# DOGECOIN87/firedancer

Hardware: AMD Instinct MI355X
Metric: verified ed25519 sigs/sec (node) (higher is better)
Workload: dtype u32; 1 GPU; cfg2: 1000000 single-sig txns/GPU, msg U[180,220] B, 90% valid / 10% corrupted, device-resident batch, full verify + per-txn combine per step; parallelism=dp1 (independent per-GPU batches), queues=2

## Files before the change

### firedancer_amd/_lib.py

```python
import ctypes
import os

_HERE = os.path.dirname(os.path.abspath(__file__))
LIB_PATH = os.environ.get("FDGPU_LIB") or os.path.join(_HERE, "libfd_ed25519_gpu.so")
HEADER_PATH = os.path.join(os.path.dirname(_HERE), "include", "fd_ed25519_gpu.h")
SHRED_HEADER_PATH = os.path.join(os.path.dirname(_HERE), "include", "fd_shred_gpu.h")
SHRED_SETS_HEADER_PATH = os.path.join(os.path.dirname(_HERE), "include", "fd_shred_sets_gpu.h")
POH_HEADER_PATH = os.path.join(os.path.dirname(_HERE), "include", "fd_poh_gpu.h")
PRECOMPILE_HEADER_PATH = os.path.join(os.path.dirname(_HERE), "include", "fd_precompile_gpu.h")
SECP256K1_HEADER_PATH = os.path.join(os.path.dirname(_HERE), "include", "fd_secp256k1_gpu.h")

_LIB = None


class FdgpuTxn(ctypes.Structure):
    _fields_ = [("msg_off", ctypes.c_uint32), ("msg_sz", ctypes.c_uint32),
                ("sig_off", ctypes.c_uint32), ("pub_off", ctypes.c_uint32),
                ("sig_cnt", ctypes.c_uint32)]


class FdgpuCfg(ctypes.Structure):
    _fields_ = [("max_txn", ctypes.c_uint64), ("max_sig", ctypes.c_uint64),
                ("max_arena", ctypes.c_uint64), ("ring_depth", ctypes.c_uint32),
                ("flags", ctypes.c_uint32)]


def lib():
    global _LIB
    if _LIB is not None:
        return _LIB
    if not os.path.exists(LIB_PATH):
        raise RuntimeError(f"firedancer_amd: engine library not built: {LIB_PATH} "
                           "(run `make -C firedancer_amd/csrc`)")
    L = ctypes.CDLL(LIB_PATH)
    c = ctypes
    vp, u8p = c.c_void_p, c.c_char_p
    L.fd_ed25519_verify.argtypes = [u8p, c.c_uint64, u8p, u8p, vp]
    L.fd_ed25519_verify.restype = c.c_int
    L.fd_ed25519_verify_batch_single_msg.argtypes = [u8p, c.c_uint64, u8p, u8p, vp, c.c_uint8]
    L.fd_ed25519_verify_batch_single_msg.restype = c.c_int
    L.fd_ed25519_strerror.argtypes = [c.c_int]
    L.fd_ed25519_strerror.restype = c.c_char_p
    L.fdgpu_engine_open.argtypes = [c.c_int, c.POINTER(FdgpuCfg)]
    L.fdgpu_engine_open.restype = vp
    L.fdgpu_engine_reserve.argtypes = [vp, c.c_uint64]
    L.fdgpu_engine_reserve.restype = c.c_int
    L.fdgpu_engine_close.argtypes = [vp]
    L.fdgpu_engine_close.restype = None
    L.fdgpu_last_error.argtypes = []
    L.fdgpu_last_error.restype = c.c_char_p
    L.fdgpu_device_count.argtypes = []
    L.fdgpu_device_count.restype = c.c_int
    L.fdgpu_kernel_path.argtypes = []
    L.fdgpu_kernel_path.restype = c.c_char_p
    L.fdgpu_build_info.argtypes = []
    L.fdgpu_build_info.restype = c.c_char_p
    L.fdgpu_submit.argtypes = [vp, vp, c.c_uint64, vp, c.c_uint64]
    L.fdgpu_submit.restype = c.c_int64
    L.fdgpu_poll.argtypes = [vp, c.c_int64, vp, c.c_int]
    L.fdgpu_poll.restype = c.c_int
    L.fdgpu_stage_acquire.argtypes = [vp, c.POINTER(c.c_uint64)]
    L.fdgpu_stage_acquire.restype = vp
    L.fdgpu_stage_submit.argtypes = [vp, c.c_uint64, vp, c.c_uint64]
    L.fdgpu_stage_submit.restype = c.c_int64
    L.fdgpu_poll_keep.argtypes = [vp, c.c_int64, vp, c.c_int]
    L.fdgpu_poll_keep.restype = c.c_int
    L.fdgpu_release.argtypes = [vp, c.c_int64]
    L.fdgpu_release.restype = c.c_int
    L.fdgpu_stage_cancel.argtypes = [vp]
    L.fdgpu_stage_cancel.restype = c.c_int
    L.fdgpu_host_register.argtypes = [vp, vp, c.c_uint64]
    L.fdgpu_host_register.restype = c.c_int
    L.fdgpu_host_unregister.argtypes = [vp, vp]
    L.fdgpu_host_unregister.restype = c.c_int
    L.fdgpu_verify_device.argtypes = [vp, vp, vp, c.c_uint64, vp, c.c_uint64, vp, vp, vp]
    L.fdgpu_verify_device.restype = c.c_int
    L.fdgpu_engine_info.argtypes = [vp, c.POINTER(c.c_uint32), c.POINTER(c.c_uint32), c.POINTER(c.c_uint64)]
    L.fdgpu_engine_info.restype = c.c_int
    L.fdgpu_debug_fe_ops.argtypes = [vp, vp, c.c_uint64, vp]
    L.fdgpu_debug_decode.argtypes = [vp, vp, c.c_uint64, c.c_int, vp]
    L.fdgpu_debug_sha512.argtypes = [vp, vp, c.c_uint64, vp, c.c_uint64, vp]
    L.fdgpu_debug_hram.argtypes = [vp, vp, c.c_uint64, vp, c.c_uint64, vp]
    L.fdgpu_debug_sc_reduce.argtypes = [vp, vp, c.c_uint64, vp]
    L.fdgpu_debug_hs_split.argtypes = [vp, vp, c.c_uint64, vp]
    L.fdgpu_debug_sig_codes.argtypes = [vp, vp, c.c_uint64, vp, c.c_uint64, vp]
    L.fdgpu_dev_batch_upload.argtypes = [vp, vp, c.c_uint64, vp, c.c_uint64]
    L.fdgpu_dev_batch_upload.restype = vp
    L.fdgpu_dev_batch_verify.argtypes = [vp, vp]
    L.fdgpu_dev_batch_verify.restype = c.c_int
    L.fdgpu_dev_batch_own_queue.argtypes = [vp, vp]
    L.fdgpu_dev_batch_own_queue.restype = c.c_int
    L.fdgpu_dev_batch_codes.argtypes = [vp, vp, vp, vp]
    L.fdgpu_dev_batch_codes.restype = c.c_int
    L.fdgpu_dev_batch_upload_frags.argtypes = [vp, vp, c.c_uint64, vp, c.c_uint64]
    L.fdgpu_dev_batch_upload_frags.restype = vp
    L.fdgpu_dev_batch_txns.argtypes = [vp, vp, vp, vp]
    L.fdgpu_dev_batch_txns.restype = c.c_int
    L.fdgpu_dev_batch_time2.argtypes = [vp, vp, c.c_int] + [c.POINTER(c.c_double)] * 4
    L.fdgpu_dev_batch_time2.restype = c.c_int
    L.fdgpu_dev_batch_free.argtypes = [vp, vp]
    L.fdgpu_dev_batch_free.restype = None
    L.fdgpu_dev_batch_sig_cnt.argtypes = [vp]
    L.fdgpu_dev_batch_sig_cnt.restype = c.c_uint64
    L.fdgpu_dev_batch_device_ptrs.argtypes = [vp] + [vp] * 6
    L.fdgpu_dev_batch_device_ptrs.restype = c.c_int
    L.fdgpu_dev_batch_time.argtypes = [vp, vp, c.c_int, c.POINTER(c.c_double), c.POINTER(c.c_double),
                                       c.POINTER(c.c_double)]
    L.fdgpu_dev_batch_time.restype = c.c_int
    L.fdgpu_sync.argtypes = [vp]
    L.fdgpu_sync.restype = c.c_int
    L.fdgpu_submit_frags.argtypes = [vp, vp, c.c_uint64, vp, c.c_uint64, c.c_uint64]
    L.fdgpu_submit_frags.restype = c.c_int64
    L.fdgpu_poll_frags.argtypes = [vp, c.c_int64, vp, vp, c.c_int]
    L.fdgpu_poll_frags.restype = c.c_int
    L.fdgpu_submit_frags_io.argtypes = [vp, vp, c.c_uint64, vp, c.c_uint64, c.c_uint64, vp, c.c_uint64]
    L.fdgpu_submit_frags_io.restype = c.c_int64
    L.fdgpu_poll_frags_io.argtypes = [vp, c.c_int64, vp, vp, vp, c.c_int]
    L.fdgpu_poll_frags_io.restype = c.c_int
    L.fdgpu_debug_submit_times.argtypes = [vp, c.c_uint64]
    L.fdgpu_debug_submit_times.restype = c.c_uint64
    L.fdgpu_debug_h2d_gbps.argtypes = [vp, vp, c.c_uint64, c.c_int]
    L.fdgpu_debug_h2d_gbps.restype = c.c_double
    L.fdgpu_frag_out_cap.argtypes = [c.c_uint32]
    L.fdgpu_frag_out_cap.restype = c.c_uint32
    L.fdgpu_ed25519_verify.argtypes = [u8p, c.c_uint64, u8p, u8p]
    L.fdgpu_ed25519_verify.restype = c.c_int
    L.fdgpu_ed25519_verify_batch_single_msg.argtypes = [u8p, c.c_uint64, u8p, u8p, c.c_uint8]
    L.fdgpu_ed25519_verify_batch_single_msg.restype = c.c_int
    L.fdgpu_sync_stats.argtypes = [c.POINTER(c.c_uint64)] * 3
    L.fdgpu_sync_stats.restype = None
    L.fdgpu_sync_errors.argtypes = []
    L.fdgpu_sync_errors.restype = c.c_uint64
    L.fdgpu_submit_shreds.argtypes = [vp, vp, c.c_uint64, vp, c.c_uint64, c.c_uint16]
    L.fdgpu_submit_shreds.restype = c.c_int64
    L.fdgpu_poll_shreds.argtypes = [vp, c.c_int64, vp, vp, c.c_int]
    L.fdgpu_poll_shreds.restype = c.c_int
    L.fdgpu_debug_sha256.argtypes = [vp, vp, c.c_uint64, vp, c.c_uint64, vp]
    L.fdgpu_debug_sha256.restype = c.c_int
    L.fdgpu_debug_shred_roots.argtypes = [vp, vp, c.c_uint64, vp, c.c_uint64, c.c_uint16, vp, vp]
    L.fdgpu_debug_shred_roots.restype = c.c_int
    L.fdgpu_debug_shred_time.argtypes = [vp, vp, c.c_uint64, vp, c.c_uint64, c.c_uint16, c.c_int,
                                         c.POINTER(c.c_double), c.POINTER(c.c_double)]
    L.fdgpu_debug_shred_time.restype = c.c_int
    L.fdgpu_submit_shred_sets.argtypes = [vp, vp, c.c_uint64, vp, c.c_uint64, c.c_uint16]
    L.fdgpu_submit_shred_sets.restype = c.c_int64
    L.fdgpu_poll_shred_sets.argtypes = [vp, c.c_int64, vp, vp, vp, c.POINTER(c.c_uint64), c.c_int]
    L.fdgpu_poll_shred_sets.restype = c.c_int
    L.fdgpu_debug_shred_sets_time.argtypes = [vp, vp, c.c_uint64, vp, c.c_uint64, c.c_uint16, c.c_int,
                                              c.POINTER(c.c_double), c.POINTER(c.c_double)]
    L.fdgpu_debug_shred_sets_time.restype = c.c_int
    L.fdgpu_submit_poh.argtypes = [vp, vp, c.c_uint64, vp, c.c_uint64, vp, c.c_uint64, c.c_uint64]
    L.fdgpu_submit_poh.restype = c.c_int64
    L.fdgpu_poll_poh.argtypes = [vp, c.c_int64, vp, vp, c.c_int]
    L.fdgpu_poll_poh.restype = c.c_int
    L.fdgpu_poh_limits.argtypes = [vp] + [c.POINTER(c.c_uint64)] * 3
    L.fdgpu_poh_limits.restype = c.c_int
    L.fdgpu_poh_chunk.argtypes = []
    L.fdgpu_poh_chunk.restype = c.c_uint32
    L.fdgpu_debug_poh.argtypes = [vp, vp, c.c_uint64, vp, c.c_uint64, vp, c.c_uint64, c.c_uint64, c.c_uint32, vp, vp]
    L.fdgpu_debug_poh.restype = c.c_int
    L.fdgpu_debug_poh_time.argtypes = [vp, vp, c.c_uint64, vp, c.c_uint64, vp, c.c_uint64, c.c_uint64, c.c_int,
                                       c.POINTER(c.c_double), c.POINTER(c.c_double)]
    L.fdgpu_debug_poh_time.restype = c.c_int
    L.fdgpu_precompile_sig_bound.argtypes = [c.c_uint64]
    L.fdgpu_precompile_sig_bound.restype = c.c_uint32
    L.fdgpu_submit_precompiles.argtypes = [vp, vp, c.c_uint64, vp, c.c_uint64]
    L.fdgpu_submit_precompiles.restype = c.c_int64
    L.fdgpu_poll_precompiles.argtypes = [vp, c.c_int64, vp, vp, c.c_int]
    L.fdgpu_poll_precompiles.restype = c.c_int
    L.fdgpu_debug_precompile_walk.argtypes = [vp, vp, c.c_uint64, vp, c.c_uint64, vp, vp, vp, c.c_uint64,
                                              c.POINTER(c.c_uint64)]
    L.fdgpu_debug_precompile_walk.restype = c.c_int
    L.fdgpu_debug_precompile_time.argtypes = [vp, vp, c.c_uint64, vp, c.c_uint64, c.c_int, c.POINTER(c.c_double),
                                              c.POINTER(c.c_double)]
    L.fdgpu_debug_precompile_time.restype = c.c_int
    L.fdgpu_secp256k1_sig_bound.argtypes = [c.c_uint64]
    L.fdgpu_secp256k1_sig_bound.restype = c.c_uint32
    L.fdgpu_submit_secp256k1.argtypes = [vp, vp, c.c_uint64, vp, c.c_uint64, c.c_uint32]
    L.fdgpu_submit_secp256k1.restype = c.c_int64
    L.fdgpu_poll_secp256k1.argtypes = [vp, c.c_int64, vp, vp, c.c_int]
    L.fdgpu_poll_secp256k1.restype = c.c_int
    L.fdgpu_debug_secp256k1_walk.argtypes = [vp, vp, c.c_uint64, vp, c.c_uint64, c.c_uint32, vp, vp, vp, c.c_uint64,
                                             c.POINTER(c.c_uint64)]
    L.fdgpu_debug_secp256k1_walk.restype = c.c_int
    L.fdgpu_debug_keccak256.argtypes = [vp, vp, c.c_uint64, vp, c.c_uint64, vp]
    L.fdgpu_debug_keccak256.restype = c.c_int
    L.fdgpu_debug_secp256k1_recover.argtypes = [vp, vp, c.c_uint64, vp, vp]
    L.fdgpu_debug_secp256k1_recover.restype = c.c_int
    L.fdgpu_debug_secp256k1_time.argtypes = [vp, vp, c.c_uint64, vp, c.c_uint64, c.c_uint32, c.c_int,
                                             c.POINTER(c.c_double), c.POINTER(c.c_double)]
    L.fdgpu_debug_secp256k1_time.restype = c.c_int
    L.fdgpu_debug_secp256k1_ops.argtypes = [vp, vp, c.c_uint64, vp]
    L.fdgpu_debug_secp256k1_ops.restype = c.c_int
    L.fdgpu_debug_fe_raw.argtypes = [vp, vp, c.c_uint64, vp]
    L.fdgpu_debug_ge_ops.argtypes = [vp, vp, c.c_uint64, vp]
    L.fdgpu_debug_sc_recode.argtypes = [vp, vp, c.c_uint64, vp]
    L.fdgpu_debug_btab.argtypes = [vp, c.c_uint64, c.c_uint64, vp]
    L.fdgpu_debug_tabpack.argtypes = [vp, vp, c.c_uint64, vp]
    L.fdgpu_debug_verify_prehashed.argtypes = [vp, vp, c.c_uint64, vp, c.c_uint64, c.c_uint32, vp,
                                               c.POINTER(c.c_uint32)]
    L.fdgpu_bcomb_dim.argtypes = [c.c_int]
    L.fdgpu_bcomb_dim.restype = c.c_uint32
    L.fdgpu_test_ge_in_words.argtypes = []
    L.fdgpu_test_ge_in_words.restype = c.c_uint32
    L.fdgpu_test_ge_results.argtypes = []
    L.fdgpu_test_ge_results.restype = c.c_uint32
    for fn in ("fdgpu_debug_fe_ops", "fdgpu_debug_decode", "fdgpu_debug_sha512", "fdgpu_debug_hram",
               "fdgpu_debug_sc_reduce", "fdgpu_debug_hs_split", "fdgpu_debug_sig_codes",
               "fdgpu_debug_fe_raw", "fdgpu_debug_ge_ops", "fdgpu_debug_sc_recode", "fdgpu_debug_btab",
               "fdgpu_debug_tabpack", "fdgpu_debug_verify_prehashed"):
        getattr(L, fn).restype = c.c_int
    _LIB = L
    return L


def header_functions(path=None):
    import re
    text = open(path or HEADER_PATH).read()
    text = re.sub(r"/\*.*?\*/", "", text, flags=re.S)
    names = re.findall(r"^[A-Za-z_][\w \t\*]*?\b(fd\w+)\s*\(", text, flags=re.M)
    return sorted(set(n for n in names if not n.startswith("FD_")))


def build_info():
    import json
    return json.loads(lib().fdgpu_build_info().decode())


def require_product_build(allow_ab=False):
    info = build_info()
    if not info.get("product") and not allow_ab:
        raise RuntimeError(f"firedancer_amd: {LIB_PATH} is not the product build: {info} "
                           "(rebuild with `make -C firedancer_amd/csrc`, or pass the A/B flag)")
    return info


def last_error():
    return lib().fdgpu_last_error().decode()
```

### firedancer_amd/csrc/fdgpu_atab.h

```cpp
#pragma once

#include <hip/hip_runtime.h>

#include "fdgpu_ge.h"
#include "fdgpu_internal.h"

namespace fdgpu {

FDG_DEV void fe_tight(fe &h) {
#pragma unroll
  for (int pass = 0; pass < 2; pass++) {
#pragma unroll
    for (int i = 0; i < 9; i++) {
      const int w = (i & 1) ? 25 : 26;
      h.v[i + 1] += h.v[i] >> w;
      h.v[i] &= (1u << w) - 1;
    }
    const uint32_t c = h.v[9] >> 25;
    h.v[9] &= (1u << 25) - 1;
    h.v[0] += 19u * c;
  }
}

FDG_DEV void fe_pack8(uint32_t (&w)[8], const fe &t) {
#pragma unroll
  for (int h = 0; h < 2; h++) {
    const uint32_t s = t.v[8 + h];
    w[4 * h + 0] = t.v[4 * h + 0] | (s << 26);
    w[4 * h + 1] = t.v[4 * h + 1] | ((s >> 6) << 25);
    w[4 * h + 2] = t.v[4 * h + 2] | ((s >> 13) << 26);
    w[4 * h + 3] = t.v[4 * h + 3] | ((s >> 19) << 25);
  }
}

FDG_DEV void fe_unpack8(uint32_t *q, const uint32_t (&w)[8]) {
#pragma unroll
  for (int j = 0; j < 8; j++) q[j] = w[j] & ((j & 1) ? (1u << 25) - 1 : (1u << 26) - 1);
#pragma unroll
  for (int h = 0; h < 2; h++) {
    uint32_t s = w[4 * h + 3] >> 25;
    s = (s << 6) | (w[4 * h + 2] >> 26);
    s = (s << 7) | (w[4 * h + 1] >> 25);
    s = (s << 6) | (w[4 * h + 0] >> 26);
    q[8 + h] = s;
  }
}

__host__ __device__ constexpr int atab_pos(int c, int j) {
  return c >= 2 ? 8 * c + j : 4 * (j / 2) + 2 * c + (j % 2);
}

struct alignas(128) tab_ident_t { uint32_t w[FDGPU_PTAB_WORDS]; };
static __device__ const tab_ident_t g_tab_ident = {{1u, 0u, 1u, 0u, 0u, 0u, 0u, 0u, 0u, 0u, 0u, 0u, 0u, 0u, 0u, 0u, 2u}};
static_assert(atab_pos(0, 0) == 0 && atab_pos(1, 0) == 2 && atab_pos(2, 0) == 16 && atab_pos(3, 7) == 31 &&
              atab_pos(0, 7) == 13 && atab_pos(1, 7) == 15, "the stored order (and the identity entry's)");

FDG_DEV const uint32_t *tab_entry(const uint32_t *tab, int e) {
  return e ? tab + (uint32_t)(e < 0 ? -e : e) * FDGPU_PTAB_WORDS : g_tab_ident.w;
}

FDG_DEV void atab_store(uint32_t *tab, uint32_t entry, const ge_cached &c) {
  uint4 *p = (uint4 *)(tab + entry * FDGPU_PTAB_WORDS);
  uint32_t o[FDGPU_PTAB_WORDS];
#pragma unroll
  for (int cc = 0; cc < 4; cc++) {
    fe t = cc == 0 ? c.YpX : cc == 1 ? c.YmX : cc == 2 ? c.Z2 : c.T2d;
    fe_tight(t);
    uint32_t w[8];
    fe_pack8(w, t);
#pragma unroll
    for (int j = 0; j < 8; j++) o[atab_pos(cc, j)] = w[j];
  }
#pragma unroll
  for (int q = 0; q < 8; q++) p[q] = make_uint4(o[4 * q], o[4 * q + 1], o[4 * q + 2], o[4 * q + 3]);
}

FDG_DEV void atab_unpack(uint32_t (&q)[40], const uint32_t (&o)[FDGPU_PTAB_WORDS]) {
#pragma unroll
  for (int cc = 0; cc < 4; cc++) {
    uint32_t w[8];
#pragma unroll
    for (int j = 0; j < 8; j++) w[j] = o[atab_pos(cc, j)];
    fe_unpack8(q + 10 * cc, w);
  }
}

FDG_DEV void atab_load(uint32_t (&q)[40], const uint32_t *tab, int e) {
  const uint4 *ent = (const uint4 *)tab_entry(tab, e);
  uint32_t o[FDGPU_PTAB_WORDS];
#pragma unroll
  for (int i = 0; i < 8; i++) {
    const uint4 v = ent[i];
    o[4 * i] = v.x; o[4 * i + 1] = v.y; o[4 * i + 2] = v.z; o[4 * i + 3] = v.w;
  }
  atab_unpack(q, o);
}

FDG_DEV uint32_t atab_limb(const uint32_t *ent, int c, int w) {
  if (w < 8) return ent[atab_pos(c, w)] & ((w & 1) ? (1u << 25) - 1 : (1u << 26) - 1);
  const int b = 4 * (w - 8);
  uint32_t s = ent[atab_pos(c, b + 3)] >> 25;
  s = (s << 6) | (ent[atab_pos(c, b + 2)] >> 26);
  s = (s << 7) | (ent[atab_pos(c, b + 1)] >> 25);
  s = (s << 6) | (ent[atab_pos(c, b + 0)] >> 26);
  return s;
}

typedef __attribute__((address_space(3))) void lds_void_t;

FDG_DEV void stage_entry(uint32_t *lds_wave, const uint32_t *tab, int e) {
  const uint32_t *src = tab_entry(tab, e);
  constexpr int NCH = FDGPU_PTAB_WORDS / 4;
#pragma unroll
  for (int c = 0; c < NCH; c++)
    __builtin_amdgcn_global_load_lds((const void *)(src + 4 * c), (lds_void_t *)(lds_wave + 256 * c), 16, 0, 0);
}

FDG_DEV void unstage_entry_signed(uint32_t (&q)[40], const uint32_t *lds_wave, bool neg) {
  const uint32_t lane = threadIdx.x & 63u;
  const uint32_t *a = lds_wave + 4 * lane + (neg ? 2u : 0u), *b = lds_wave + 4 * lane + (neg ? 0u : 2u);
  uint32_t o[FDGPU_PTAB_WORDS];
#pragma unroll
  for (int c = 0; c < 4; c++) {
    const uint2 x = *(const uint2 *)(a + 256 * c), y = *(const uint2 *)(b + 256 * c);
    o[4 * c] = x.x; o[4 * c + 1] = x.y; o[4 * c + 2] = y.x; o[4 * c + 3] = y.y;
  }
#pragma unroll
  for (int c = 4; c < 8; c++) {
    const uint4 v = *(const uint4 *)(lds_wave + 256 * c + 4 * lane);
    o[4 * c] = v.x; o[4 * c + 1] = v.y; o[4 * c + 2] = v.z; o[4 * c + 3] = v.w;
  }
  atab_unpack(q, o);
}

}
```

### firedancer_amd/csrc/fdgpu_consts.h

```cpp
#pragma once
#include <stdint.h>

#define FDGPU_FE_D { 0x35978a3u, 0x0d37284u, 0x3156ebdu, 0x06a0a0eu, 0x001c029u, 0x179e898u, 0x3a03cbbu, 0x1ce7198u, 0x2e2b6ffu, 0x1480db3u }
#define FDGPU_FE_D2 { 0x2b2f159u, 0x1a6e509u, 0x22add7au, 0x0d4141du, 0x0038052u, 0x0f3d130u, 0x3407977u, 0x19ce331u, 0x1c56dffu, 0x0901b67u }
#define FDGPU_FE_SQRTM1 { 0x20ea0b0u, 0x186c9d2u, 0x08f189du, 0x035697fu, 0x0bd0c60u, 0x1fbd7a7u, 0x2804c9eu, 0x1e16569u, 0x004fc1du, 0x0ae0c92u }
#define FDGPU_FE_BX { 0x325d51au, 0x18b5823u, 0x0f6592au, 0x104a92du, 0x1a4b31du, 0x1d6dc5cu, 0x27118feu, 0x07fd814u, 0x13cd6e5u, 0x085a4dbu }
#define FDGPU_FE_BY { 0x2666658u, 0x1999999u, 0x0ccccccu, 0x1333333u, 0x1999999u, 0x0666666u, 0x3333333u, 0x0ccccccu, 0x2666666u, 0x1999999u }
#define FDGPU_FE_BT { 0x1b7dda3u, 0x1a2ace9u, 0x25eadbbu, 0x003ba8au, 0x083c27eu, 0x0abe37du, 0x1274732u, 0x0ccacddu, 0x0fd78b7u, 0x19e1d7cu }
#define FDGPU_FE_Y0 { 0x395e826u, 0x1ecb0a3u, 0x068b604u, 0x1944fa6u, 0x3c263bfu, 0x1acdfd5u, 0x1e36982u, 0x1162726u, 0x2d88023u, 0x017f14du }
#define FDGPU_FE_Y1 { 0x06a17c7u, 0x0134f5cu, 0x39749fbu, 0x06bb059u, 0x03d9c40u, 0x053202au, 0x21c967du, 0x0e9d8d9u, 0x1277fdcu, 0x1e80eb2u }

#define FDGPU_FE_2P { 0x07ffffdau, 0x03fffffeu, 0x07fffffeu, 0x03fffffeu, 0x07fffffeu, 0x03fffffeu, 0x07fffffeu, 0x03fffffeu, 0x07fffffeu, 0x03fffffeu }
#define FDGPU_FE_4P { 0x0fffffb4u, 0x07fffffcu, 0x0ffffffcu, 0x07fffffcu, 0x0ffffffcu, 0x07fffffcu, 0x0ffffffcu, 0x07fffffcu, 0x0ffffffcu, 0x07fffffcu }

#define FDGPU_SC_L { 0x5cf5d3edu, 0x5812631au, 0xa2f79cd6u, 0x14def9deu, 0x00000000u, 0x00000000u, 0x00000000u, 0x10000000u }
#define FDGPU_SC_MU { 0x0a2c131bu, 0xed9ce5a3u, 0x086329a7u, 0x2106215du, 0xffffffebu, 0xffffffffu, 0xffffffffu, 0xffffffffu, 0x0000000fu }
```

### firedancer_amd/csrc/fdgpu_diag.cpp

```cpp
#include "fdgpu_engine.h"
#include "fdgpu_shred.h"

using namespace fdgpu;

#define DALLOC(buf, n) do { if ((buf).alloc((size_t)(n) * sizeof(*(buf).p) + 64) != hipSuccess) { \
  set_err("alloc"); return FDGPU_ERR_DEVICE; } } while (0)

using MsgLaunch = hipError_t (*)(const uint8_t *, const fdgpu_sig_desc_t *, uint32_t, uint32_t *, hipStream_t);
static int debug_msgs(fdgpu_engine_t *e, uint8_t const *arena, uint64_t arena_sz, fdgpu_txn_t const *txns, uint64_t n,
                      uint8_t *out, MsgLaunch launch, uint64_t out_bytes, bool sig_pub) {
  if (!e || !n) return FDGPU_ERR_INVAL;
  HIPCHK(hipSetDevice(e->device), FDGPU_ERR_DEVICE);
  std::vector<fdgpu_sig_desc_t> d(n);
  for (uint64_t i = 0; i < n; i++) {
    if ((uint64_t)txns[i].msg_off + txns[i].msg_sz > arena_sz ||
        (sig_pub && ((uint64_t)txns[i].sig_off + 64 > arena_sz || (uint64_t)txns[i].pub_off + 32 > arena_sz))) {
      set_err("descriptor out of bounds"); return FDGPU_ERR_INVAL;
    }
    d[i].msg_off = txns[i].msg_off; d[i].msg_sz = txns[i].msg_sz;
    d[i].sig_off = txns[i].sig_off; d[i].pub_off = txns[i].pub_off;
  }
  DevBuf<uint8_t> da;
  DevBuf<fdgpu_sig_desc_t> dd;
  DevBuf<uint8_t> dout;
  HIPCHK(dev_arena(da, arena, arena_sz), FDGPU_ERR_DEVICE);
  DALLOC(dd, n);
  DALLOC(dout, n * out_bytes);
  HIPCHK(hipMemcpy(dd, d.data(), n * sizeof(fdgpu_sig_desc_t), hipMemcpyHostToDevice), FDGPU_ERR_DEVICE);
  HIPCHK(launch(da, dd, (uint32_t)n, (uint32_t *)dout.p, e->compute), FDGPU_ERR_DEVICE);
  HIPCHK(hipStreamSynchronize(e->compute), FDGPU_ERR_DEVICE);
  HIPCHK(hipMemcpy(out, dout, n * out_bytes, hipMemcpyDeviceToHost), FDGPU_ERR_DEVICE);
  return FDGPU_OK;
}

template <class Launch>
static int debug_map(fdgpu_engine_t *e, uint8_t const *in, uint64_t n, uint64_t in_words, uint64_t out_words,
                     uint8_t *out, Launch launch) {
  if (!e || !n) return FDGPU_ERR_INVAL;
  HIPCHK(hipSetDevice(e->device), FDGPU_ERR_DEVICE);
  DevBuf<uint32_t> din, dout;
  DALLOC(din, n * in_words);
  DALLOC(dout, n * out_words);
  HIPCHK(hipMemcpy(din, in, n * in_words * 4, hipMemcpyHostToDevice), FDGPU_ERR_DEVICE);
  HIPCHK(launch(din.p, dout.p, (uint32_t)n, e->compute), FDGPU_ERR_DEVICE);
  HIPCHK(hipStreamSynchronize(e->compute), FDGPU_ERR_DEVICE);
  HIPCHK(hipMemcpy(out, dout, n * out_words * 4, hipMemcpyDeviceToHost), FDGPU_ERR_DEVICE);
  return FDGPU_OK;
}

int fdgpu::time_two_stages(hipStream_t st, int iters, const char *what, const std::function<bool()> &warm,
                           const std::function<bool()> &first, const std::function<bool()> &second, double *first_ms,
                           double *second_ms) {
  Events ev;
  if (!ev.create(3)) { (void)hipGetLastError(); set_err("event"); return FDGPU_ERR_DEVICE; }
  bool ok = warm() && hipEventRecord(ev[0], st) == hipSuccess;
  for (int i = 0; i < iters && ok; i++) ok = first();
  ok = ok && hipEventRecord(ev[1], st) == hipSuccess;
  for (int i = 0; i < iters && ok; i++) ok = second();
  ok = ok && hipEventRecord(ev[2], st) == hipSuccess && hipEventSynchronize(ev[2]) == hipSuccess;
  float a = 0.f, b = 0.f;
  ok = ok && hipEventElapsedTime(&a, ev[0], ev[1]) == hipSuccess && hipEventElapsedTime(&b, ev[1], ev[2]) == hipSuccess;
  if (!ok) { (void)hipGetLastError(); set_err("%s timing failed", what); return FDGPU_ERR_DEVICE; }
  *first_ms = a / iters;
  *second_ms = b / iters;
  return FDGPU_OK;
}

extern "C" {

int fdgpu_debug_fe_ops(fdgpu_engine_t *e, uint8_t const *ab, uint64_t n, uint8_t *out) {
  return debug_map(e, ab, n, 16, 64, out, fdgpu_launch_test_fe);
}

int fdgpu_debug_decode(fdgpu_engine_t *e, uint8_t const *enc, uint64_t n, int ref_mapping, uint8_t *out) {
  const uint32_t flags = ref_mapping ? FDGPU_FLAG_REF_MAP : 0u;
  return debug_map(e, enc, n, 8, 18, out, [flags](const uint32_t *i, uint32_t *o, uint32_t k, hipStream_t st) {
    return fdgpu_launch_test_decode(i, o, k, flags, st);
  });
}

int fdgpu_debug_sha512(fdgpu_engine_t *e, uint8_t const *arena, uint64_t arena_sz, fdgpu_txn_t const *msgs,
                       uint64_t n, uint8_t *out) {
  return debug_msgs(e, arena, arena_sz, msgs, n, out, fdgpu_launch_test_sha512, 64, false);
}

int fdgpu_debug_hram(fdgpu_engine_t *e, uint8_t const *arena, uint64_t arena_sz, fdgpu_txn_t const *txns,
                     uint64_t n, uint8_t *out) {
  return debug_msgs(e, arena, arena_sz, txns, n, out, fdgpu_launch_test_hram, 32, true);
}

int fdgpu_debug_sha256(fdgpu_engine_t *e, uint8_t const *arena, uint64_t arena_sz, fdgpu_txn_t const *msgs, uint64_t n,
                       uint8_t *out) {
  if (!e || !n || !msgs || !out || (!arena && arena_sz) || arena_sz > 0xFFFFFF00ull) { set_err("bad argument"); return FDGPU_ERR_INVAL; }
  return debug_msgs(e, arena, arena_sz, msgs, n, out, fdgpu_launch_test_sha256, 32, false);
}

int fdgpu_debug_sc_reduce(fdgpu_engine_t *e, uint8_t const *in, uint64_t n, uint8_t *out) {
  return debug_map(e, in, n, 16, 8, out, fdgpu_launch_test_sc_reduce);
}

int fdgpu_debug_hs_split(fdgpu_engine_t *e, uint8_t const *k, uint64_t n, uint8_t *out) {
  return debug_map(e, k, n, 8, 16, out, fdgpu_launch_test_hs_split);
}

int fdgpu_debug_fe_raw(fdgpu_engine_t *e, uint8_t const *fg, uint64_t n, uint8_t *out) {
  return debug_map(e, fg, n, 20, 80, out, fdgpu_launch_test_fe_raw);
}

int fdgpu_debug_ge_ops(fdgpu_engine_t *e, uint8_t const *in, uint64_t n, uint8_t *out) {
  return debug_map(e, in, n, fdgpu_test_ge_in_words(), 32u * fdgpu_test_ge_results(), out, fdgpu_launch_test_ge);
}

int fdgpu_debug_sc_recode(fdgpu_engine_t *e, uint8_t const *s, uint64_t n, uint8_t *out) {
  return debug_map(e, s, n, 8, 16, out, fdgpu_launch_test_sc_recode);
}

int fdgpu_debug_tabpack(fdgpu_engine_t *e, uint8_t const *in, uint64_t n, uint8_t *out) {
  return debug_map(e, in, n, FDGPU_ATAB_WORDS, FDGPU_TABPACK_OUT_WORDS, out, fdgpu_launch_test_tabpack);
}

int fdgpu_debug_verify_prehashed(fdgpu_engine_t *e, uint8_t const *arena, uint64_t arena_sz,
                                 fdgpu_sig_desc_t const *descs, uint64_t n, uint32_t flags, int8_t *codes_out,
                                 uint32_t *n_full_out) {
  if (!e || !e->d_btab || !arena || !descs || !codes_out || !n_full_out || !n || n > (1u << 20) ||
      arena_sz > 0xFFFFFF00ull || (flags & ~(uint32_t)(FDGPU_FLAG_REF_MAP | FDGPU_FLAG_KFULL | FDGPU_FLAG_KPAIR))) {
    set_err("fdgpu_debug_verify_prehashed: bad argument"); return FDGPU_ERR_INVAL;
  }
  for (uint64_t i = 0; i < n; i++) {
    if ((descs[i].msg_off & 7u) || (uint64_t)descs[i].msg_off + 64 > arena_sz ||
        (uint64_t)descs[i].sig_off + 64 > arena_sz || (uint64_t)descs[i].pub_off + 32 > arena_sz) {
      set_err("fdgpu_debug_verify_prehashed: descriptor out of bounds"); return FDGPU_ERR_INVAL;
    }
  }
  HIPCHK(hipSetDevice(e->device), FDGPU_ERR_DEVICE);
  DevBuf<uint8_t> da;
  DevBuf<fdgpu_sig_desc_t> dd;
  DevBuf<int8_t> dc;
  DevBuf<uint32_t> dws;
  HIPCHK(dev_arena(da, arena, arena_sz), FDGPU_ERR_DEVICE);
  DALLOC(dd, n);
  DALLOC(dc, n);
  if (dws.alloc(fdgpu_ws_bytes(n)) != hipSuccess) { set_err("alloc"); return FDGPU_ERR_DEVICE; }
  HIPCHK(hipMemcpy(dd, descs, n * sizeof(fdgpu_sig_desc_t), hipMemcpyHostToDevice), FDGPU_ERR_DEVICE);
  HIPCHK(hipMemsetAsync(dc, 0x7f, n, e->compute), FDGPU_ERR_DEVICE);
  HIPCHK(fdgpu_launch_verify_prehashed(da, dd, (uint32_t)n, e->d_btab, dws, dc, flags, e->compute), FDGPU_ERR_DEVICE);
  HIPCHK(hipStreamSynchronize(e->compute), FDGPU_ERR_DEVICE);
  HIPCHK(hipMemcpy(codes_out, dc, n, hipMemcpyDeviceToHost), FDGPU_ERR_DEVICE);
  HIPCHK(hipMemcpy(n_full_out, fdgpu_ws_layout(dws, n).cnt, sizeof(uint32_t), hipMemcpyDeviceToHost), FDGPU_ERR_DEVICE);
  return FDGPU_OK;
}

int fdgpu_debug_btab(fdgpu_engine_t *e, uint64_t first_entry, uint64_t n_entries, uint32_t *out) {
  const uint64_t total = (uint64_t)FDGPU_BCOMB_NDIG * FDGPU_BCOMB_ENTRIES;
  if (!e || !e->d_btab || !out || first_entry > total || n_entries > total - first_entry) {
    set_err("fdgpu_debug_btab: entries out of the table"); return FDGPU_ERR_INVAL;
  }
  if (!n_entries) return FDGPU_OK;
  HIPCHK(hipSetDevice(e->device), FDGPU_ERR_DEVICE);
  HIPCHK(hipStreamSynchronize(e->compute), FDGPU_ERR_DEVICE);
  HIPCHK(hipMemcpy(out, e->d_btab + first_entry * FDGPU_BCOMB_STRIDE, n_entries * FDGPU_BCOMB_STRIDE * sizeof(uint32_t),
                   hipMemcpyDeviceToHost), FDGPU_ERR_DEVICE);
  return FDGPU_OK;
}

uint32_t fdgpu_bcomb_dim(int which) {
  switch (which) {
    case 0: return FDGPU_BCOMB_BITS;
    case 1: return FDGPU_BCOMB_NDIG;
    case 2: return FDGPU_BCOMB_ENTRIES;
    case 3: return FDGPU_BCOMB_STRIDE;
    case 4: return FDGPU_BCOMB_CHUNK;
    default: return 0u;
  }
}

int fdgpu_debug_sig_codes(fdgpu_engine_t *e, uint8_t const *arena, uint64_t arena_sz, fdgpu_txn_t const *txns,
                          uint64_t txn_cnt, int8_t *sig_codes) {
  if (!e) return FDGPU_ERR_INVAL;
  HIPCHK(hipSetDevice(e->device), FDGPU_ERR_DEVICE);
  uint64_t total = 0;
  for (uint64_t t = 0; t < txn_cnt; t++) total += (txns[t].sig_cnt >= 1 && txns[t].sig_cnt <= 16) ? txns[t].sig_cnt : 0;
  std::vector<fdgpu_sig_desc_t> sd(total + 1);
  std::vector<fdgpu_txn_desc_t> td(txn_cnt + 1);
  std::vector<uint32_t> pm(total + 1);
  uint32_t *perm = bucket(e) ? pm.data() : nullptr;
  const int64_t ns = expand(arena_sz, txns, txn_cnt, total, sd.data(), td.data(), perm);
  if (ns < 0) return FDGPU_ERR_INVAL;
  if (!ns) return FDGPU_OK;
  DevBuf<uint8_t> da;
  DevBuf<fdgpu_sig_desc_t> dd;
  DevBuf<uint32_t> dp;
  DevBuf<int8_t> dc;
  HIPCHK(dev_arena(da, arena, arena_sz), FDGPU_ERR_DEVICE);
  DALLOC(dd, ns);
  DALLOC(dp, ns);
  DALLOC(dc, ns);
  HIPCHK(hipMemcpy(dd, sd.data(), ns * sizeof(fdgpu_sig_desc_t), hipMemcpyHostToDevice), FDGPU_ERR_DEVICE);
  if (perm) HIPCHK(hipMemcpy(dp, perm, ns * sizeof(uint32_t), hipMemcpyHostToDevice), FDGPU_ERR_DEVICE);
  const uint32_t flags = kflags(e);
  if ((uint64_t)ns > e->ws_sig) { int rc = ensure_ws(e, (uint64_t)ns); if (rc) return rc; }
  HIPCHK(fdgpu_launch_verify_sigs(da, dd, (uint32_t)ns, perm ? dp.p : nullptr, e->d_btab, e->d_ws, dc, flags,
                                  e->compute, nullptr, e->resident_blocks, e->kc_seed),
         FDGPU_ERR_DEVICE);
  HIPCHK(hipStreamSynchronize(e->compute), FDGPU_ERR_DEVICE);
  HIPCHK(hipMemcpy(sig_codes, dc, ns, hipMemcpyDeviceToHost), FDGPU_ERR_DEVICE);
  return FDGPU_OK;
}

}
```

### firedancer_amd/csrc/fdgpu_ge.h

```cpp
#pragma once

#include "fdgpu_fe.h"

namespace fdgpu {

struct ge_p2 { fe X, Y, Z; };
struct ge_p3 { fe X, Y, Z, T; };
struct ge_p1p1 { fe X, Y, Z, T; };
struct ge_cached { fe YpX, YmX, Z2, T2d; };
struct ge_niels { fe ypx, ymx, xy2d; };

FDG_DEV void ge_p2_0(ge_p2 &h) { fe_0(h.X); fe_1(h.Y); fe_1(h.Z); }
FDG_DEV void ge_p3_0(ge_p3 &h) { fe_0(h.X); fe_1(h.Y); fe_1(h.Z); fe_0(h.T); }
FDG_DEV void ge_cached_0(ge_cached &h) { fe_1(h.YpX); fe_1(h.YmX); fe_0(h.Z2); h.Z2.v[0] = 2; fe_0(h.T2d); }

FDG_DEV void ge_p1p1_to_p2(ge_p2 &r, const ge_p1p1 &p) {
  fe_mul(r.X, p.X, p.T);
  fe_mul(r.Y, p.Z, p.Y);
  fe_mul(r.Z, p.Z, p.T);
}
FDG_DEV void ge_p1p1_to_p3(ge_p3 &r, const ge_p1p1 &p) {
  fe_mul(r.X, p.X, p.T);
  fe_mul(r.Y, p.Z, p.Y);
  fe_mul(r.Z, p.Z, p.T);
  fe_mul(r.T, p.X, p.Y);
}

FDG_DEV void ge_dbl(ge_p1p1 &r, const ge_p2 &p) {
  fe s;
  fe_sq(r.X, p.X);
  fe_sq(r.Z, p.Y);
  fe_add(r.Y, r.Z, r.X);
  fe_sub(r.Z, r.Z, r.X);
  fe_add(s, p.X, p.Y);
  fe_sq(r.X, s);
  fe_sub4(r.X, r.X, r.Y);
  fe_sq2(r.T, p.Z);
  fe_sub4(r.T, r.T, r.Z);
  fe_carry_par(r.T);
}

FDG_DEV void fe_cswap(fe &a, fe &b, bool c) {
#pragma unroll
  for (int i = 0; i < 10; i++) { const uint32_t x = a.v[i], y = b.v[i]; a.v[i] = c ? y : x; b.v[i] = c ? x : y; }
}
FDG_DEV void fe_cneg(fe &a, bool c) {
  constexpr uint32_t P2[10] = FDGPU_FE_2P;
#pragma unroll
  for (int i = 0; i < 10; i++) a.v[i] = c ? P2[i] - a.v[i] : a.v[i];
}

FDG_DEV void ge_add_cached(ge_p1p1 &r, const ge_p3 &p, ge_cached q, bool neg) {
  fe t;
  fe_cswap(q.YpX, q.YmX, neg);
  fe_cneg(q.T2d, neg);
  fe_mul(r.Z, p.T, q.T2d);
  fe_mul(r.T, p.Z, q.Z2);
  fe_add(t, p.Y, p.X);
  fe_mul(r.X, t, q.YpX);
  fe_sub(t, p.Y, p.X);
  fe_mul(r.Y, t, q.YmX);
  fe_add(t, r.T, r.Z);
  fe_sub(r.T, r.T, r.Z);
  r.Z = t;
  fe_add(t, r.X, r.Y);
  fe_sub(r.X, r.X, r.Y);
  r.Y = t;
}

FDG_DEV void ge_add_niels(ge_p1p1 &r, const ge_p3 &p, ge_niels q, bool neg) {
  fe t;
  fe_cswap(q.ypx, q.ymx, neg);
  fe_cneg(q.xy2d, neg);
  fe_mul(r.Z, p.T, q.xy2d);
  fe_add(r.T, p.Z, p.Z);
  fe_add(t, p.Y, p.X);
  fe_mul(r.X, t, q.ypx);
  fe_sub(t, p.Y, p.X);
  fe_mul(r.Y, t, q.ymx);
  fe_add(t, r.T, r.Z);
  fe_sub(r.T, r.T, r.Z);
  fe_carry(r.T);
  r.Z = t;
  fe_add(t, r.X, r.Y);
  fe_sub(r.X, r.X, r.Y);
  r.Y = t;
}

template <class LD>
FDG_DEV void ld_fe(fe &h, const LD &ld, int coord) {
#pragma unroll
  for (int i = 0; i < 10; i++) h.v[i] = ld(coord, i);
}

template <class LD>
FDG_DEV void ge_add_cached_ld(ge_p1p1 &r, const ge_p3 &p, const LD &ld, bool neg) {
  fe t, q;
  ld_fe(q, ld, 3); fe_cneg(q, neg);
  fe_mul(r.Z, p.T, q);
  ld_fe(q, ld, 2);
  fe_mul(r.T, p.Z, q);
  ld_fe(q, ld, neg ? 1 : 0);
  fe_add(t, p.Y, p.X);
  fe_mul(r.X, t, q);
  ld_fe(q, ld, neg ? 0 : 1);
  fe_sub(t, p.Y, p.X);
  fe_mul(r.Y, t, q);
  fe_add(t, r.T, r.Z);
  fe_sub(r.T, r.T, r.Z);
  r.Z = t;
  fe_add(t, r.X, r.Y);
  fe_sub(r.X, r.X, r.Y);
  r.Y = t;
}

template <class LD>
FDG_DEV void ge_add_niels_ld(ge_p1p1 &r, const ge_p3 &p, const LD &ld, bool neg) {
  fe t, q;
  ld_fe(q, ld, 2); fe_cneg(q, neg);
  fe_mul(r.Z, p.T, q);
  fe_add(r.T, p.Z, p.Z);
  ld_fe(q, ld, neg ? 1 : 0);
  fe_add(t, p.Y, p.X);
  fe_mul(r.X, t, q);
  ld_fe(q, ld, neg ? 0 : 1);
  fe_sub(t, p.Y, p.X);
  fe_mul(r.Y, t, q);
  fe_add(t, r.T, r.Z);
  fe_sub(r.T, r.T, r.Z);
  fe_carry_par(r.T);
  r.Z = t;
  fe_add(t, r.X, r.Y);
  fe_sub(r.X, r.X, r.Y);
  r.Y = t;
}

FDG_DEV void ge_add_cached_regs(ge_p1p1 &r, const ge_p3 &p, const uint32_t (&q)[40], bool neg) {
  fe t, c;
#pragma unroll
  for (int i = 0; i < 10; i++) c.v[i] = q[30 + i];
  fe_cneg(c, neg);
  fe_mul(r.Z, p.T, c);
#pragma unroll
  for (int i = 0; i < 10; i++) c.v[i] = q[20 + i];
  fe_mul(r.T, p.Z, c);
#pragma unroll
  for (int i = 0; i < 10; i++) c.v[i] = neg ? q[10 + i] : q[i];
  fe_add(t, p.Y, p.X);
  fe_mul(r.X, t, c);
#pragma unroll
  for (int i = 0; i < 10; i++) c.v[i] = neg ? q[i] : q[10 + i];
  fe_sub(t, p.Y, p.X);
  fe_mul(r.Y, t, c);
  fe_add(t, r.T, r.Z);
  fe_sub(r.T, r.T, r.Z);
  r.Z = t;
  fe_add(t, r.X, r.Y);
  fe_sub(r.X, r.X, r.Y);
  r.Y = t;
}

FDG_DEV void ge_add_cached_regs_swapped(ge_p1p1 &r, const ge_p3 &p, const uint32_t (&q)[40], bool neg) {
  fe t, c;
#pragma unroll
  for (int i = 0; i < 10; i++) c.v[i] = q[30 + i];
  fe_cneg(c, neg);
  fe_mul(r.Z, p.T, c);
#pragma unroll
  for (int i = 0; i < 10; i++) c.v[i] = q[20 + i];
  fe_mul(r.T, p.Z, c);
#pragma unroll
  for (int i = 0; i < 10; i++) c.v[i] = q[i];
  fe_add(t, p.Y, p.X);
  fe_mul(r.X, t, c);
#pragma unroll
  for (int i = 0; i < 10; i++) c.v[i] = q[10 + i];
  fe_sub(t, p.Y, p.X);
  fe_mul(r.Y, t, c);
  fe_add(t, r.T, r.Z);
  fe_sub(r.T, r.T, r.Z);
  r.Z = t;
  fe_add(t, r.X, r.Y);
  fe_sub(r.X, r.X, r.Y);
  r.Y = t;
}

FDG_DEV void ge_cached_regs_to_p2(ge_p2 &r, const uint32_t (&q)[40], bool neg) {
  fe a, b;
#pragma unroll
  for (int i = 0; i < 10; i++) { a.v[i] = neg ? q[10 + i] : q[i]; b.v[i] = neg ? q[i] : q[10 + i]; }
  fe_sub(r.X, a, b); fe_carry(r.X);
  fe_add(r.Y, a, b); fe_carry(r.Y);
#pragma unroll
  for (int i = 0; i < 10; i++) r.Z.v[i] = q[20 + i];
}

FDG_DEV void ge_niels_regs_to_p3(ge_p3 &r, const uint32_t (&q)[32], bool neg) {
  fe a, b, x2, y2;
#pragma unroll
  for (int i = 0; i < 10; i++) { a.v[i] = neg ? q[10 + i] : q[i]; b.v[i] = neg ? q[i] : q[10 + i]; }
  fe_sub(x2, a, b); fe_carry(x2);
  fe_add(y2, a, b); fe_carry(y2);
  fe_mul(r.T, x2, y2);
  fe_add(r.X, x2, x2); fe_carry(r.X);
  fe_add(r.Y, y2, y2); fe_carry(r.Y);
  fe_0(r.Z); r.Z.v[0] = 4;
}

FDG_DEV void ge_add_niels_regs(ge_p1p1 &r, const ge_p3 &p, const uint32_t (&q)[32], bool neg) {
  fe t, c;
#pragma unroll
  for (int i = 0; i < 10; i++) c.v[i] = q[20 + i];
  fe_cneg(c, neg);
  fe_mul(r.Z, p.T, c);
  fe_add(r.T, p.Z, p.Z);
#pragma unroll
  for (int i = 0; i < 10; i++) c.v[i] = neg ? q[10 + i] : q[i];
  fe_add(t, p.Y, p.X);
  fe_mul(r.X, t, c);
#pragma unroll
  for (int i = 0; i < 10; i++) c.v[i] = neg ? q[i] : q[10 + i];
  fe_sub(t, p.Y, p.X);
  fe_mul(r.Y, t, c);
  fe_add(t, r.T, r.Z);
  fe_sub(r.T, r.T, r.Z);
  fe_carry_par(r.T);
  r.Z = t;
  fe_add(t, r.X, r.Y);
  fe_sub(r.X, r.X, r.Y);
  r.Y = t;
}

FDG_DEV void ge_p3_to_cached(ge_cached &r, const ge_p3 &p) {
  constexpr uint32_t D2[10] = FDGPU_FE_D2;
  fe d2; fe_set(d2, D2);
  fe_add(r.YpX, p.Y, p.X); fe_carry(r.YpX);
  fe_sub(r.YmX, p.Y, p.X); fe_carry(r.YmX);
  fe_add(r.Z2, p.Z, p.Z);  fe_carry(r.Z2);
  fe_mul(r.T2d, p.T, d2);
}

FDG_DEV void ge_p3_to_p2(ge_p2 &r, const ge_p3 &p) { r.X = p.X; r.Y = p.Y; r.Z = p.Z; }

FDG_DEV void ge_p3_neg(ge_p3 &r, const ge_p3 &p) {
  fe_neg(r.X, p.X); fe_carry(r.X);
  r.Y = p.Y; r.Z = p.Z;
  fe_neg(r.T, p.T); fe_carry(r.T);
}

FDG_DEV bool ge_decode(ge_p3 &P, const uint32_t (&enc)[8], bool ref_map) {
  constexpr uint32_t DD[10] = FDGPU_FE_D, SQ[10] = FDGPU_FE_SQRTM1;
  fe d, sqrtm1, one;
  fe_set(d, DD); fe_set(sqrtm1, SQ); fe_1(one);
  const uint32_t sign = enc[7] >> 31;
  fe y, ysq, u, v, v2, v3, v4, uv3, uv7, t0, x, x2, vx2, t1, t2;
  fe_frombytes(y, enc);
  fe_sq(ysq, y);
  fe_sub(u, ysq, one);
  fe_mul(v, d, ysq); fe_add(v, v, one);
  fe_sq(v2, v);
  fe_sq(v4, v2);
  fe_mul(v3, v, v2);
  fe_mul(uv3, u, v3);
  fe_mul(uv7, uv3, v4);
  fe_pow22523(t0, uv7);
  fe_mul(x, uv3, t0);
  fe_sq(x2, x);
  fe_mul(vx2, v, x2);
  fe_carry(u);
  fe_sub(t1, vx2, u);
  fe_add(t2, vx2, u);
  const bool t1nz = !fe_iszero(t1), t2nz = !fe_iszero(t2);
  bool ok = !(t1nz && t2nz);
  fe xs; fe_mul(xs, x, sqrtm1);
  fe_cmov(x, xs, x, t1nz);
  fe xc = x; fe_canon(xc);
  uint32_t xnz = 0;
#pragma unroll
  for (int i = 0; i < 10; i++) xnz |= xc.v[i];
  if (!ref_map && xnz == 0 && sign) ok = false;
  fe nx; fe_neg(nx, xc); fe_carry(nx);
  fe_cmov(x, nx, xc, (xc.v[0] & 1u) != sign);
  P.X = x; P.Y = y; fe_1(P.Z); fe_mul(P.T, x, y);
  return ok;
}

FDG_DEV bool ge_is_small_order_affine(const ge_p3 &P) {
  constexpr uint32_t Y0[10] = FDGPU_FE_Y0, Y1[10] = FDGPU_FE_Y1;
  fe y0, y1; fe_set(y0, Y0); fe_set(y1, Y1);
  fe yc = P.Y; fe_canon(yc);
  bool yz = true, e0 = true, e1 = true;
#pragma unroll
  for (int i = 0; i < 10; i++) { yz &= yc.v[i] == 0; e0 &= yc.v[i] == y0.v[i]; e1 &= yc.v[i] == y1.v[i]; }
  return fe_iszero(P.X) || yz || e0 || e1;
}

}
```

### firedancer_amd/csrc/fdgpu_internal.h

```cpp
#pragma once

#include <hip/hip_runtime_api.h>
#include <stddef.h>
#include <stdint.h>

#include "../../include/fd_ed25519_gpu.h"
#include "../../include/fd_poh_gpu.h"

typedef struct {
  uint32_t msg_off;
  uint32_t msg_sz;
  uint32_t sig_off;
  uint32_t pub_off;
} fdgpu_sig_desc_t;

typedef struct {
  uint32_t sig0;
  uint32_t sig_cnt;
} fdgpu_txn_desc_t;

#define FDGPU_ARENA_SLACK   160u
#define FDGPU_ATAB_ENTRIES  9u
#ifndef FDGPU_ATAB_WORDS
#define FDGPU_ATAB_WORDS    40u
#endif
#define FDGPU_PTAB_WORDS    32u
#ifndef FDGPU_VERIFY_WAVES
#define FDGPU_VERIFY_WAVES  2
#endif
#ifndef FDGPU_PHASE_STAMPS
#define FDGPU_PHASE_STAMPS  0
#endif
#define FDGPU_BCOMB_BITS    16u
#define FDGPU_BCOMB_NDIG    ((254u + FDGPU_BCOMB_BITS - 1u) / FDGPU_BCOMB_BITS)
#define FDGPU_BCOMB_ENTRIES ((1u << (FDGPU_BCOMB_BITS - 1u)) + 1u)
#define FDGPU_BCOMB_STRIDE  32u
#define FDGPU_BCOMB_CHUNK   64u
#define HS_MAX_WIN          40u
#define FDGPU_TAB_STORED    (FDGPU_ATAB_ENTRIES - 1u)
#define FDGPU_WS_RTAB       FDGPU_TAB_STORED
#define FDGPU_WS_ENTRIES    (2u * FDGPU_TAB_STORED + 2u)
#define FDGPU_WS_LANE_WORDS (FDGPU_WS_ENTRIES * FDGPU_ATAB_WORDS)
#define FDGPU_WS_TAB_WORDS  (2u * FDGPU_TAB_STORED * FDGPU_PTAB_WORDS)
#define FDGPU_WS_AUX_WORDS  (FDGPU_WS_LANE_WORDS - FDGPU_WS_TAB_WORDS)
#define FDGPU_AUX_PARK      0u
#define FDGPU_AUX_SB        FDGPU_ATAB_WORDS
#define FDGPU_BLOCK         256u
#define FDGPU_FLAG_REF_MAP  1u
#define FDGPU_FLAG_KFULL    2u
#define FDGPU_FLAG_KCACHE   4u
#define FDGPU_FLAG_KPAIR    8u
#define FDGPU_FLAG_KSPREAD  16u
#define FDGPU_STAGE_WAVE_WORDS (FDGPU_PTAB_WORDS / 4u * 256u)
#define FDGPU_STAGE_LDS        (FDGPU_BLOCK / 64u * 2u * FDGPU_STAGE_WAVE_WORDS * 4u)
#define FDGPU_STAGE_LDS_PAIR   (FDGPU_BLOCK / 64u * FDGPU_STAGE_WAVE_WORDS * 4u)
#define FDGPU_CU_LDS           (160u * 1024u)
#define FDGPU_SPREAD_LDS       (FDGPU_CU_LDS / 2u - FDGPU_STAGE_LDS + 1024u)
#define FDGPU_SPREAD_LDS_PAIR  (FDGPU_CU_LDS / 2u - FDGPU_STAGE_LDS_PAIR + 1024u)
#ifdef __cplusplus
static_assert(2u * (FDGPU_STAGE_LDS + FDGPU_SPREAD_LDS) > FDGPU_CU_LDS &&
              2u * (FDGPU_STAGE_LDS_PAIR + FDGPU_SPREAD_LDS_PAIR) > FDGPU_CU_LDS &&
              FDGPU_STAGE_LDS + FDGPU_SPREAD_LDS <= FDGPU_CU_LDS && FDGPU_STAGE_LDS_PAIR + FDGPU_SPREAD_LDS_PAIR <= FDGPU_CU_LDS,
              "a spread launch's LDS admits one block per CU, and no more");
#endif
#define FDGPU_FULL_BLOCKS   16u
#define FDGPU_AUX_BLOCKS    64u
#define FDGPU_IO_BLOCKS     16u
#define FDGPU_NBLK_GROUPS   32u
#define FDGPU_POH_CHUNK     64u

#ifdef __cplusplus
extern "C" {
#endif


size_t     fdgpu_btab_bytes(void);
hipError_t fdgpu_btab_build(uint32_t *d_btab, hipStream_t stream);

hipError_t fdgpu_launch_verify_sigs(const uint8_t *d_arena, const fdgpu_sig_desc_t *d_sigs, uint32_t n_sig,
                                    const uint32_t *d_perm, const uint32_t *d_btab, uint32_t *d_ws,
                                    int8_t *d_sig_codes, uint32_t flags, hipStream_t stream,
                                    const uint32_t *d_n_sig, uint32_t resident_blocks, uint64_t kc_seed,
                                    int cnt_zeroed = 0);
uint64_t   fdgpu_sha512_stream_blocks(uint64_t msg_sz);
hipError_t fdgpu_launch_sha512_stream(const uint8_t *d_mbuf, uint64_t m0, uint64_t mlen, uint64_t msg_sz,
                                      uint64_t blk0, uint32_t nblk, const uint8_t *d_ra, uint64_t *d_state,
                                      uint32_t n, hipStream_t stream);
hipError_t fdgpu_launch_verify_prehashed(const uint8_t *d_arena, const fdgpu_sig_desc_t *d_sigs, uint32_t n_sig,
                                         const uint32_t *d_btab, uint32_t *d_ws, int8_t *d_sig_codes, uint32_t flags,
                                         hipStream_t stream);
typedef struct {
  uint64_t lanes, ht_slots;
  uint32_t *queue, *cnt, *rep_cnt, *ht, *key_of, *kverd, *reps;
  size_t bytes;
} fdgpu_ws_layout_t;
static inline fdgpu_ws_layout_t fdgpu_ws_layout(uint32_t *d_ws, uint64_t n_sig) {
  fdgpu_ws_layout_t l;
  l.lanes = (n_sig + FDGPU_BLOCK - 1) / FDGPU_BLOCK * FDGPU_BLOCK;
  for (l.ht_slots = 64; l.ht_slots < 2 * l.lanes;) l.ht_slots <<= 1;
  const uint64_t queue = l.lanes * FDGPU_WS_LANE_WORDS, cnt = queue + l.lanes, ht = cnt + 16, key_of = ht + l.ht_slots;
  auto at = [d_ws](uint64_t word) { return d_ws ? d_ws + word : nullptr; };
  l.queue = at(queue);
  l.cnt = at(cnt);
  l.rep_cnt = at(cnt + 1);
  l.ht = at(ht);
  l.key_of = at(key_of);
  l.kverd = at(key_of + l.lanes);
  l.reps = at(key_of + 2 * l.lanes);
  l.bytes = (size_t)(key_of + 3 * l.lanes) * sizeof(uint32_t);
  return l;
}
typedef struct {
  const uint8_t *arena;
  const fdgpu_sig_desc_t *sigs;
  const uint32_t *n_sig;
  uint32_t *ws;
  int8_t *codes;
  uint32_t *queue, *cnt;
  uint32_t bound;
  uint32_t slow;
} fdgpu_mbatch_t;
hipError_t fdgpu_launch_verify_multi(const fdgpu_mbatch_t *mb, uint32_t nb, uint32_t grid_max, uint32_t slow_max,
                                     const uint32_t *d_btab, uint32_t flags, hipStream_t stream);
hipError_t fdgpu_launch_combine(const fdgpu_txn_desc_t *d_txns, uint32_t n_txn, const int8_t *d_sig_codes,
                                int8_t *d_txn_codes, uint64_t *d_accept, hipStream_t stream);
hipError_t fdgpu_verify_occupancy(int *blocks_per_cu);
int        fdgpu_kernel_build_info(char *buf, size_t n);
size_t     fdgpu_ws_bytes(uint64_t n_sig);

__attribute__((visibility("hidden"))) hipError_t fdgpu_ingest_load(void);
uint64_t   fdgpu_frag_sig_bound(uint32_t sz);
hipError_t fdgpu_launch_frag_ingest(const uint8_t *d_arena, const void *d_frags, uint32_t frag_stride, uint32_t n,
                                    uint8_t *d_txn_out, uint16_t *d_txn_sz, fdgpu_txn_t *d_txd, uint32_t *d_cnt,
                                    uint32_t *d_sig0, uint32_t *d_blocktot, uint32_t *d_n_sig,
                                    fdgpu_sig_desc_t *d_sigs, fdgpu_txn_desc_t *d_tds, hipStream_t stream);
hipError_t fdgpu_launch_frag_codes(const uint16_t *d_txn_sz, uint32_t n, int8_t *d_codes, hipStream_t stream);
#define FDGPU_SMALL_SCAN_MAX 65536u
hipError_t fdgpu_launch_frag_ring(const uint8_t *d_arena, const fdgpu_frag_ex_t *d_fx, uint32_t n, uint8_t *d_txn_out,
                                  uint16_t *d_txn_sz, fdgpu_txn_t *d_txd, uint32_t *d_cnt, uint32_t *d_sig0,
                                  uint32_t *d_blocktot, uint32_t *d_n_sig, fdgpu_sig_desc_t *d_sigs,
                                  fdgpu_txn_desc_t *d_tds, hipStream_t stream);
hipError_t fdgpu_launch_frag_finish(const fdgpu_txn_desc_t *d_tds, uint32_t n, const int8_t *d_sig_codes,
                                    const uint16_t *d_txn_sz, const fdgpu_frag_ex_t *d_fx, const uint8_t *d_txn_out,
                                    int8_t *d_codes, uint8_t *d_trailers, hipStream_t stream);
#define FDGPU_FX_LAPPED 0x80000000u
#define FDGPU_IO_RANGES_MAX 255u
uint64_t   fdgpu_frag_fp_bound(uint32_t sz);
hipError_t fdgpu_launch_frag_ingest_io(const uint64_t *d_src, const fdgpu_frag_ex_t *d_fx, const uint64_t *d_chk,
                                       const uint64_t *d_rtab, uint32_t n, uint8_t *d_arena,
                                       fdgpu_frag_ex_t *d_fx_dev, uint8_t *d_txn_out, uint16_t *d_txn_sz,
                                       fdgpu_sig_desc_t *d_sigs, fdgpu_txn_desc_t *d_tds, uint32_t *d_n_sig,
                                       uint32_t *d_zero_word, hipStream_t stream);
hipError_t fdgpu_launch_frag_finish_io(const fdgpu_txn_desc_t *d_tds, uint32_t n, const int8_t *d_sig_codes,
                                       const uint16_t *d_txn_sz, const fdgpu_frag_ex_t *d_fx, const uint8_t *d_txn_out,
                                       const uint8_t *d_arena, uint64_t hash_seed, uint8_t *d_out, int8_t *d_codes,
                                       uint64_t *d_tags, uint16_t *d_out_szs, uint32_t *d_zero_next,
                                       hipStream_t stream);

hipError_t fdgpu_launch_poh_tree(const uint8_t *d_arena, const fdgpu_poh_entry_t *d_entries, uint32_t n,
                                 const uint32_t *d_sig_offs, uint32_t sig_total, uint32_t *d_nodes, hipStream_t stream);
hipError_t fdgpu_launch_poh_chains(const uint8_t *d_arena, const fdgpu_poh_entry_t *d_entries, uint32_t n,
                                   const uint32_t *d_order, uint32_t n_q, const uint32_t *d_nodes, uint32_t cap,
                                   uint32_t grid_waves, uint32_t *d_head, int8_t *d_codes, uint8_t *d_hashes,
                                   hipStream_t stream);

hipError_t fdgpu_launch_test_fe(const uint32_t *d_in, uint32_t *d_out, uint32_t n, hipStream_t stream);
hipError_t fdgpu_launch_test_decode(const uint32_t *d_enc, uint32_t *d_out, uint32_t n, uint32_t flags, hipStream_t stream);
hipError_t fdgpu_launch_test_sha512(const uint8_t *d_arena, const fdgpu_sig_desc_t *d_msgs, uint32_t n,
                                    uint32_t *d_out, hipStream_t stream);
hipError_t fdgpu_launch_test_hram(const uint8_t *d_arena, const fdgpu_sig_desc_t *d_sigs, uint32_t n,
                                  uint32_t *d_out, hipStream_t stream);
hipError_t fdgpu_launch_test_sc_reduce(const uint32_t *d_in, uint32_t *d_out, uint32_t n, hipStream_t stream);
hipError_t fdgpu_launch_test_hs_split(const uint32_t *d_in, uint32_t *d_out, uint32_t n, hipStream_t stream);
hipError_t fdgpu_launch_test_fe_raw(const uint32_t *d_in, uint32_t *d_out, uint32_t n, hipStream_t stream);
uint32_t   fdgpu_test_ge_in_words(void);
uint32_t   fdgpu_test_ge_results(void);
hipError_t fdgpu_launch_test_ge(const uint32_t *d_in, uint32_t *d_out, uint32_t n, hipStream_t stream);
hipError_t fdgpu_launch_test_sc_recode(const uint32_t *d_in, uint32_t *d_out, uint32_t n, hipStream_t stream);
#define FDGPU_TABPACK_OUT_WORDS 160u
hipError_t fdgpu_launch_test_tabpack(const uint32_t *d_in, uint32_t *d_out, uint32_t n, hipStream_t stream);

int      fdgpu_debug_fe_raw(fdgpu_engine_t *e, uint8_t const *fg, uint64_t n, uint8_t *out);
int      fdgpu_debug_ge_ops(fdgpu_engine_t *e, uint8_t const *in, uint64_t n, uint8_t *out);
int      fdgpu_debug_sc_recode(fdgpu_engine_t *e, uint8_t const *s, uint64_t n, uint8_t *out);
int      fdgpu_debug_tabpack(fdgpu_engine_t *e, uint8_t const *in, uint64_t n, uint8_t *out);
int      fdgpu_debug_verify_prehashed(fdgpu_engine_t *e, uint8_t const *arena, uint64_t arena_sz,
                                      fdgpu_sig_desc_t const *descs, uint64_t n, uint32_t flags, int8_t *codes_out,
                                      uint32_t *n_full_out);
int      fdgpu_debug_btab(fdgpu_engine_t *e, uint64_t first_entry, uint64_t n_entries, uint32_t *out);
uint32_t fdgpu_bcomb_dim(int which);

#ifdef __cplusplus
}
#endif
```

### firedancer_amd/csrc/fdgpu_sha512.h

```cpp
#pragma once

#include "fdgpu_fe.h"

namespace fdgpu {

__constant__ static const uint64_t SHA512_K[80] = {
  0x428a2f98d728ae22ULL, 0x7137449123ef65cdULL, 0xb5c0fbcfec4d3b2fULL, 0xe9b5dba58189dbbcULL,
  0x3956c25bf348b538ULL, 0x59f111f1b605d019ULL, 0x923f82a4af194f9bULL, 0xab1c5ed5da6d8118ULL,
  0xd807aa98a3030242ULL, 0x12835b0145706fbeULL, 0x243185be4ee4b28cULL, 0x550c7dc3d5ffb4e2ULL,
  0x72be5d74f27b896fULL, 0x80deb1fe3b1696b1ULL, 0x9bdc06a725c71235ULL, 0xc19bf174cf692694ULL,
  0xe49b69c19ef14ad2ULL, 0xefbe4786384f25e3ULL, 0x0fc19dc68b8cd5b5ULL, 0x240ca1cc77ac9c65ULL,
  0x2de92c6f592b0275ULL, 0x4a7484aa6ea6e483ULL, 0x5cb0a9dcbd41fbd4ULL, 0x76f988da831153b5ULL,
  0x983e5152ee66dfabULL, 0xa831c66d2db43210ULL, 0xb00327c898fb213fULL, 0xbf597fc7beef0ee4ULL,
  0xc6e00bf33da88fc2ULL, 0xd5a79147930aa725ULL, 0x06ca6351e003826fULL, 0x142929670a0e6e70ULL,
  0x27b70a8546d22ffcULL, 0x2e1b21385c26c926ULL, 0x4d2c6dfc5ac42aedULL, 0x53380d139d95b3dfULL,
  0x650a73548baf63deULL, 0x766a0abb3c77b2a8ULL, 0x81c2c92e47edaee6ULL, 0x92722c851482353bULL,
  0xa2bfe8a14cf10364ULL, 0xa81a664bbc423001ULL, 0xc24b8b70d0f89791ULL, 0xc76c51a30654be30ULL,
  0xd192e819d6ef5218ULL, 0xd69906245565a910ULL, 0xf40e35855771202aULL, 0x106aa07032bbd1b8ULL,
  0x19a4c116b8d2d0c8ULL, 0x1e376c085141ab53ULL, 0x2748774cdf8eeb99ULL, 0x34b0bcb5e19b48a8ULL,
  0x391c0cb3c5c95a63ULL, 0x4ed8aa4ae3418acbULL, 0x5b9cca4f7763e373ULL, 0x682e6ff3d6b2b8a3ULL,
  0x748f82ee5defb2fcULL, 0x78a5636f43172f60ULL, 0x84c87814a1f0ab72ULL, 0x8cc702081a6439ecULL,
  0x90befffa23631e28ULL, 0xa4506cebde82bde9ULL, 0xbef9a3f7b2c67915ULL, 0xc67178f2e372532bULL,
  0xca273eceea26619cULL, 0xd186b8c721c0c207ULL, 0xeada7dd6cde0eb1eULL, 0xf57d4f7fee6ed178ULL,
  0x06f067aa72176fbaULL, 0x0a637dc5a2c898a6ULL, 0x113f9804bef90daeULL, 0x1b710b35131c471bULL,
  0x28db77f523047d84ULL, 0x32caab7b40c72493ULL, 0x3c9ebe0a15c9bebcULL, 0x431d67c49c100d4cULL,
  0x4cc5d4becb3e42b6ULL, 0x597f299cfc657e2aULL, 0x5fcb6fab3ad6faecULL, 0x6c44198c4a475817ULL,
};

FDG_DEV uint64_t rotr64(uint64_t x, int r) {
  const uint32_t lo = (uint32_t)x, hi = (uint32_t)(x >> 32);
  const uint32_t a = r < 32 ? hi : lo, b = r < 32 ? lo : hi, n = (uint32_t)(r & 31);
  return ((uint64_t)__builtin_amdgcn_alignbit(b, a, n) << 32) | __builtin_amdgcn_alignbit(a, b, n);
}
FDG_DEV uint64_t maj64(uint64_t a, uint64_t b, uint64_t c) {
  const uint32_t lo = __builtin_amdgcn_bitop3_b32((uint32_t)a, (uint32_t)b, (uint32_t)c, 0xE8);
  const uint32_t hi = __builtin_amdgcn_bitop3_b32((uint32_t)(a >> 32), (uint32_t)(b >> 32), (uint32_t)(c >> 32), 0xE8);
  return ((uint64_t)hi << 32) | lo;
}
FDG_DEV uint64_t shr64(uint64_t x, int r) {
  const uint32_t lo = (uint32_t)x, hi = (uint32_t)(x >> 32);
  return ((uint64_t)(hi >> r) << 32) | __builtin_amdgcn_alignbit(hi, lo, (uint32_t)r);
}
FDG_DEV uint64_t xor3_64(uint64_t a, uint64_t b, uint64_t c) {
  const uint32_t lo = __builtin_amdgcn_bitop3_b32((uint32_t)a, (uint32_t)b, (uint32_t)c, 0x96);
  const uint32_t hi = __builtin_amdgcn_bitop3_b32((uint32_t)(a >> 32), (uint32_t)(b >> 32), (uint32_t)(c >> 32), 0x96);
  return ((uint64_t)hi << 32) | lo;
}
FDG_DEV uint32_t bswap32(uint32_t x) { return __builtin_bswap32(x); }

FDG_DEV void sha512_compress(uint64_t (&h)[8], uint64_t (&w)[16]) {
  uint64_t a = h[0], b = h[1], c = h[2], d = h[3], e = h[4], f = h[5], g = h[6], hh = h[7];
  for (int r = 0; r < 80; r += 16) {
#pragma unroll
    for (int t = 0; t < 16; t++) {
      if (r) {
        const uint64_t w15 = w[(t + 1) & 15], w2 = w[(t + 14) & 15];
        const uint64_t s0 = xor3_64(rotr64(w15, 1), rotr64(w15, 8), shr64(w15, 7));
        const uint64_t s1 = xor3_64(rotr64(w2, 19), rotr64(w2, 61), shr64(w2, 6));
        w[t] += s0 + w[(t + 9) & 15] + s1;
      }
      const uint64_t S1 = xor3_64(rotr64(e, 14), rotr64(e, 18), rotr64(e, 41));
      const uint64_t ch = (e & f) ^ (~e & g);
      const uint64_t t1 = hh + S1 + ch + SHA512_K[r + t] + w[t];
      const uint64_t S0 = xor3_64(rotr64(a, 28), rotr64(a, 34), rotr64(a, 39));
      const uint64_t maj = maj64(a, b, c);
      hh = g; g = f; f = e; e = d + t1; d = c; c = b; b = a; a = t1 + S0 + maj;
    }
  }
  h[0] += a; h[1] += b; h[2] += c; h[3] += d; h[4] += e; h[5] += f; h[6] += g; h[7] += hh;
}

FDG_DEV uint32_t load_u32_unaligned(const uint8_t *p) {
  const uint32_t mis = (uint32_t)((uintptr_t)p & 3u);
  const uint32_t *q = (const uint32_t *)(p - mis);
  const uint32_t lo = q[0], hi = q[1];
  return (uint32_t)((((uint64_t)hi << 32) | lo) >> (8u * mis));
}

template <int T0>
FDG_DEV void msg_block(uint64_t (&w)[16], const uint8_t *msg, uint32_t msg_sz, uint32_t base) {
  constexpr int NW = 16 - T0;
  const uint32_t lb = base < msg_sz ? base : 0u;
  const uint8_t *p = msg + lb;
  const uint32_t mis = (uint32_t)((uintptr_t)p & 3u);
  const uint32_t *q = (const uint32_t *)(p - mis);
  uint32_t d[2 * NW + 1];
#pragma unroll
  for (int i = 0; i < 2 * NW + 1; i++) d[i] = q[i];
#pragma unroll
  for (int u = 0; u < NW; u++) {
    const uint32_t lo = (uint32_t)((((uint64_t)d[2 * u + 1] << 32) | d[2 * u]) >> (8u * mis));
    const uint32_t hi = (uint32_t)((((uint64_t)d[2 * u + 2] << 32) | d[2 * u + 1]) >> (8u * mis));
    uint64_t v = ((uint64_t)hi << 32) | lo;
    const int64_t rem = (int64_t)msg_sz - (int64_t)base - 8 * u;
    if (rem < 8) {
      const int n = rem < 0 ? 0 : (int)rem;
      v = n ? (v & ((~0ull) >> (64 - 8 * n))) : 0ull;
      if (rem >= 0) v |= 0x80ull << (8 * n);
    }
    w[T0 + u] = ((uint64_t)bswap32((uint32_t)v) << 32) | bswap32((uint32_t)(v >> 32));
  }
}

FDG_DEV uint32_t sha512_hram_blocks(uint32_t msg_sz) { return (64u + msg_sz + 16u) / 128u + 1u; }

FDG_DEV void sha512_hram(uint64_t (&h)[8], const uint32_t (&R)[8], const uint32_t (&A)[8],
                         const uint8_t *msg, uint32_t msg_sz, uint32_t nblk_wave) {
  const uint64_t H0[8] = {0x6a09e667f3bcc908ULL, 0xbb67ae8584caa73bULL, 0x3c6ef372fe94f82bULL,
                          0xa54ff53a5f1d36f1ULL, 0x510e527fade682d1ULL, 0x9b05688c2b3e6c1fULL,
                          0x1f83d9abfb41bd6bULL, 0x5be0cd19137e2179ULL};
#pragma unroll
  for (int i = 0; i < 8; i++) h[i] = H0[i];
  const uint32_t nblk = sha512_hram_blocks(msg_sz);
  const uint64_t bitlen = (uint64_t)(64u + msg_sz) * 8u;
  for (uint32_t blk = 0; blk < nblk_wave; blk++) {
    uint64_t w[16];
    if (blk == 0) {
      msg_block<8>(w, msg, msg_sz, 0u);
#pragma unroll
      for (int t = 0; t < 4; t++) w[t] = ((uint64_t)bswap32(R[2 * t]) << 32) | bswap32(R[2 * t + 1]);
#pragma unroll
      for (int t = 0; t < 4; t++) w[4 + t] = ((uint64_t)bswap32(A[2 * t]) << 32) | bswap32(A[2 * t + 1]);
    } else {
      msg_block<0>(w, msg, msg_sz, 128u * blk - 64u);
    }
    if (blk + 1 == nblk) { w[14] = 0; w[15] = bitlen; }
    uint64_t hs[8];
#pragma unroll
    for (int i = 0; i < 8; i++) hs[i] = h[i];
    sha512_compress(hs, w);
    if (blk < nblk) {
#pragma unroll
      for (int i = 0; i < 8; i++) h[i] = hs[i];
    }
  }
}

FDG_DEV void sha512_plain(uint64_t (&h)[8], const uint8_t *msg, uint32_t msg_sz, uint32_t nblk_wave) {
  const uint64_t H0[8] = {0x6a09e667f3bcc908ULL, 0xbb67ae8584caa73bULL, 0x3c6ef372fe94f82bULL,
                          0xa54ff53a5f1d36f1ULL, 0x510e527fade682d1ULL, 0x9b05688c2b3e6c1fULL,
                          0x1f83d9abfb41bd6bULL, 0x5be0cd19137e2179ULL};
#pragma unroll
  for (int i = 0; i < 8; i++) h[i] = H0[i];
  const uint32_t nblk = (msg_sz + 16u) / 128u + 1u;
  const uint64_t bitlen = (uint64_t)msg_sz * 8u;
  for (uint32_t blk = 0; blk < nblk_wave; blk++) {
    uint64_t w[16];
    msg_block<0>(w, msg, msg_sz, 128u * blk);
    if (blk + 1 == nblk) { w[14] = 0; w[15] = bitlen; }
    uint64_t hs[8];
#pragma unroll
    for (int i = 0; i < 8; i++) hs[i] = h[i];
    sha512_compress(hs, w);
    if (blk < nblk) {
#pragma unroll
      for (int i = 0; i < 8; i++) h[i] = hs[i];
    }
  }
}

}
```

### firedancer_amd/csrc/fdgpu_test_kernels.hip

```cpp
#include <hip/hip_runtime.h>

#include "fdgpu_atab.h"
#include "fdgpu_ge.h"
#include "fdgpu_hram.h"
#include "fdgpu_internal.h"
#include "fdgpu_lattice.h"
#include "fdgpu_sc.h"
#include "fdgpu_sha512.h"

using namespace fdgpu;

namespace {

__global__ void __launch_bounds__(64) fdgpu_test_fe_kernel(const uint32_t *in, uint32_t *out, uint32_t n) {
  const uint32_t i = blockIdx.x * blockDim.x + threadIdx.x;
  if (i >= n) return;
  uint32_t aw[8], bw[8];
#pragma unroll
  for (int j = 0; j < 8; j++) { aw[j] = in[16 * i + j]; bw[j] = in[16 * i + 8 + j]; }
  fe a, b, r;
  fe_frombytes(a, aw); fe_frombytes(b, bw);
  uint32_t o[8];
  uint32_t *dst = out + 64 * i;
  fe_mul(r, a, b); fe_tobytes(o, r);
  for (int j = 0; j < 8; j++) dst[j] = o[j];
  fe_sq(r, a); fe_tobytes(o, r);
  for (int j = 0; j < 8; j++) dst[8 + j] = o[j];
  fe_add(r, a, b); fe_tobytes(o, r);
  for (int j = 0; j < 8; j++) dst[16 + j] = o[j];
  fe_sub(r, a, b); fe_tobytes(o, r);
  for (int j = 0; j < 8; j++) dst[24 + j] = o[j];
  fe_pow22523(r, a); fe_tobytes(o, r);
  for (int j = 0; j < 8; j++) dst[32 + j] = o[j];
  fe_invert(r, a); fe_tobytes(o, r);
  for (int j = 0; j < 8; j++) dst[40 + j] = o[j];
  fe_tobytes(o, a);
  for (int j = 0; j < 8; j++) dst[48 + j] = o[j];
  fe_neg(r, a); fe_tobytes(o, r);
  for (int j = 0; j < 8; j++) dst[56 + j] = o[j];
}

__global__ void __launch_bounds__(64) fdgpu_test_decode_kernel(const uint32_t *enc, uint32_t *out, uint32_t n, uint32_t flags) {
  const uint32_t i = blockIdx.x * blockDim.x + threadIdx.x;
  if (i >= n) return;
  uint32_t e[8];
  for (int j = 0; j < 8; j++) e[j] = enc[8 * i + j];
  ge_p3 P;
  const bool ok = ge_decode(P, e, (flags & FDGPU_FLAG_REF_MAP) != 0);
  uint32_t *dst = out + 18 * i;
  dst[0] = ok ? 0u : 0xffffffffu;
  dst[1] = ok ? (ge_is_small_order_affine(P) ? 1u : 0u) : 0xffffffffu;
  uint32_t x[8], y[8];
  fe_tobytes(x, P.X); fe_tobytes(y, P.Y);
  for (int j = 0; j < 8; j++) { dst[2 + j] = x[j]; dst[10 + j] = y[j]; }
}

__global__ void __launch_bounds__(64) fdgpu_test_sha512_kernel(const uint8_t *arena, const fdgpu_sig_desc_t *msgs, uint32_t n,
                                         uint32_t *out) {
  const uint32_t i = blockIdx.x * blockDim.x + threadIdx.x;
  const bool active = i < n;
  const fdgpu_sig_desc_t d = msgs[active ? i : n - 1];
  uint32_t nb = (d.msg_sz + 16u) / 128u + 1u;
  for (int off = 32; off > 0; off >>= 1) nb = max(nb, (uint32_t)__shfl_xor((int)nb, off));
  uint64_t h[8];
  sha512_plain(h, arena + d.msg_off, d.msg_sz, nb);
  if (!active) return;
  for (int j = 0; j < 8; j++) {
    out[16 * i + 2 * j] = bswap32((uint32_t)(h[j] >> 32));
    out[16 * i + 2 * j + 1] = bswap32((uint32_t)h[j]);
  }
}

__global__ void __launch_bounds__(64) fdgpu_test_hram_kernel(const uint8_t *arena, const fdgpu_sig_desc_t *sigs, uint32_t n,
                                       uint32_t *out) {
  const uint32_t i = blockIdx.x * blockDim.x + threadIdx.x;
  const bool active = i < n;
  const fdgpu_sig_desc_t d = sigs[active ? i : n - 1];
  const uint32_t nb = wave_max_u32(sha512_hram_blocks(d.msg_sz));
  uint32_t R[8], A[8], k[8];
  load32(R, arena + d.sig_off);
  load32(A, arena + d.pub_off);
  hram_k(k, R, A, arena, d, nb);
  if (!active) return;
  for (int j = 0; j < 8; j++) out[8 * i + j] = k[j];
}

__global__ void __launch_bounds__(64) fdgpu_test_sc_reduce_kernel(const uint32_t *in, uint32_t *out, uint32_t n) {
  const uint32_t i = blockIdx.x * blockDim.x + threadIdx.x;
  if (i >= n) return;
  uint32_t x[16], r[8];
  for (int j = 0; j < 16; j++) x[j] = in[16 * i + j];
  sc_reduce512(r, x);
  for (int j = 0; j < 8; j++) out[8 * i + j] = r[j];
}

__global__ void __launch_bounds__(64) fdgpu_test_hs_split_kernel(const uint32_t *in, uint32_t *out, uint32_t n) {
  const uint32_t i = blockIdx.x * blockDim.x + threadIdx.x;
  uint32_t k[8];
  for (int j = 0; j < 8; j++) k[j] = i < n ? in[8 * i + j] : 0u;
  hs_split_t o;
  hs_split(o, k);
  if (i >= n) return;
  uint32_t *w = out + 16 * (size_t)i;
  for (int j = 0; j < 5; j++) { w[j] = o.u[j]; w[5 + j] = o.v[j]; }
  w[10] = o.ok; w[11] = o.u_neg; w[12] = o.v_neg; w[13] = o.bits; w[14] = 0u; w[15] = 0u;
}

FDG_DEV void put_fe(uint32_t *dst, const fe &f) {
  uint32_t o[8];
  fe_tobytes(o, f);
#pragma unroll
  for (int j = 0; j < 8; j++) dst[j] = o[j];
}

__global__ void __launch_bounds__(64) fdgpu_test_fe_raw_kernel(const uint32_t *in, uint32_t *out, uint32_t n) {
  const uint32_t i = blockIdx.x * blockDim.x + threadIdx.x;
  if (i >= n) return;
  fe f, g, r, s;
#pragma unroll
  for (int j = 0; j < 10; j++) { f.v[j] = in[20 * (size_t)i + j]; g.v[j] = in[20 * (size_t)i + 10 + j]; }
  uint32_t *dst = out + 80 * (size_t)i;
  fe_mul(r, f, g);  put_fe(dst, r);
  fe_sq(r, f);      put_fe(dst + 8, r);
  fe_add(r, f, g);  put_fe(dst + 16, r);
  fe_sub(s, f, g);  put_fe(dst + 24, s);
  fe_mul(r, s, g);  put_fe(dst + 32, r);
  fe_neg(s, f);     put_fe(dst + 40, s);
  fe_mul(r, s, g);  put_fe(dst + 48, r);
  put_fe(dst + 56, f);
  fe_sub4(s, f, g); put_fe(dst + 64, s);
  fe_mul(r, s, g);  put_fe(dst + 72, r);
}

FDG_DEV void get_fe(fe &h, const uint32_t *src) {
  uint32_t w[8];
#pragma unroll
  for (int j = 0; j < 8; j++) w[j] = src[j];
  fe_frombytes(h, w);
}
FDG_DEV void put_p3(uint32_t *dst, const ge_p3 &p) {
  put_fe(dst, p.X); put_fe(dst + 8, p.Y); put_fe(dst + 16, p.Z); put_fe(dst + 24, p.T);
}
FDG_DEV void put_p2(uint32_t *dst, const ge_p2 &p) {
  put_fe(dst, p.X); put_fe(dst + 8, p.Y); put_fe(dst + 16, p.Z);
#pragma unroll
  for (int j = 0; j < 8; j++) dst[24 + j] = 0u;
}
FDG_DEV void put_p1p1(uint32_t *dst, const ge_p1p1 &t) {
  ge_p3 r;
  ge_p1p1_to_p3(r, t);
  put_p3(dst, r);
}

#define GE_IN_WORDS  88u
#define GE_RESULTS   21u
#define GE_OUT_WORDS (GE_RESULTS * 32u)

__global__ void __launch_bounds__(64) fdgpu_test_ge_kernel(const uint32_t *in, uint32_t *out, uint32_t n) {
  const uint32_t i = blockIdx.x * blockDim.x + threadIdx.x;
  if (i >= n) return;
  const uint32_t *src = in + GE_IN_WORDS * (size_t)i;
  uint32_t *dst = out + GE_OUT_WORDS * (size_t)i;
  ge_p3 P, Q;
  get_fe(P.X, src); get_fe(P.Y, src + 8); get_fe(P.Z, src + 16); get_fe(P.T, src + 24);
  get_fe(Q.X, src + 32); get_fe(Q.Y, src + 40); get_fe(Q.Z, src + 48); get_fe(Q.T, src + 56);
  ge_niels N;
  get_fe(N.ypx, src + 64); get_fe(N.ymx, src + 72); get_fe(N.xy2d, src + 80);
  ge_cached C;
  ge_p3_to_cached(C, Q);
  uint32_t qc[40], qn[32];
#pragma unroll
  for (int w = 0; w < 10; w++) {
    qc[w] = C.YpX.v[w]; qc[10 + w] = C.YmX.v[w]; qc[20 + w] = C.Z2.v[w]; qc[30 + w] = C.T2d.v[w];
    qn[w] = N.ypx.v[w]; qn[10 + w] = N.ymx.v[w]; qn[20 + w] = N.xy2d.v[w];
  }
  qn[30] = 0u; qn[31] = 0u;

  ge_p1p1 t;
  ge_p2 a2;
  ge_p3 r3;
  ge_p3_to_p2(a2, P);
  ge_dbl(t, a2);
  put_p1p1(dst, t);
  ge_p1p1_to_p2(a2, t);
  put_p2(dst + 32, a2);

  auto ldc = [&C](int c, int w) { return c == 0 ? C.YpX.v[w] : c == 1 ? C.YmX.v[w] : c == 2 ? C.Z2.v[w] : C.T2d.v[w]; };
#pragma unroll 1
  for (int s = 0; s < 2; s++) {
    const bool neg = s != 0;
    uint32_t *d = dst + 32 * s;
    ge_add_cached(t, P, C, neg);          put_p1p1(d + 32 * 2, t);
    ge_add_cached_ld(t, P, ldc, neg);     put_p1p1(d + 32 * 4, t);
    ge_add_cached_regs(t, P, qc, neg);    put_p1p1(d + 32 * 6, t);
    uint32_t qs[40];
#pragma unroll
    for (int w = 0; w < 10; w++) {
      qs[w] = neg ? qc[10 + w] : qc[w]; qs[10 + w] = neg ? qc[w] : qc[10 + w]; qs[20 + w] = qc[20 + w]; qs[30 + w] = qc[30 + w];
    }
    ge_add_cached_regs_swapped(t, P, qs, neg); put_p1p1(d + 32 * 8, t);
    ge_add_niels(t, P, N, neg);           put_p1p1(d + 32 * 10, t);
    ge_add_niels_regs(t, P, qn, neg);     put_p1p1(d + 32 * 12, t);
    ge_cached_regs_to_p2(a2, qc, neg);    put_p2(d + 32 * 14, a2);
    ge_niels_regs_to_p3(r3, qn, neg);     put_p3(d + 32 * 16, r3);

    ge_p3_to_p2(a2, P);
#pragma unroll 1
    for (int k = 0; k < 4; k++) { ge_dbl(t, a2); ge_p1p1_to_p2(a2, t); }
    r3.X = a2.X; r3.Y = a2.Y; r3.Z = a2.Z; fe_mul(r3.T, t.X, t.Y);
    ge_add_cached_regs_swapped(t, r3, qc, false);
    ge_p1p1_to_p3(r3, t);
    ge_add_cached_regs_swapped(t, r3, qs, neg);
    put_p1p1(d + 32 * 19, t);
  }
  ge_p3_neg(r3, P);
  put_p3(dst + 32 * 18, r3);
}

__global__ void __launch_bounds__(64) fdgpu_test_sc_recode_kernel(const uint32_t *in, uint32_t *out, uint32_t n) {
  const uint32_t i = blockIdx.x * blockDim.x + threadIdx.x;
  if (i >= n) return;
  constexpr int NW = COMB_WORDS(FDGPU_BCOMB_BITS, FDGPU_BCOMB_NDIG);
  static_assert(NW <= 8, "the record holds 8 words of comb digits");
  uint32_t s[8], d16[8], dc[NW];
  for (int j = 0; j < 8; j++) s[j] = in[8 * (size_t)i + j];
  sc_recode16(d16, s);
  sc_recode_comb<(int)FDGPU_BCOMB_BITS, (int)FDGPU_BCOMB_NDIG>(dc, s);
  uint32_t *w = out + 16 * (size_t)i;
  for (int j = 0; j < 8; j++) { w[j] = d16[j]; w[8 + j] = j < NW ? dc[j] : 0u; }
}

__global__ void __launch_bounds__(64) fdgpu_test_tabpack_kernel(const uint32_t *in, uint32_t *out, uint32_t n) {
  __shared__ uint32_t s_stage[FDGPU_STAGE_WAVE_WORDS];
  const uint32_t i = blockIdx.x * blockDim.x + threadIdx.x;
  if (i >= n) return;
  const uint32_t *src = in + FDGPU_ATAB_WORDS * (size_t)i;
  uint32_t *dst = out + FDGPU_TABPACK_OUT_WORDS * (size_t)i;
  ge_cached c;
#pragma unroll
  for (int w = 0; w < 10; w++) { c.YpX.v[w] = src[w]; c.YmX.v[w] = src[10 + w]; c.Z2.v[w] = src[20 + w]; c.T2d.v[w] = src[30 + w]; }
  uint32_t *tab = dst - FDGPU_PTAB_WORDS;
  atab_store(tab, 1, c);
  __threadfence();
  uint32_t q[40];
  atab_load(q, tab, 1);
#pragma unroll
  for (int w = 0; w < 40; w++) dst[32 + w] = q[w];
  stage_entry(s_stage, tab, 1);
  asm volatile("s_waitcnt vmcnt(0)" ::: "memory");
  unstage_entry_signed(q, s_stage, false);
#pragma unroll
  for (int w = 0; w < 40; w++) dst[72 + w] = q[w];
  unstage_entry_signed(q, s_stage, true);
#pragma unroll
  for (int w = 0; w < 40; w++) dst[112 + w] = q[w];
}

}

extern "C" {

hipError_t fdgpu_launch_test_fe(const uint32_t *d_in, uint32_t *d_out, uint32_t n, hipStream_t stream) {
  hipLaunchKernelGGL(fdgpu_test_fe_kernel, dim3((n + 63) / 64), dim3(64), 0, stream, d_in, d_out, n);
  return hipGetLastError();
}
hipError_t fdgpu_launch_test_decode(const uint32_t *d_enc, uint32_t *d_out, uint32_t n, uint32_t flags,
                                    hipStream_t stream) {
  hipLaunchKernelGGL(fdgpu_test_decode_kernel, dim3((n + 63) / 64), dim3(64), 0, stream, d_enc, d_out, n, flags);
  return hipGetLastError();
}
hipError_t fdgpu_launch_test_sha512(const uint8_t *d_arena, const fdgpu_sig_desc_t *d_msgs, uint32_t n,
                                    uint32_t *d_out, hipStream_t stream) {
  hipLaunchKernelGGL(fdgpu_test_sha512_kernel, dim3((n + 63) / 64), dim3(64), 0, stream, d_arena, d_msgs, n, d_out);
  return hipGetLastError();
}
hipError_t fdgpu_launch_test_hram(const uint8_t *d_arena, const fdgpu_sig_desc_t *d_sigs, uint32_t n,
                                  uint32_t *d_out, hipStream_t stream) {
  hipLaunchKernelGGL(fdgpu_test_hram_kernel, dim3((n + 63) / 64), dim3(64), 0, stream, d_arena, d_sigs, n, d_out);
  return hipGetLastError();
}
hipError_t fdgpu_launch_test_sc_reduce(const uint32_t *d_in, uint32_t *d_out, uint32_t n, hipStream_t stream) {
  hipLaunchKernelGGL(fdgpu_test_sc_reduce_kernel, dim3((n + 63) / 64), dim3(64), 0, stream, d_in, d_out, n);
  return hipGetLastError();
}
hipError_t fdgpu_launch_test_hs_split(const uint32_t *d_in, uint32_t *d_out, uint32_t n, hipStream_t stream) {
  hipLaunchKernelGGL(fdgpu_test_hs_split_kernel, dim3((n + 63) / 64), dim3(64), 0, stream, d_in, d_out, n);
  return hipGetLastError();
}
hipError_t fdgpu_launch_test_fe_raw(const uint32_t *d_in, uint32_t *d_out, uint32_t n, hipStream_t stream) {
  hipLaunchKernelGGL(fdgpu_test_fe_raw_kernel, dim3((n + 63) / 64), dim3(64), 0, stream, d_in, d_out, n);
  return hipGetLastError();
}
uint32_t fdgpu_test_ge_in_words(void) { return GE_IN_WORDS; }
uint32_t fdgpu_test_ge_results(void) { return GE_RESULTS; }
hipError_t fdgpu_launch_test_ge(const uint32_t *d_in, uint32_t *d_out, uint32_t n, hipStream_t stream) {
  hipLaunchKernelGGL(fdgpu_test_ge_kernel, dim3((n + 63) / 64), dim3(64), 0, stream, d_in, d_out, n);
  return hipGetLastError();
}
hipError_t fdgpu_launch_test_sc_recode(const uint32_t *d_in, uint32_t *d_out, uint32_t n, hipStream_t stream) {
  hipLaunchKernelGGL(fdgpu_test_sc_recode_kernel, dim3((n + 63) / 64), dim3(64), 0, stream, d_in, d_out, n);
  return hipGetLastError();
}
hipError_t fdgpu_launch_test_tabpack(const uint32_t *d_in, uint32_t *d_out, uint32_t n, hipStream_t stream) {
  hipLaunchKernelGGL(fdgpu_test_tabpack_kernel, dim3((n + 63) / 64), dim3(64), 0, stream, d_in, d_out, n);
  return hipGetLastError();
}

}
```

### firedancer_amd/csrc/fdgpu_verify.hip

```cpp
#include <hip/hip_runtime.h>

#include "fdgpu_atab.h"
#include "fdgpu_bcomb.h"
#include "fdgpu_ge.h"
#include "fdgpu_hram.h"
#include "fdgpu_internal.h"
#include "fdgpu_lattice.h"
#include "fdgpu_sc.h"
#include "fdgpu_sha512.h"
#include "fdgpu_stamps.h"

using namespace fdgpu;

namespace {


FDG_DEV uint32_t *tab_a(uint32_t *wsl) { return wsl - FDGPU_PTAB_WORDS; }
FDG_DEV const uint32_t *tab_a(const uint32_t *wsl) { return wsl - FDGPU_PTAB_WORDS; }
FDG_DEV uint32_t *tab_r(uint32_t *wsl) { return wsl + (FDGPU_WS_RTAB - 1u) * FDGPU_PTAB_WORDS; }

FDG_DEV void sb_store(uint32_t *aux, const ge_cached &c) {
  uint4 *p = (uint4 *)(aux + FDGPU_AUX_SB);
  uint32_t w[40];
#pragma unroll
  for (int i = 0; i < 10; i++) { w[i] = c.YpX.v[i]; w[10 + i] = c.YmX.v[i]; w[20 + i] = c.Z2.v[i]; w[30 + i] = c.T2d.v[i]; }
#pragma unroll
  for (int q = 0; q < 10; q++) p[q] = make_uint4(w[4 * q], w[4 * q + 1], w[4 * q + 2], w[4 * q + 3]);
}
FDG_DEV void sb_load(uint32_t (&q)[40], const uint32_t *aux) {
  const uint4 *ent = (const uint4 *)(aux + FDGPU_AUX_SB);
#pragma unroll
  for (int i = 0; i < 10; i++) {
    const uint4 v = ent[i];
    q[4 * i] = v.x; q[4 * i + 1] = v.y; q[4 * i + 2] = v.z; q[4 * i + 3] = v.w;
  }
}
FDG_DEV int sext4(uint32_t x) { return ((int)(x << 28)) >> 28; }

#define KD_WORDS 8

FDG_DEV void shl4(uint32_t (&w)[8]) {
#pragma unroll
  for (int i = 7; i > 0; i--) w[i] = (w[i] << 4) | (w[i - 1] >> 28);
  w[0] <<= 4;
}

FDG_DEV void dsm_k(ge_p2 &acc2, uint32_t (&kd)[KD_WORDS], const uint32_t *aux, const uint32_t *ta) {
  ge_p3 acc3;
  ge_p1p1 t;
  uint32_t q[40];
  {
    const int e = sext4(kd[7] >> 28);
    shl4(kd);
    atab_load(q, ta, e);
    ge_cached_regs_to_p2(acc2, q, e < 0);
  }
#pragma unroll 1
  for (int j = 62; j >= 0; j--) {
    const int e = sext4(kd[7] >> 28);
    shl4(kd);
    atab_load(q, ta, e);
#pragma unroll 1
    for (int r = 0; r < 4; r++) {
      ge_dbl(t, acc2);
      ge_p1p1_to_p2(acc2, t);
    }
    acc3.X = acc2.X; acc3.Y = acc2.Y; acc3.Z = acc2.Z; fe_mul(acc3.T, t.X, t.Y);
    ge_add_cached_regs(t, acc3, q, e < 0);
    if (j == 0) break;
    ge_p1p1_to_p2(acc2, t);
  }
  ge_p1p1_to_p3(acc3, t);
  uint32_t qs[40];
  sb_load(qs, aux);
  ge_add_cached_regs(t, acc3, qs, false);
  ge_p1p1_to_p2(acc2, t);
}

FDG_DEV void comb_sb(ge_p3 &acc, const uint32_t (&S)[8], const uint32_t *__restrict__ btab, uint32_t lo = 0,
                     uint32_t hi = BC_NDIG) {
  constexpr int NW = COMB_WORDS(BC_W, BC_NDIG), SLOT = COMB_SLOT(BC_W);
  uint32_t dg[NW];
  sc_recode_comb<(int)BC_W, (int)BC_NDIG>(dg, S);
  auto next_digit = [&dg]() {
    const int d = SLOT == 16 ? (int)(int16_t)(dg[0] & 0xffffu) : (int)dg[0];
#pragma unroll
    for (int i = 0; i < NW - 1; i++) dg[i] = SLOT == 16 ? (dg[i] >> 16) | (dg[i + 1] << 16) : dg[i + 1];
    dg[NW - 1] = SLOT == 16 ? dg[NW - 1] >> 16 : 0u;
    return d;
  };
  auto load_entry = [btab](uint32_t (&q)[32], uint32_t ti, int d) {
    const uint4 *ent = (const uint4 *)(btab + ((size_t)ti * BC_ENT + (uint32_t)(d < 0 ? -d : d)) * FDGPU_BCOMB_STRIDE);
#pragma unroll
    for (int i = 0; i < 8; i++) {
      const uint4 v = ent[i];
      q[4 * i] = v.x; q[4 * i + 1] = v.y; q[4 * i + 2] = v.z; q[4 * i + 3] = v.w;
    }
  };
  uint32_t qa[32], qb[32];
#pragma unroll 1
  for (uint32_t i = 0; i < lo; i++) (void)next_digit();
  int d = next_digit();
  load_entry(qa, lo, d);
  {
    const int dn = next_digit();
    load_entry(qb, lo + 1, dn);
    ge_niels_regs_to_p3(acc, qa, d < 0);
#pragma unroll
    for (int w = 0; w < 32; w++) qa[w] = qb[w];
    d = dn;
  }
  ge_p1p1 t;
#pragma unroll 1
  for (uint32_t i = lo + 1; i < hi; i++) {
    const int dn = next_digit();
    if (i + 1 < hi) load_entry(qb, i + 1, dn);
    ge_add_niels_regs(t, acc, qa, d < 0);
    ge_p1p1_to_p3(acc, t);
#pragma unroll
    for (int w = 0; w < 32; w++) qa[w] = qb[w];
    d = dn;
  }
}

FDG_DEV void atab_build(uint32_t *wsl, const ge_p3 &An) {
  ge_cached c;
  ge_p3_to_cached(c, An); atab_store(wsl, 1, c);
  ge_p1p1 t; ge_p2 a2; ge_p3 P;
  ge_p3_to_p2(a2, An); ge_dbl(t, a2); ge_p1p1_to_p3(P, t);
  ge_p3_to_cached(c, P); atab_store(wsl, 2, c);
  const uint32_t *ent1 = wsl + 1u * FDGPU_PTAB_WORDS;
  auto ld1 = [ent1](int cc, int w) { return atab_limb(ent1, cc, w); };
#pragma unroll 1
  for (uint32_t e = 3; e < FDGPU_ATAB_ENTRIES; e++) {
    if (e & 1u) {
      ge_add_cached_ld(t, P, ld1, false);
    } else {
      uint32_t q[40];
      atab_load(q, wsl, (int)(e >> 1));
      ge_cached_regs_to_p2(a2, q, false);
      ge_dbl(t, a2);
    }
    ge_p1p1_to_p3(P, t);
    ge_p3_to_cached(c, P); atab_store(wsl, e, c);
  }
}

FDG_DEV uint32_t *lane_ws(uint32_t *ws, uint32_t i) {
  return ws + (size_t)i * FDGPU_WS_TAB_WORDS;
}
FDG_DEV uint32_t *lane_aux(uint32_t *queue, uint32_t i) {
  return queue - ((size_t)i + 1u) * FDGPU_WS_AUX_WORDS;
}
FDG_DEV const uint32_t *lane_aux(const uint32_t *queue, uint32_t i) {
  return queue - ((size_t)i + 1u) * FDGPU_WS_AUX_WORDS;
}

FDG_DEV uint32_t out_idx(const uint32_t *__restrict__ perm, uint32_t i) { return perm ? perm[i] : i; }


#define HPARK_KD 0
#define HPARK_CODE 30
static_assert(HPARK_KD + KD_WORDS <= HPARK_CODE && HPARK_CODE < (int)FDGPU_AUX_SB - (int)FDGPU_AUX_PARK &&
              FDGPU_AUX_SB + FDGPU_ATAB_WORDS <= FDGPU_WS_AUX_WORDS && FDGPU_AUX_SB % 4u == 0 && FDGPU_WS_AUX_WORDS % 4u == 0,
              "aux layout");

FDG_DEV void recode16_160(uint32_t (&out)[5], uint32_t &nd, const uint32_t (&m)[5]) {
  uint32_t carry = 0;
  nd = 0;
#pragma unroll
  for (int w = 0; w < 5; w++) {
    uint32_t o = 0;
#pragma unroll
    for (int n = 0; n < 8; n++) {
      uint32_t e = ((m[w] >> (4 * n)) & 15u) + carry;
      carry = e >= 8u;
      e = (e - (carry << 4)) & 15u;
      o |= e << (4 * n);
      nd = e ? (uint32_t)(8 * w + n + 1) : nd;
    }
    out[w] = o;
  }
  nd = carry ? 41u : nd;
}

FDG_DEV void shl4_5(uint32_t (&w)[5]) {
#pragma unroll
  for (int i = 4; i > 0; i--) w[i] = (w[i] << 4) | (w[i - 1] >> 28);
  w[0] <<= 4;
}

FDG_DEV void hs_wscalar(uint32_t (&w)[8], const uint32_t (&v)[5], bool v_neg, const uint32_t (&S)[8]) {
  uint32_t x[16];
#pragma unroll
  for (int i = 0; i < 16; i++) x[i] = 0;
#pragma unroll
  for (int i = 0; i < 5; i++) {
    uint64_t c = 0;
#pragma unroll
    for (int j = 0; j < 8; j++) {
      const uint64_t t = (uint64_t)v[i] * S[j] + x[i + j] + c;
      x[i + j] = (uint32_t)t;
      c = t >> 32;
    }
    x[i + 8] = (uint32_t)c;
  }
  uint32_t r[8];
  sc_reduce512(r, x);
  constexpr uint32_t L[8] = FDGPU_SC_L;
  uint32_t nz = 0;
#pragma unroll
  for (int i = 0; i < 8; i++) nz |= r[i];
  const bool flip = v_neg && nz != 0;
  uint32_t bw = 0;
#pragma unroll
  for (int i = 0; i < 8; i++) {
    const uint64_t d = (uint64_t)L[i] - r[i] - bw;
    w[i] = flip ? (uint32_t)d : r[i];
    bw = (uint32_t)(d >> 63);
  }
}

FDG_DEV void hs_chain(ge_p1p1 &t, uint32_t (&ud)[5], uint32_t (&vd)[5], bool u_neg, bool v_neg, uint32_t nwin,
                      const uint32_t *wsl, const uint32_t *ta) {
  const uint32_t *tr = tab_r(const_cast<uint32_t *>(wsl));
  __shared__ uint32_t s_stage[FDGPU_BLOCK / 64][2][FDGPU_STAGE_WAVE_WORDS];
  static_assert(sizeof(s_stage) == FDGPU_STAGE_LDS, "FDGPU_SPREAD_LDS is derived from this");
  uint32_t *st_r = &s_stage[threadIdx.x >> 6][0][0];
  uint32_t *st_a = &s_stage[threadIdx.x >> 6][1][0];
  ge_p2 acc2;
  ge_p3 acc3;
  uint32_t q[40];
  {
    const int du = sext4(ud[4] >> 28), dv = sext4(vd[4] >> 28);
    shl4_5(ud); shl4_5(vd);
    atab_load(q, ta, du);
    ge_p3_0(acc3);
    ge_add_cached_regs(t, acc3, q, (du < 0) != u_neg);
    ge_p1p1_to_p3(acc3, t);
    atab_load(q, tr, dv);
    ge_add_cached_regs(t, acc3, q, (dv < 0) != v_neg);
  }
#pragma unroll 1
  for (uint32_t j = 1; j < nwin; j++) {
    ge_p1p1_to_p2(acc2, t);
    const int du = sext4(ud[4] >> 28), dv = sext4(vd[4] >> 28);
    shl4_5(ud); shl4_5(vd);
    stage_entry(st_a, ta, du);
    stage_entry(st_r, tr, dv);
#pragma unroll 1
    for (int r = 0; r < 4; r++) {
      ge_dbl(t, acc2);
      ge_p1p1_to_p2(acc2, t);
    }
    acc3.X = acc2.X; acc3.Y = acc2.Y; acc3.Z = acc2.Z; fe_mul(acc3.T, t.X, t.Y);
    asm volatile("s_waitcnt vmcnt(0)" ::: "memory");
    unstage_entry_signed(q, st_a, (du < 0) != u_neg);
    ge_add_cached_regs_swapped(t, acc3, q, (du < 0) != u_neg);
    ge_p1p1_to_p3(acc3, t);
    unstage_entry_signed(q, st_r, (dv < 0) != v_neg);
    ge_add_cached_regs_swapped(t, acc3, q, (dv < 0) != v_neg);
  }
}


FDG_DEV uint32_t decode_neg_table(uint32_t *tab, const uint32_t (&enc)[8], bool ref_map) {
  ge_p3 P, Pn;
  const bool ok = ge_decode(P, enc, ref_map);
  const bool small = ge_is_small_order_affine(P);
  ge_p3_neg(Pn, P);
  atab_build(tab, Pn);
  return (ok ? 1u : 0u) | (small ? 2u : 0u);
}

FDG_DEV void hs_split_masked(hs_split_t &hs, const uint32_t (&k)[8], bool need) {
  uint32_t ke[8];
#pragma unroll
  for (int j = 0; j < 8; j++) ke[j] = need ? k[j] : 0u;
  hs_split(hs, ke);
}

FDG_DEV uint32_t hs_digits(uint32_t (&ud)[5], uint32_t (&vd)[5], const hs_split_t &hs) {
  uint32_t ndu = 0, ndv = 0;
  recode16_160(ud, ndu, hs.u);
  recode16_160(vd, ndv, hs.v);
  return max(max(ndu, ndv), 1u);
}

FDG_DEV void comb_scalar(uint32_t (&w)[8], const hs_split_t &hs, const uint32_t (&S)[8], bool half) {
  hs_wscalar(w, hs.v, hs.v_neg, S);
#pragma unroll
  for (int j = 0; j < 8; j++) w[j] = half ? w[j] : S[j];
}

FDG_DEV void park_full(uint32_t *park, const uint32_t (&k)[8]) {
  uint32_t kd[KD_WORDS];
  sc_recode16(kd, k);
#pragma unroll
  for (int j = 0; j < KD_WORDS; j++) park[HPARK_KD + j] = kd[j];
  park[HPARK_CODE] = 0u;
}

FDG_DEV void queue_full_lanes(uint32_t *queue, uint32_t *queue_cnt, bool q_full, uint32_t i) {
  const uint64_t m = __ballot(q_full);
  if (m) {
    const int lane = (int)(threadIdx.x & 63u);
    const int leader = __ffsll((long long)m) - 1;
    uint32_t base = 0;
    if (lane == leader) base = atomicAdd(queue_cnt, (uint32_t)__popcll(m));
    base = (uint32_t)__shfl((int)base, leader, 64);
    if (q_full) queue[base + (uint32_t)__popcll(m & ((1ull << lane) - 1ull))] = i;
  }
}

template <bool KC, bool PH = false>
FDG_DEV void verify_hs_body(const uint8_t *__restrict__ arena, const fdgpu_sig_desc_t *__restrict__ sigs, uint32_t n_sig_arg,
                            const uint32_t *__restrict__ n_sig_dev, const uint32_t *__restrict__ btab,
                            uint32_t *__restrict__ ws, const uint32_t *__restrict__ perm, int8_t *__restrict__ codes,
                            uint32_t *__restrict__ queue, uint32_t *__restrict__ queue_cnt, uint32_t flags,
                            const uint32_t *__restrict__ key_of, const uint32_t *__restrict__ kverd, uint32_t bx) {
  const uint32_t n_sig = n_sig_dev ? *n_sig_dev : n_sig_arg;
  if (bx * blockDim.x >= n_sig) return;
  const uint32_t i = bx * blockDim.x + threadIdx.x;
  const bool active = i < n_sig;
  const bool ref_map = (flags & FDGPU_FLAG_REF_MAP) != 0;
  const fdgpu_sig_desc_t d = sigs[active ? i : n_sig - 1];
  uint32_t nb = sha512_hram_blocks(d.msg_sz);
#pragma unroll
  for (int off = 32; off > 0; off >>= 1) nb = max(nb, (uint32_t)__shfl_xor((int)nb, off));
  uint32_t *wsl = lane_ws(ws, i);
  uint32_t *aux = lane_aux(queue, i);
  const uint32_t *ta = tab_a(wsl);
  FDGPU_STAMP(0);
  uint32_t Renc[8], Aenc[8];
  load32(Renc, arena + d.sig_off);
  load32(Aenc, arena + d.pub_off);
  uint32_t k[8];
  {
    uint64_t h[8];
    if (PH) {
#pragma unroll
      for (int j = 0; j < 8; j++) h[j] = ((const uint64_t *)(arena + d.msg_off))[j];
    } else {
      sha512_hram(h, Renc, Aenc, arena + d.msg_off, d.msg_sz, nb);
    }
    FDGPU_STAMP(1);
    uint32_t kx[16];
#pragma unroll
    for (int j = 0; j < 8; j++) { kx[2 * j] = bswap32((uint32_t)(h[j] >> 32)); kx[2 * j + 1] = bswap32((uint32_t)h[j]); }
    sc_reduce512(k, kx);
  }
  uint32_t S[8];
  load32(S, arena + d.sig_off + 32);
  int code = sc_lt_L(S) ? 0 : -1;
#pragma unroll
  for (int j = 0; j < 8; j++) S[j] = code ? 0u : S[j];
  FDGPU_STAMP(2);
  {
    ge_p3 P, Pn;
    bool a_ok, a_small;
    if (KC) {
      const uint32_t di = active ? i : n_sig - 1u, r = key_of[di], vd = kverd[r];
      a_ok = (vd & 1u) != 0;
      a_small = (vd & 2u) != 0;
      ta = tab_a(lane_ws(ws, r));
    } else {
      a_ok = ge_decode(P, Aenc, ref_map);
      a_small = ge_is_small_order_affine(P);
      ge_p3_neg(Pn, P);
      atab_build(tab_a(wsl), Pn);
    }
    FDGPU_STAMP(3);
    const bool r_ok = ge_decode(P, Renc, ref_map);
    const bool r_small = ge_is_small_order_affine(P);
    ge_p3_neg(Pn, P);
    atab_build(tab_r(wsl), Pn);
    if (code == 0 && !a_ok) code = ref_map ? -2 : -1;
    if (code == 0 && !r_ok) code = -1;
    if (code == 0 && a_small) code = -2;
    if (code == 0 && r_small) code = -1;
  }
  FDGPU_STAMP(4);
  const bool need = active && code == 0;
  hs_split_t hs;
  hs_split_masked(hs, k, need);
  uint32_t ud[5], vd[5];
  const uint32_t nd_lane = hs_digits(ud, vd, hs);
  const bool full = need && (!hs.ok || nd_lane > HS_MAX_WIN || (flags & FDGPU_FLAG_KFULL));
  const bool half = need && !full;
  FDGPU_STAMP(5);
  {
    uint32_t w[8];
    comb_scalar(w, hs, S, half);
    ge_p3 WB;
    comb_sb(WB, w, btab);
    ge_cached c; ge_p3_to_cached(c, WB);
    sb_store(aux, c);
  }
  if (full) park_full(aux + FDGPU_AUX_PARK, k);
  FDGPU_STAMP(6);
  bool eq = false;
  if (__any(half)) {
    const uint32_t nwin = wave_max_u32(half ? nd_lane : 1u);
#pragma unroll 1
    for (uint32_t s = nwin; s < 40; s++) { shl4_5(ud); shl4_5(vd); }
    ge_p1p1 t;
    hs_chain(t, ud, vd, hs.u_neg, hs.v_neg, nwin, wsl, ta);
    uint32_t q[40];
    sb_load(q, aux);
    fe ypx, ymx, z2, xw, yw, l1, l2;
#pragma unroll
    for (int j = 0; j < 10; j++) { ypx.v[j] = q[j]; ymx.v[j] = q[10 + j]; z2.v[j] = q[20 + j]; }
    fe_sub(xw, ypx, ymx);
    fe_add(yw, ypx, ymx);
    fe_mul(l1, t.X, z2);
    fe_mul(l2, t.Z, xw);
    fe_add(l1, l1, l2);
    const bool ex = fe_iszero(l1);
    fe_mul(l1, t.Y, z2);
    fe_mul(l2, t.T, yw);
    fe_sub(l1, l1, l2);
    eq = ex && fe_iszero(l1);
  }
  FDGPU_STAMP(7);
  if (active && !full) codes[out_idx(perm, i)] = (int8_t)(code ? code : (eq ? 0 : -3));
  queue_full_lanes(queue, queue_cnt, full, i);
}

template <bool KC, bool PH = false>
__global__ void __launch_bounds__(FDGPU_BLOCK, FDGPU_VERIFY_WAVES)
fdgpu_verify_hs_kernel(const uint8_t *__restrict__ arena, const fdgpu_sig_desc_t *__restrict__ sigs, uint32_t n_sig_arg,
                       const uint32_t *__restrict__ n_sig_dev, const uint32_t *__restrict__ btab,
                       uint32_t *__restrict__ ws, const uint32_t *__restrict__ perm, int8_t *__restrict__ codes,
                       uint32_t *__restrict__ queue, uint32_t *__restrict__ queue_cnt, uint32_t flags,
                       const uint32_t *__restrict__ key_of, const uint32_t *__restrict__ kverd) {
  verify_hs_body<KC, PH>(arena, sigs, n_sig_arg, n_sig_dev, btab, ws, perm, codes, queue, queue_cnt, flags, key_of,
                         kverd, blockIdx.x);
}

__global__ void __launch_bounds__(64) fdgpu_sha512_stream_kernel(const uint8_t *__restrict__ mbuf, uint64_t m0,
                                                                 uint64_t mlen, uint64_t msg_sz, uint64_t blk0,
                                                                 uint32_t nblk, const uint8_t *__restrict__ ra,
                                                                 uint64_t *__restrict__ state, uint32_t n) {
  const uint32_t i = threadIdx.x;
  if (i >= n) return;
  const uint64_t H0[8] = {0x6a09e667f3bcc908ULL, 0xbb67ae8584caa73bULL, 0x3c6ef372fe94f82bULL,
                          0xa54ff53a5f1d36f1ULL, 0x510e527fade682d1ULL, 0x9b05688c2b3e6c1fULL,
                          0x1f83d9abfb41bd6bULL, 0x5be0cd19137e2179ULL};
  uint64_t h[8];
  for (int j = 0; j < 8; j++) h[j] = blk0 ? state[8 * i + j] : H0[j];
  const uint64_t total = (64u + msg_sz + 16u) / 128u + 1u, bitlen = (64u + msg_sz) * 8u;
  for (uint64_t b = blk0; b < blk0 + nblk; b++) {
    uint64_t w[16];
    for (int t = 0; t < 16; t++) {
      uint64_t v = 0;
      for (int j = 0; j < 8; j++) {
        const uint64_t s = 128u * b + 8u * (uint64_t)t + (uint64_t)j;
        uint32_t byte;
        if (s < 64u) {
          byte = ra[64u * i + s];
        } else {
          const uint64_t g = s - 64u;
          byte = g < msg_sz ? (g >= m0 && g < m0 + mlen ? mbuf[g - m0] : 0u) : g == msg_sz ? 0x80u : 0u;
        }
        v = (v << 8) | byte;
      }
      w[t] = v;
    }
    if (b + 1 == total) { w[14] = 0; w[15] = bitlen; }
    sha512_compress(h, w);
  }
  for (int j = 0; j < 8; j++) state[8 * i + j] = h[j];
}

__global__ void __launch_bounds__(FDGPU_BLOCK, FDGPU_VERIFY_WAVES)
fdgpu_verify_hs_multi_kernel(const fdgpu_mbatch_t *__restrict__ mb, const uint32_t *__restrict__ btab, uint32_t flags) {
  const fdgpu_mbatch_t b = mb[blockIdx.y];
  if (blockIdx.x * blockDim.x >= b.bound) return;
  verify_hs_body<false>(b.arena, b.sigs, b.bound, b.n_sig, btab, b.ws, nullptr, b.codes, b.queue, b.cnt, flags, nullptr,
                        nullptr, blockIdx.x);
}


FDG_DEV void hs_chain1(ge_p1p1 &t, uint32_t (&dd)[5], bool neg, uint32_t nwin, const uint32_t *tab) {
  __shared__ uint32_t s_stage1[FDGPU_BLOCK / 64][FDGPU_STAGE_WAVE_WORDS];
  static_assert(sizeof(s_stage1) == FDGPU_STAGE_LDS_PAIR, "FDGPU_SPREAD_LDS_PAIR is derived from this");
  uint32_t *st = &s_stage1[threadIdx.x >> 6][0];
  ge_p2 acc2;
  ge_p3 acc3;
  uint32_t q[40];
  {
    const int d = sext4(dd[4] >> 28);
    shl4_5(dd);
    atab_load(q, tab, d);
    ge_p3_0(acc3);
    ge_add_cached_regs(t, acc3, q, (d < 0) != neg);
  }
#pragma unroll 1
  for (uint32_t j = 1; j < nwin; j++) {
    ge_p1p1_to_p2(acc2, t);
    const int d = sext4(dd[4] >> 28);
    shl4_5(dd);
    stage_entry(st, tab, d);
#pragma unroll 1
    for (int r = 0; r < 4; r++) {
      ge_dbl(t, acc2);
      ge_p1p1_to_p2(acc2, t);
    }
    acc3.X = acc2.X; acc3.Y = acc2.Y; acc3.Z = acc2.Z; fe_mul(acc3.T, t.X, t.Y);
    asm volatile("s_waitcnt vmcnt(0)" ::: "memory");
    unstage_entry_signed(q, st, (d < 0) != neg);
    ge_add_cached_regs_swapped(t, acc3, q, (d < 0) != neg);
  }
}

FDG_DEV void fe_xchg_pair(fe &r, const fe &a) {
#pragma unroll
  for (int j = 0; j < 10; j++) r.v[j] = (uint32_t)__shfl_xor((int)a.v[j], 1);
}

template <bool PH = false>
__global__ void __launch_bounds__(FDGPU_BLOCK, FDGPU_VERIFY_WAVES)
fdgpu_verify_pair_kernel(const uint8_t *__restrict__ arena, const fdgpu_sig_desc_t *__restrict__ sigs, uint32_t n_sig_arg,
                         const uint32_t *__restrict__ n_sig_dev, const uint32_t *__restrict__ btab,
                         uint32_t *__restrict__ ws, const uint32_t *__restrict__ perm, int8_t *__restrict__ codes,
                         uint32_t *__restrict__ queue, uint32_t *__restrict__ queue_cnt, uint32_t flags) {
  const uint32_t n_sig = n_sig_dev ? *n_sig_dev : n_sig_arg;
  if (blockIdx.x * (blockDim.x / 2u) >= n_sig) return;
  const uint32_t g = blockIdx.x * blockDim.x + threadIdx.x, i = g >> 1;
  const bool rl = (g & 1u) != 0;
  const bool active = i < n_sig;
  const bool ref_map = (flags & FDGPU_FLAG_REF_MAP) != 0;
  const fdgpu_sig_desc_t d = sigs[active ? i : n_sig - 1];
  const uint32_t nb = wave_max_u32(sha512_hram_blocks(d.msg_sz));
  uint32_t *wsl = lane_ws(ws, i);
  uint32_t *aux = lane_aux(queue, i);
  uint32_t *tab = rl ? tab_r(wsl) : tab_a(wsl);
  uint32_t Renc[8], Aenc[8];
  load32(Renc, arena + d.sig_off);
  load32(Aenc, arena + d.pub_off);
  uint32_t k[8];
  if (PH) {
    uint32_t kx[16];
#pragma unroll
    for (int j = 0; j < 8; j++) {
      const uint64_t h = ((const uint64_t *)(arena + d.msg_off))[j];
      kx[2 * j] = bswap32((uint32_t)(h >> 32)); kx[2 * j + 1] = bswap32((uint32_t)h);
    }
    sc_reduce512(k, kx);
  } else {
    hram_k(k, Renc, Aenc, arena, d, nb);
  }
  uint32_t S[8];
  load32(S, arena + d.sig_off + 32);
  int code = sc_lt_L(S) ? 0 : -1;
#pragma unroll
  for (int j = 0; j < 8; j++) S[j] = code ? 0u : S[j];
  {
    uint32_t enc[8];
#pragma unroll
    for (int j = 0; j < 8; j++) enc[j] = rl ? Renc[j] : Aenc[j];
    const uint32_t mine = decode_neg_table(tab, enc, ref_map);
    const uint32_t other = (uint32_t)__shfl_xor((int)mine, 1);
    const uint32_t av = rl ? other : mine, rv = rl ? mine : other;
    if (code == 0 && !(av & 1u)) code = ref_map ? -2 : -1;
    if (code == 0 && !(rv & 1u)) code = -1;
    if (code == 0 && (av & 2u)) code = -2;
    if (code == 0 && (rv & 2u)) code = -1;
  }
  const bool need = active && code == 0;
  hs_split_t hs;
  hs_split_masked(hs, k, need);
  uint32_t ud[5], vd[5];
  const uint32_t nd_lane = hs_digits(ud, vd, hs);
  const bool full = need && (!hs.ok || nd_lane > HS_MAX_WIN || (flags & FDGPU_FLAG_KFULL));
  const bool half = need && !full;
  {
    uint32_t w[8];
    comb_scalar(w, hs, S, half);
    ge_p3 WB, WBo;
    comb_sb(WB, w, btab, rl ? BC_NDIG / 2u : 0u, rl ? BC_NDIG : BC_NDIG / 2u);
    fe_xchg_pair(WBo.X, WB.X);
    fe_xchg_pair(WBo.Y, WB.Y);
    fe_xchg_pair(WBo.Z, WB.Z);
    fe_xchg_pair(WBo.T, WB.T);
    ge_cached c; ge_p3_to_cached(c, WBo);
    ge_p1p1 tw; ge_add_cached(tw, WB, c, false);
    ge_p1p1_to_p3(WB, tw);
    ge_p3_to_cached(c, WB);
    if (!rl) sb_store(aux, c);
  }
  if (full && !rl) park_full(aux + FDGPU_AUX_PARK, k);
  bool eq = false;
  if (__any(half)) {
    const uint32_t nwin = wave_max_u32(half ? nd_lane : 1u);
    uint32_t dd[5];
#pragma unroll
    for (int j = 0; j < 5; j++) dd[j] = rl ? vd[j] : ud[j];
#pragma unroll 1
    for (uint32_t s2 = nwin; s2 < 40; s2++) shl4_5(dd);
    ge_p1p1 t;
    hs_chain1(t, dd, rl ? hs.v_neg : hs.u_neg, nwin, tab);
    ge_p3 mine, other;
    ge_p1p1_to_p3(mine, t);
    fe_xchg_pair(other.X, mine.X);
    fe_xchg_pair(other.Y, mine.Y);
    fe_xchg_pair(other.Z, mine.Z);
    fe_xchg_pair(other.T, mine.T);
    ge_cached oc;
    ge_p3_to_cached(oc, other);
    ge_add_cached(t, mine, oc, false);
    uint32_t q[40];
    sb_load(q, aux);
    fe ypx, ymx, z2, xw, yw, l1, l2;
#pragma unroll
    for (int j = 0; j < 10; j++) { ypx.v[j] = q[j]; ymx.v[j] = q[10 + j]; z2.v[j] = q[20 + j]; }
    fe_sub(xw, ypx, ymx);
    fe_add(yw, ypx, ymx);
    fe_mul(l1, t.X, z2);
    fe_mul(l2, t.Z, xw);
    fe_add(l1, l1, l2);
    const bool ex = fe_iszero(l1);
    fe_mul(l1, t.Y, z2);
    fe_mul(l2, t.T, yw);
    fe_sub(l1, l1, l2);
    eq = ex && fe_iszero(l1);
  }
  if (active && !full && !rl) codes[out_idx(perm, i)] = (int8_t)(code ? code : (eq ? 0 : -3));
  queue_full_lanes(queue, queue_cnt, full && !rl, i);
}

#define KC_PROBES 32u
#define KC_EMPTY 0xffffffffu

FDG_DEV uint32_t kc_hash(const uint32_t (&a)[8], uint64_t seed) {
  uint64_t h = seed;
#pragma unroll
  for (int j = 0; j < 4; j++) {
    h ^= ((uint64_t)a[2 * j + 1] << 32) | a[2 * j];
    h *= 0x9e3779b97f4a7c15ull;
    h ^= h >> 29;
  }
  h *= 0xbf58476d1ce4e5b9ull;
  return (uint32_t)(h >> 32) ^ (uint32_t)h;
}

__global__ void __launch_bounds__(256) fdgpu_key_dedup_kernel(const uint8_t *__restrict__ arena,
                                                              const fdgpu_sig_desc_t *__restrict__ sigs,
                                                              uint32_t n_sig_arg, const uint32_t *__restrict__ n_sig_dev,
                                                              uint32_t *__restrict__ ht, uint32_t ht_mask,
                                                              uint32_t *__restrict__ key_of, uint32_t *__restrict__ reps,
                                                              uint32_t *__restrict__ rep_cnt, uint64_t seed) {
  const uint32_t n_sig = n_sig_dev ? *n_sig_dev : n_sig_arg;
  if (blockIdx.x * blockDim.x >= n_sig) return;
  const uint32_t i = blockIdx.x * blockDim.x + threadIdx.x;
  bool is_rep = false;
  if (i < n_sig) {
    uint32_t a[8];
    load32(a, arena + sigs[i].pub_off);
    uint32_t slot = kc_hash(a, seed) & ht_mask, rep = i;
    for (uint32_t p = 0; p < KC_PROBES; p++, slot = (slot + 1u) & ht_mask) {
      uint32_t v = ht[slot];
      if (v == KC_EMPTY) {
        v = atomicCAS(&ht[slot], KC_EMPTY, i);
        if (v == KC_EMPTY) break;
      }
      uint32_t b[8];
      load32(b, arena + sigs[v].pub_off);
      uint32_t diff = 0;
#pragma unroll
      for (int j = 0; j < 8; j++) diff |= a[j] ^ b[j];
      if (!diff) { rep = v; break; }
    }
    key_of[i] = rep;
    is_rep = rep == i;
  }
  __shared__ uint32_t s_cnt, s_base;
  if (threadIdx.x == 0) s_cnt = 0;
  __syncthreads();
  const uint64_t m = __ballot(is_rep);
  const int lane = (int)(threadIdx.x & 63u);
  uint32_t wbase = 0;
  if (m && lane == __ffsll((long long)m) - 1) wbase = atomicAdd(&s_cnt, (uint32_t)__popcll(m));
  if (m) wbase = (uint32_t)__shfl((int)wbase, __ffsll((long long)m) - 1, 64);
  __syncthreads();
  if (threadIdx.x == 0) s_base = s_cnt ? atomicAdd(rep_cnt, s_cnt) : 0u;
  __syncthreads();
  if (is_rep) reps[s_base + wbase + (uint32_t)__popcll(m & ((1ull << lane) - 1ull))] = i;
}

__global__ void __launch_bounds__(FDGPU_BLOCK, FDGPU_VERIFY_WAVES)
fdgpu_key_table_kernel(const uint8_t *__restrict__ arena, const fdgpu_sig_desc_t *__restrict__ sigs,
                       uint32_t *__restrict__ ws, const uint32_t *__restrict__ reps,
                       const uint32_t *__restrict__ rep_cnt, uint32_t *__restrict__ kverd, uint32_t flags) {
  const uint32_t q = blockIdx.x * blockDim.x + threadIdx.x;
  if (q >= *rep_cnt) return;
  const uint32_t i = reps[q];
  uint32_t Aenc[8];
  load32(Aenc, arena + sigs[i].pub_off);
  kverd[i] = decode_neg_table(tab_a(lane_ws(ws, i)), Aenc, (flags & FDGPU_FLAG_REF_MAP) != 0);
}

__global__ void __launch_bounds__(FDGPU_BLOCK, FDGPU_VERIFY_WAVES)
fdgpu_full_kernel(uint32_t *__restrict__ ws, const uint32_t *__restrict__ perm, int8_t *__restrict__ codes,
                  const uint32_t *__restrict__ queue, const uint32_t *__restrict__ queue_cnt, uint32_t slots,
                  const uint32_t *__restrict__ key_of);

FDG_DEV void full_body(uint32_t *__restrict__ ws, const uint32_t *__restrict__ perm, int8_t *__restrict__ codes,
                       const uint32_t *__restrict__ queue, const uint32_t *__restrict__ queue_cnt, uint32_t slots,
                       const uint32_t *__restrict__ key_of, uint32_t bx) {
  const uint32_t cnt = *queue_cnt;
  if (bx * blockDim.x >= cnt) return;
  for (uint32_t q = bx * blockDim.x + threadIdx.x; q < cnt; q += slots) {
    const uint32_t i = queue[q];
    uint32_t *wsl = lane_ws(ws, i);
    const uint32_t *aux = lane_aux(queue, i), *park = aux + FDGPU_AUX_PARK;
    uint32_t kd[KD_WORDS];
#pragma unroll
    for (int j = 0; j < KD_WORDS; j++) kd[j] = park[HPARK_KD + j];
    ge_p2 Rc;
    dsm_k(Rc, kd, aux, tab_a(key_of ? lane_ws(ws, key_of[i]) : wsl));
    uint32_t er[40];
    atab_load(er, tab_r(wsl), 1);
    fe ypx, ymx, z2, x2, y2, l, r;
#pragma unroll
    for (int j = 0; j < 10; j++) { ypx.v[j] = er[j]; ymx.v[j] = er[10 + j]; z2.v[j] = er[20 + j]; }
    fe_carry(ypx); fe_carry(ymx); fe_carry(z2);
    fe_sub(x2, ymx, ypx);
    fe_add(y2, ypx, ymx);
    fe_mul(l, Rc.X, z2); fe_mul(r, x2, Rc.Z);
    bool eq = fe_eq(l, r);
    fe_mul(l, Rc.Y, z2); fe_mul(r, y2, Rc.Z);
    eq = eq && fe_eq(l, r);
    codes[out_idx(perm, i)] = (int8_t)(eq ? 0 : -3);
  }
}

__global__ void __launch_bounds__(FDGPU_BLOCK, FDGPU_VERIFY_WAVES)
fdgpu_full_kernel(uint32_t *__restrict__ ws, const uint32_t *__restrict__ perm, int8_t *__restrict__ codes,
                  const uint32_t *__restrict__ queue, const uint32_t *__restrict__ queue_cnt, uint32_t slots,
                  const uint32_t *__restrict__ key_of) {
  full_body(ws, perm, codes, queue, queue_cnt, slots, key_of, blockIdx.x);
}

__global__ void __launch_bounds__(FDGPU_BLOCK, FDGPU_VERIFY_WAVES)
fdgpu_full_multi_kernel(const fdgpu_mbatch_t *__restrict__ mb) {
  const fdgpu_mbatch_t b = mb[blockIdx.y];
  if (blockIdx.x >= b.slow) return;
  full_body(b.ws, nullptr, b.codes, b.queue, b.cnt, b.slow * FDGPU_BLOCK, nullptr, blockIdx.x);
}

__global__ void __launch_bounds__(256) fdgpu_combine_kernel(const fdgpu_txn_desc_t *__restrict__ txns, uint32_t n_txn,
                                                            const int8_t *__restrict__ sig_codes,
                                                            int8_t *__restrict__ txn_codes,
                                                            uint64_t *__restrict__ accept) {
  for (uint32_t t0 = blockIdx.x * blockDim.x; t0 < n_txn; t0 += gridDim.x * blockDim.x) {
    const uint32_t t = t0 + threadIdx.x;
    int code = -1;
    if (t < n_txn) {
      const fdgpu_txn_desc_t d = txns[t];
      if (d.sig_cnt >= 1 && d.sig_cnt <= 16) {
        int first_struct = 0, any_msg = 0;
        for (uint32_t j = 0; j < d.sig_cnt; j++) {
          const int c = sig_codes[d.sig0 + j];
          if (c == -3) any_msg = 1;
          else if (c != 0 && first_struct == 0) first_struct = c;
        }
        code = first_struct ? first_struct : (any_msg ? -3 : 0);
      }
      txn_codes[t] = (int8_t)code;
    }
    const uint64_t ok = __ballot(t < n_txn && code == 0);
    if (accept && (threadIdx.x & 63u) == 0 && t < n_txn) accept[t >> 6] = ok;
  }
}

}

extern "C" {

char const *fdgpu_kernel_path(void) { return "halfsize: fdgpu_verify_hs_kernel + fdgpu_full_kernel"; }

int fdgpu_kernel_build_info(char *buf, size_t n) {
  snprintf(buf, n, "\"verify_waves\":%d,\"atab_words\":%u,\"phase_stamps\":%d", (int)FDGPU_VERIFY_WAVES,
           (unsigned)FDGPU_ATAB_WORDS, (int)FDGPU_PHASE_STAMPS);
  return FDGPU_VERIFY_WAVES == 2 && FDGPU_ATAB_WORDS == 40u && FDGPU_PHASE_STAMPS == 0;
}

hipError_t fdgpu_verify_occupancy(int *blocks_per_cu) {
  return hipOccupancyMaxActiveBlocksPerMultiprocessor(blocks_per_cu, fdgpu_verify_hs_kernel<false>, FDGPU_BLOCK, 0);
}

size_t fdgpu_ws_bytes(uint64_t n_sig) { return fdgpu_ws_layout(nullptr, n_sig).bytes; }

hipError_t fdgpu_launch_verify_sigs(const uint8_t *d_arena, const fdgpu_sig_desc_t *d_sigs, uint32_t n_sig,
                                    const uint32_t *d_perm, const uint32_t *d_btab, uint32_t *d_ws,
                                    int8_t *d_sig_codes, uint32_t flags, hipStream_t stream, const uint32_t *d_n_sig,
                                    uint32_t resident_blocks, uint64_t kc_seed, int cnt_zeroed) {
  if (!n_sig) return hipSuccess;
  const uint32_t grid = (n_sig + FDGPU_BLOCK - 1) / FDGPU_BLOCK;
  const fdgpu_ws_layout_t l = fdgpu_ws_layout(d_ws, n_sig);
  hipError_t e = cnt_zeroed ? hipSuccess : hipMemsetAsync(l.cnt, 0, sizeof(uint32_t), stream);
  if (e != hipSuccess) return e;
  if (!resident_blocks) resident_blocks = 1;
  uint32_t slow_blocks = grid < resident_blocks ? grid : resident_blocks;
  const uint32_t slow_cap = grid > 64u ? FDGPU_FULL_BLOCKS : FDGPU_FULL_BLOCKS / 4u;
  if (slow_blocks > slow_cap) slow_blocks = slow_cap;
  const uint32_t *key_of = nullptr;
  if (flags & FDGPU_FLAG_KCACHE) {
    e = hipMemsetAsync(l.ht, 0xff, l.ht_slots * sizeof(uint32_t), stream);
    if (e == hipSuccess) e = hipMemsetAsync(l.rep_cnt, 0, sizeof(uint32_t), stream);
    if (e != hipSuccess) return e;
    hipLaunchKernelGGL(fdgpu_key_dedup_kernel, dim3((n_sig + 255) / 256), dim3(256), 0, stream, d_arena, d_sigs, n_sig,
                       d_n_sig, l.ht, (uint32_t)(l.ht_slots - 1), l.key_of, l.reps, l.rep_cnt, kc_seed);
    hipLaunchKernelGGL(fdgpu_key_table_kernel, dim3(grid), dim3(FDGPU_BLOCK), 0, stream, d_arena, d_sigs, d_ws, l.reps,
                       l.rep_cnt, l.kverd, flags);
    hipLaunchKernelGGL(fdgpu_verify_hs_kernel<true>, dim3(grid), dim3(FDGPU_BLOCK), 0, stream, d_arena, d_sigs, n_sig,
                       d_n_sig, d_btab, d_ws, d_perm, d_sig_codes, l.queue, l.cnt, flags, l.key_of, l.kverd);
    key_of = l.key_of;
  } else if (flags & FDGPU_FLAG_KPAIR) {
    const uint32_t pgrid = (2u * n_sig + FDGPU_BLOCK - 1) / FDGPU_BLOCK;
    hipLaunchKernelGGL(fdgpu_verify_pair_kernel<false>, dim3(pgrid), dim3(FDGPU_BLOCK),
                       (flags & FDGPU_FLAG_KSPREAD) ? FDGPU_SPREAD_LDS_PAIR : 0, stream, d_arena, d_sigs, n_sig,
                       d_n_sig, d_btab, d_ws, d_perm, d_sig_codes, l.queue, l.cnt, flags);
  } else {
    hipLaunchKernelGGL(fdgpu_verify_hs_kernel<false>, dim3(grid), dim3(FDGPU_BLOCK),
                       (flags & FDGPU_FLAG_KSPREAD) ? FDGPU_SPREAD_LDS : 0, stream, d_arena, d_sigs, n_sig,
                       d_n_sig, d_btab, d_ws, d_perm, d_sig_codes, l.queue, l.cnt, flags, nullptr, nullptr);
  }
  hipLaunchKernelGGL(fdgpu_full_kernel, dim3(slow_blocks), dim3(FDGPU_BLOCK), 0, stream, d_ws, d_perm, d_sig_codes,
                     l.queue, l.cnt, slow_blocks * FDGPU_BLOCK, key_of);
  return hipGetLastError();
}

uint64_t fdgpu_sha512_stream_blocks(uint64_t msg_sz) { return (64u + msg_sz + 16u) / 128u + 1u; }

hipError_t fdgpu_launch_sha512_stream(const uint8_t *d_mbuf, uint64_t m0, uint64_t mlen, uint64_t msg_sz,
                                      uint64_t blk0, uint32_t nblk, const uint8_t *d_ra, uint64_t *d_state,
                                      uint32_t n, hipStream_t stream) {
  if (!n || n > 64 || !nblk) return hipErrorInvalidValue;
  hipLaunchKernelGGL(fdgpu_sha512_stream_kernel, dim3(1), dim3(64), 0, stream, d_mbuf, m0, mlen, msg_sz, blk0, nblk,
                     d_ra, d_state, n);
  return hipGetLastError();
}

hipError_t fdgpu_launch_verify_prehashed(const uint8_t *d_arena, const fdgpu_sig_desc_t *d_sigs, uint32_t n_sig,
                                         const uint32_t *d_btab, uint32_t *d_ws, int8_t *d_sig_codes, uint32_t flags,
                                         hipStream_t stream) {
  if (!n_sig) return hipSuccess;
  const uint32_t grid = (n_sig + FDGPU_BLOCK - 1) / FDGPU_BLOCK;
  const fdgpu_ws_layout_t l = fdgpu_ws_layout(d_ws, n_sig);
  hipError_t e = hipMemsetAsync(l.cnt, 0, sizeof(uint32_t), stream);
  if (e != hipSuccess) return e;
  const uint32_t kf = flags & (FDGPU_FLAG_REF_MAP | FDGPU_FLAG_KFULL);
  if (flags & FDGPU_FLAG_KPAIR) {
    const uint32_t pgrid = (2u * n_sig + FDGPU_BLOCK - 1) / FDGPU_BLOCK;
    hipLaunchKernelGGL(fdgpu_verify_pair_kernel<true>, dim3(pgrid), dim3(FDGPU_BLOCK), 0, stream, d_arena, d_sigs,
                       n_sig, nullptr, d_btab, d_ws, nullptr, d_sig_codes, l.queue, l.cnt, kf);
  } else {
    hipLaunchKernelGGL((fdgpu_verify_hs_kernel<false, true>), dim3(grid), dim3(FDGPU_BLOCK), 0, stream, d_arena, d_sigs,
                       n_sig, nullptr, d_btab, d_ws, nullptr, d_sig_codes, l.queue, l.cnt, kf, nullptr, nullptr);
  }
  hipLaunchKernelGGL(fdgpu_full_kernel, dim3(1), dim3(FDGPU_BLOCK), 0, stream, d_ws, nullptr, d_sig_codes, l.queue,
                     l.cnt, FDGPU_BLOCK, nullptr);
  return hipGetLastError();
}

hipError_t fdgpu_launch_verify_multi(const fdgpu_mbatch_t *mb, uint32_t nb, uint32_t grid_max, uint32_t slow_max,
                                     const uint32_t *d_btab, uint32_t flags, hipStream_t stream) {
  if (!nb || !grid_max) return hipSuccess;
  hipLaunchKernelGGL(fdgpu_verify_hs_multi_kernel, dim3(grid_max, nb), dim3(FDGPU_BLOCK), 0, stream, mb, d_btab, flags);
  hipLaunchKernelGGL(fdgpu_full_multi_kernel, dim3(slow_max ? slow_max : 1, nb), dim3(FDGPU_BLOCK), 0, stream, mb);
  return hipGetLastError();
}

hipError_t fdgpu_launch_combine(const fdgpu_txn_desc_t *d_txns, uint32_t n_txn, const int8_t *d_sig_codes,
                                int8_t *d_txn_codes, uint64_t *d_accept, hipStream_t stream) {
  if (!n_txn) return hipSuccess;
  const uint32_t blocks = (n_txn + 255) / 256;
  hipLaunchKernelGGL(fdgpu_combine_kernel, dim3(blocks < FDGPU_AUX_BLOCKS ? blocks : FDGPU_AUX_BLOCKS), dim3(256), 0,
                     stream, d_txns, n_txn, d_sig_codes, d_txn_codes, d_accept);
  return hipGetLastError();
}

#if FDGPU_PHASE_STAMPS
int fdgpu_debug_stamps(uint64_t *out, uint64_t n_waves) {
  if (n_waves > FDGPU_STAMP_WAVES) n_waves = FDGPU_STAMP_WAVES;
  return hipMemcpyFromSymbol(out, HIP_SYMBOL(g_fdgpu_stamps), n_waves * FDGPU_STAMP_SLOTS * sizeof(uint64_t)) ==
                 hipSuccess ? 0 : -1;
}
#endif

}
```

### firedancer_amd/ed25519.py

```python
import ctypes

import numpy as np

from . import _lib

SUCCESS, ERR_SIG, ERR_PUBKEY, ERR_MSG = 0, -1, -2, -3

FLAG_REF_MAPPING = 1
FLAG_NO_BUCKET = 2
FLAG_FULL_PATH = 4
FLAG_KEY_CACHE = 8
FLAG_PAIR = 16
FLAG_PAIR_AUTO = 32
FLAG_MERGE = 64
FLAG_SPREAD = 128
FLAG_SPREAD_AUTO = 256

TXN_DTYPE = np.dtype([("msg_off", "<u4"), ("msg_sz", "<u4"), ("sig_off", "<u4"),
                      ("pub_off", "<u4"), ("sig_cnt", "<u4")])
SIG_DESC_DTYPE = np.dtype([("msg_off", "<u4"), ("msg_sz", "<u4"), ("sig_off", "<u4"), ("pub_off", "<u4")])
TXN_DESC_DTYPE = np.dtype([("sig0", "<u4"), ("sig_cnt", "<u4")])
KFLAG_REF_MAP, KFLAG_FULL, KFLAG_PAIR = 1, 2, 8
ARENA_SLACK = 160
SHRED_DTYPE = np.dtype([("off", "<u4"), ("sz", "<u4"), ("pub_off", "<u4")])
CODE_SHRED_REJECT = -67
SHRED_SZ_MAX = 1228 + 4
SET_SHRED_DTYPE = np.dtype([("off", "<u4"), ("sz", "<u4"), ("pub_off", "<u4"), ("known_off", "<u4")])
SHRED_NO_ROOT = 0xFFFFFFFF
CODE_SHRED_ROOT_MISMATCH = -74
POH_DTYPE = np.dtype([("hash_cnt", "<u8"), ("prev_off", "<u4"), ("hash_off", "<u4"), ("sig_first", "<u4"),
                      ("sig_cnt", "<u4"), ("mix_off", "<u4"), ("_pad", "<u4")])
POH_NO_MIX = 0xFFFFFFFF
POH_HASH_CNT_MAX = 1 << 20
CODE_POH_MISMATCH = -68
CODE_POH_TOO_LONG = -69
PRECOMPILE_DTYPE = np.dtype([("off", "<u4"), ("sz", "<u4"), ("sig_cap", "<u4")])
PRECOMPILE_INFO_DTYPE = np.dtype([("instr_idx", "<u2"), ("rec_idx", "<u2"), ("ed_instr_cnt", "<u2"), ("sig_cnt", "<u2"),
                                  ("ed_code", "i1"), ("_pad", "u1", (7,))])
PRECOMPILE_WALK_DTYPE = np.dtype([("sig0", "<u4"), ("sig_cnt", "<u2"), ("instr_idx", "<u2"), ("rec_idx", "<u2"),
                                  ("ed_instr_cnt", "<u2"), ("code", "i1"), ("_pad", "u1", (3,))])
CODE_PRECOMPILE_DATA_SIZE = -70
CODE_PRECOMPILE_DATA_OFFSET = -71
CODE_PRECOMPILE_SIGNATURE = -72
CODE_PRECOMPILE_CAP = -73


SECP256K1_FAIL_ON_BAD_COUNT = 1
SECP256K1_ERR_RECID = -1
SECP256K1_ERR_RANGE = -2
SECP256K1_ERR_POINT = -3
SECP256K1_ERR_INFINITY = -4
SECP256K1_ERR_ADDRESS = -5
SECP256K1_OPS_IN, SECP256K1_OPS_OUT = 49, 17


def secp256k1_sig_bound(sz):
    return int(_lib.lib().fdgpu_secp256k1_sig_bound(int(sz)))


def precompile_sig_bound(sz):
    return int(_lib.lib().fdgpu_precompile_sig_bound(int(sz)))


def poh_chunk():
    return int(_lib.lib().fdgpu_poh_chunk())


def bcomb_dims():
    L = _lib.lib()
    return {k: int(L.fdgpu_bcomb_dim(i)) for i, k in enumerate(("w", "ndig", "entries", "stride", "chunk"))}


def ge_ops_shape():
    L = _lib.lib()
    return int(L.fdgpu_test_ge_in_words()), int(L.fdgpu_test_ge_results())


def _poh_arrays(arena, entries, sig_offs):
    return (np.ascontiguousarray(arena, dtype=np.uint8), np.ascontiguousarray(entries, dtype=POH_DTYPE),
            np.ascontiguousarray(sig_offs, dtype=np.uint32))


def verify(msg, sig, public_key, sha=None):
    msg = bytes(msg)
    sig, public_key = bytes(sig), bytes(public_key)
    if len(sig) != 64 or len(public_key) != 32:
        raise ValueError("sig must be 64 bytes and public_key 32 bytes")
    return _lib.lib().fd_ed25519_verify(msg, len(msg), sig, public_key, None)


def verify_batch_single_msg(msg, signatures, pubkeys, shas, batch_sz):
    msg = bytes(msg)
    signatures, pubkeys = bytes(signatures), bytes(pubkeys)
    n = int(batch_sz)
    if n < 0 or n > 255:
        raise ValueError("batch_sz is a uchar")
    if 1 <= n <= 16 and (len(signatures) < 64 * n or len(pubkeys) < 32 * n):
        raise ValueError("signatures/pubkeys shorter than batch_sz records")
    return _lib.lib().fd_ed25519_verify_batch_single_msg(msg, len(msg), signatures, pubkeys, None, n)


def sync_stats():
    import ctypes as c
    v = [c.c_uint64() for _ in range(3)]
    _lib.lib().fdgpu_sync_stats(*[c.byref(x) for x in v])
    return {"calls": v[0].value, "batches": v[1].value, "errors": v[2].value}


def strerror(err):
    return _lib.lib().fd_ed25519_strerror(int(err)).decode()


def expand_txns(txns):
    txns = np.asarray(txns, dtype=TXN_DTYPE)
    cnt = txns["sig_cnt"].astype(np.int64)
    valid = (cnt >= 1) & (cnt <= 16)
    used = np.where(valid, cnt, 0)
    sig0 = np.zeros(len(txns), dtype=np.int64)
    if len(txns):
        sig0[1:] = np.cumsum(used)[:-1]
    n_sig = int(used.sum())
    tdesc = np.zeros(len(txns), dtype=TXN_DESC_DTYPE)
    tdesc["sig0"] = sig0
    tdesc["sig_cnt"] = used
    sdesc = np.zeros(n_sig, dtype=SIG_DESC_DTYPE)
    t_of_sig = np.repeat(np.arange(len(txns)), used)
    j = np.arange(n_sig) - sig0[t_of_sig]
    sdesc["msg_off"] = txns["msg_off"][t_of_sig]
    sdesc["msg_sz"] = txns["msg_sz"][t_of_sig]
    sdesc["sig_off"] = txns["sig_off"][t_of_sig] + 64 * j
    sdesc["pub_off"] = txns["pub_off"][t_of_sig] + 32 * j
    return sdesc, tdesc


class VerifyEngine:

    def __init__(self, device=0, max_txn=1 << 16, max_sig=None, max_arena=None, ring_depth=2, ref_mapping=False,
                 bucket=True, full_path=False, key_cache=False, pair=False, pair_auto=False, merge=False,
                 spread=False, spread_auto=False):
        L = _lib.lib()
        self.max_sig = max_sig or 12 * max_txn
        flags = ((FLAG_REF_MAPPING if ref_mapping else 0) | (0 if bucket else FLAG_NO_BUCKET) |
                 (FLAG_FULL_PATH if full_path else 0) | (FLAG_KEY_CACHE if key_cache else 0) |
                 (FLAG_PAIR if pair else 0) | (FLAG_PAIR_AUTO if pair_auto else 0) | (FLAG_MERGE if merge else 0) |
                 (FLAG_SPREAD if spread else 0) | (FLAG_SPREAD_AUTO if spread_auto else 0))
        cfg = _lib.FdgpuCfg(max_txn, self.max_sig, max_arena or 1232 * max_txn, ring_depth, flags)
        self._cfg = cfg
        self.max_arena = cfg.max_arena
        self._h = L.fdgpu_engine_open(int(device), ctypes.byref(cfg))
        if not self._h:
            raise RuntimeError(f"fdgpu_engine_open({device}) failed: {_lib.last_error()}")
        self.device = device
        self._pending = {}

    def reserve(self, n_sig=0):
        r = _lib.lib().fdgpu_engine_reserve(self._h, int(n_sig))
        if r:
            raise RuntimeError(f"fdgpu_engine_reserve failed: {r} ({_lib.last_error()})")

    def host_register(self, buf):
        arr = np.asarray(buf)
        r = _lib.lib().fdgpu_host_register(self._h, arr.ctypes.data, arr.nbytes)
        if r:
            raise RuntimeError(f"fdgpu_host_register failed: {r} ({_lib.last_error()})")

    def host_unregister(self, buf):
        r = _lib.lib().fdgpu_host_unregister(self._h, np.asarray(buf).ctypes.data)
        if r:
            raise RuntimeError(f"fdgpu_host_unregister failed: {r} ({_lib.last_error()})")

    def close(self):
        if self._h:
            _lib.lib().fdgpu_engine_close(self._h)
            self._h = None

    def __enter__(self):
        return self

    def __exit__(self, *a):
        self.close()

    def __del__(self):
        try:
            self.close()
        except Exception:
            pass

    def info(self):
        g, b, w = ctypes.c_uint32(), ctypes.c_uint32(), ctypes.c_uint64()
        _lib.lib().fdgpu_engine_info(self._h, ctypes.byref(g), ctypes.byref(b), ctypes.byref(w))
        return {"resident_blocks": g.value, "block_threads": b.value, "ws_bytes": w.value}

    def submit(self, arena, txns):
        arena = np.ascontiguousarray(arena, dtype=np.uint8)
        txns = np.ascontiguousarray(txns, dtype=TXN_DTYPE)
        tk = _lib.lib().fdgpu_submit(self._h, arena.ctypes.data, arena.size, txns.ctypes.data, len(txns))
        if tk < 0:
            raise RuntimeError(f"fdgpu_submit failed ({tk}): {_lib.last_error()}")
        self._pending[tk] = len(txns)
        return tk

    def poll(self, ticket, blocking=True):
        n = self._pending.get(ticket)
        if n is None:
            raise KeyError(ticket)
        out = np.zeros(max(n, 1), dtype=np.int8)
        rc = _lib.lib().fdgpu_poll(self._h, ticket, out.ctypes.data, 1 if blocking else 0)
        if rc == 1:
            return None
        if rc != 0:
            raise RuntimeError(f"fdgpu_poll failed ({rc}): {_lib.last_error()}")
        del self._pending[ticket]
        return out[:n]

    def verify_txns(self, arena, txns):
        return self.poll(self.submit(arena, txns), blocking=True)

    def submit_frags(self, arena, frags, trailer_sz):
        arena = np.ascontiguousarray(arena, dtype=np.uint8)
        frags = np.ascontiguousarray(frags, dtype=FRAG_EX_DTYPE)
        tk = _lib.lib().fdgpu_submit_frags(self._h, arena.ctypes.data, arena.size, frags.ctypes.data, len(frags),
                                           int(trailer_sz))
        if tk < 0:
            raise RuntimeError(f"fdgpu_submit_frags failed ({tk}): {_lib.last_error()}")
        self._pending[tk] = (len(frags), int(trailer_sz))
        return tk

    def poll_frags(self, ticket, blocking=True):
        n, tsz = self._pending[ticket]
        codes = np.zeros(max(n, 1), dtype=np.int8)
        tr = np.zeros(max(tsz, 1), dtype=np.uint8)
        rc = _lib.lib().fdgpu_poll_frags(self._h, ticket, codes.ctypes.data, tr.ctypes.data, 1 if blocking else 0)
        if rc == 1:
            return None
        if rc != 0:
            raise RuntimeError(f"fdgpu_poll_frags failed ({rc}): {_lib.last_error()}")
        del self._pending[ticket]
        return codes[:n], tr[:tsz]

    def submit_frags_io(self, frags, out, out_sz, hash_seed, links=None):
        frags = np.ascontiguousarray(frags, dtype=FRAG_IO_DTYPE)
        out = np.asarray(out)
        if out_sz > out.nbytes:
            raise ValueError("out_sz exceeds the out buffer")
        lk = np.array(list(links or []), dtype=LINK_DTYPE)
        tk = _lib.lib().fdgpu_submit_frags_io(self._h, frags.ctypes.data, len(frags), out.ctypes.data, int(out_sz),
                                              int(hash_seed), lk.ctypes.data if len(lk) else None, len(lk))
        if tk < 0:
            raise RuntimeError(f"fdgpu_submit_frags_io failed ({tk}): {_lib.last_error()}")
        self._pending[tk] = (len(frags), frags)
        return tk

    def poll_frags_io(self, ticket, blocking=True):
        n, _ = self._pending[ticket]
        codes = np.zeros(max(n, 1), dtype=np.int8)
        tags = np.zeros(max(n, 1), dtype=np.uint64)
        osz = np.zeros(max(n, 1), dtype=np.uint16)
        rc = _lib.lib().fdgpu_poll_frags_io(self._h, ticket, codes.ctypes.data, tags.ctypes.data, osz.ctypes.data,
                                            1 if blocking else 0)
        if rc == 1:
            return None
        if rc != 0:
            raise RuntimeError(f"fdgpu_poll_frags_io failed ({rc}): {_lib.last_error()}")
        del self._pending[ticket]
        return codes[:n], tags[:n], osz[:n]

    def submit_shreds(self, arena, shreds, expected_version):
        arena = np.ascontiguousarray(arena, dtype=np.uint8)
        shreds = np.ascontiguousarray(shreds, dtype=SHRED_DTYPE)
        tk = _lib.lib().fdgpu_submit_shreds(self._h, arena.ctypes.data, arena.size, shreds.ctypes.data, len(shreds),
                                            int(expected_version))
        if tk < 0:
            raise RuntimeError(f"fdgpu_submit_shreds failed ({tk}): {_lib.last_error()}")
        self._pending[tk] = len(shreds)
        return tk

    def poll_shreds(self, ticket, blocking=True):
        n = self._pending[ticket]
        codes = np.zeros(max(n, 1), dtype=np.int8)
        roots = np.zeros((max(n, 1), 32), dtype=np.uint8)
        rc = _lib.lib().fdgpu_poll_shreds(self._h, ticket, codes.ctypes.data, roots.ctypes.data, 1 if blocking else 0)
        if rc == 1:
            return None
        if rc != 0:
            raise RuntimeError(f"fdgpu_poll_shreds failed ({rc}): {_lib.last_error()}")
        del self._pending[ticket]
        return codes[:n], roots[:n]

    def verify_shreds(self, arena, shreds, expected_version):
        return self.poll_shreds(self.submit_shreds(arena, shreds, expected_version), blocking=True)

    def submit_shred_sets(self, arena, shreds, expected_version):
        arena = np.ascontiguousarray(arena, dtype=np.uint8)
        shreds = np.ascontiguousarray(shreds, dtype=SET_SHRED_DTYPE)
        tk = _lib.lib().fdgpu_submit_shred_sets(self._h, arena.ctypes.data, arena.size, shreds.ctypes.data, len(shreds),
                                                int(expected_version))
        if tk < 0:
            raise RuntimeError(f"fdgpu_submit_shred_sets failed ({tk}): {_lib.last_error()}")
        self._pending[tk] = len(shreds)
        return tk

    def poll_shred_sets(self, ticket, blocking=True, want_rep=True):
        n = self._pending[ticket]
        codes = np.zeros(max(n, 1), dtype=np.int8)
        roots = np.zeros((max(n, 1), 32), dtype=np.uint8)
        rep = np.zeros(max(n, 1), dtype=np.uint32) if want_rep else None
        lanes = ctypes.c_uint64(0)
        rc = _lib.lib().fdgpu_poll_shred_sets(self._h, ticket, codes.ctypes.data, roots.ctypes.data,
                                              rep.ctypes.data if want_rep else None,
                                              ctypes.byref(lanes) if want_rep else None, 1 if blocking else 0)
        if rc == 1:
            return None
        if rc != 0:
            raise RuntimeError(f"fdgpu_poll_shred_sets failed ({rc}): {_lib.last_error()}")
        del self._pending[ticket]
        return codes[:n], roots[:n], (rep[:n] if want_rep else None), (int(lanes.value) if want_rep else None)

    def verify_shred_sets(self, arena, shreds, expected_version):
        return self.poll_shred_sets(self.submit_shred_sets(arena, shreds, expected_version), blocking=True)

    def submit_precompiles(self, arena, txns):
        arena = np.ascontiguousarray(arena, dtype=np.uint8)
        txns = np.ascontiguousarray(txns, dtype=PRECOMPILE_DTYPE)
        tk = _lib.lib().fdgpu_submit_precompiles(self._h, arena.ctypes.data, arena.size, txns.ctypes.data, len(txns))
        if tk < 0:
            raise RuntimeError(f"fdgpu_submit_precompiles failed ({tk}): {_lib.last_error()}")
        self._pending[tk] = len(txns)
        return tk

    def poll_precompiles(self, ticket, blocking=True):
        n = self._pending[ticket]
        codes = np.zeros(max(n, 1), dtype=np.int8)
        info = np.zeros(max(n, 1), dtype=PRECOMPILE_INFO_DTYPE)
        rc = _lib.lib().fdgpu_poll_precompiles(self._h, ticket, codes.ctypes.data, info.ctypes.data,
                                               1 if blocking else 0)
        if rc == 1:
            return None
        if rc != 0:
            raise RuntimeError(f"fdgpu_poll_precompiles failed ({rc}): {_lib.last_error()}")
        del self._pending[ticket]
        return codes[:n], info[:n]

    def verify_precompiles(self, arena, txns):
        return self.poll_precompiles(self.submit_precompiles(arena, txns), blocking=True)

    def submit_secp256k1(self, arena, txns, flags=0):
        arena = np.ascontiguousarray(arena, dtype=np.uint8)
        txns = np.ascontiguousarray(txns, dtype=PRECOMPILE_DTYPE)
        tk = _lib.lib().fdgpu_submit_secp256k1(self._h, arena.ctypes.data, arena.size, txns.ctypes.data, len(txns),
                                               int(flags))
        if tk < 0:
            raise RuntimeError(f"fdgpu_submit_secp256k1 failed ({tk}): {_lib.last_error()}")
        self._pending[tk] = len(txns)
        return tk

    def poll_secp256k1(self, ticket, blocking=True):
        n = self._pending[ticket]
        codes = np.zeros(max(n, 1), dtype=np.int8)
        info = np.zeros(max(n, 1), dtype=PRECOMPILE_INFO_DTYPE)
        rc = _lib.lib().fdgpu_poll_secp256k1(self._h, ticket, codes.ctypes.data, info.ctypes.data, 1 if blocking else 0)
        if rc == 1:
            return None
        if rc != 0:
            raise RuntimeError(f"fdgpu_poll_secp256k1 failed ({rc}): {_lib.last_error()}")
        del self._pending[ticket]
        return codes[:n], info[:n]

    def verify_secp256k1(self, arena, txns, flags=0):
        return self.poll_secp256k1(self.submit_secp256k1(arena, txns, flags), blocking=True)

    def submit_poh(self, arena, entries, sig_offs, hash_cnt_cap):
        arena, entries, sig_offs = _poh_arrays(arena, entries, sig_offs)
        tk = _lib.lib().fdgpu_submit_poh(self._h, arena.ctypes.data, arena.size, entries.ctypes.data, len(entries),
                                         sig_offs.ctypes.data, len(sig_offs), int(hash_cnt_cap))
        if tk < 0:
            raise RuntimeError(f"fdgpu_submit_poh failed ({tk}): {_lib.last_error()}")
        self._pending[tk] = len(entries)
        return tk

    def poll_poh(self, ticket, blocking=True):
        n = self._pending[ticket]
        codes = np.zeros(max(n, 1), dtype=np.int8)
        hashes = np.zeros((max(n, 1), 32), dtype=np.uint8)
        rc = _lib.lib().fdgpu_poll_poh(self._h, ticket, codes.ctypes.data, hashes.ctypes.data, 1 if blocking else 0)
        if rc == 1:
            return None
        if rc != 0:
            raise RuntimeError(f"fdgpu_poll_poh failed ({rc}): {_lib.last_error()}")
        del self._pending[ticket]
        return codes[:n], hashes[:n]

    def verify_poh(self, arena, entries, sig_offs, hash_cnt_cap):
        return self.poll_poh(self.submit_poh(arena, entries, sig_offs, hash_cnt_cap), blocking=True)

    def verify_device(self, d_arena, d_sig_desc, n_sig, d_txn_desc, n_txn, d_sig_codes, d_txn_codes, stream=0):
        rc = _lib.lib().fdgpu_verify_device(self._h, d_arena, d_sig_desc, n_sig, d_txn_desc, n_txn,
                                            d_sig_codes, d_txn_codes, stream or None)
        if rc != 0:
            raise RuntimeError(f"fdgpu_verify_device failed ({rc}): {_lib.last_error()}")

    def upload(self, arena, txns):
        return DeviceBatch(self, arena, txns)

    def upload_frags(self, arena, frags):
        return FragBatch(self, arena, frags)

    def sync(self):
        self._chk(_lib.lib().fdgpu_sync(self._h), "fdgpu_sync")

    def _chk(self, rc, what):
        if rc != 0:
            raise RuntimeError(f"{what} failed ({rc}): {_lib.last_error()}")

    def debug_fe_ops(self, ab):
        ab = np.ascontiguousarray(ab, dtype=np.uint8).reshape(-1, 64)
        out = np.zeros((len(ab), 8, 32), dtype=np.uint8)
        self._chk(_lib.lib().fdgpu_debug_fe_ops(self._h, ab.ctypes.data, len(ab), out.ctypes.data), "debug_fe_ops")
        return out

    def debug_decode(self, enc, ref_mapping=False):
        enc = np.ascontiguousarray(enc, dtype=np.uint8).reshape(-1, 32)
        out = np.zeros((len(enc), 72), dtype=np.uint8)
        self._chk(_lib.lib().fdgpu_debug_decode(self._h, enc.ctypes.data, len(enc), 1 if ref_mapping else 0,
                                                out.ctypes.data), "debug_decode")
        rc = out[:, 0:4].copy().view(np.int32)[:, 0]
        so = out[:, 4:8].copy().view(np.int32)[:, 0]
        return rc, so, out[:, 8:40], out[:, 40:72]

    def debug_sha512(self, arena, txns):
        arena = np.ascontiguousarray(arena, dtype=np.uint8)
        txns = np.ascontiguousarray(txns, dtype=TXN_DTYPE)
        out = np.zeros((len(txns), 64), dtype=np.uint8)
        self._chk(_lib.lib().fdgpu_debug_sha512(self._h, arena.ctypes.data, arena.size, txns.ctypes.data, len(txns),
                                                out.ctypes.data), "debug_sha512")
        return out

    def debug_sha256(self, arena, txns):
        arena = np.ascontiguousarray(arena, dtype=np.uint8)
        txns = np.ascontiguousarray(txns, dtype=TXN_DTYPE)
        out = np.zeros((len(txns), 32), dtype=np.uint8)
        self._chk(_lib.lib().fdgpu_debug_sha256(self._h, arena.ctypes.data, arena.size, txns.ctypes.data, len(txns),
                                                out.ctypes.data), "debug_sha256")
        return out

    def debug_shred_roots(self, arena, shreds, expected_version):
        arena = np.ascontiguousarray(arena, dtype=np.uint8)
        shreds = np.ascontiguousarray(shreds, dtype=SHRED_DTYPE)
        ok = np.zeros(len(shreds), dtype=np.int8)
        roots = np.zeros((len(shreds), 32), dtype=np.uint8)
        self._chk(_lib.lib().fdgpu_debug_shred_roots(self._h, arena.ctypes.data, arena.size, shreds.ctypes.data,
                                                     len(shreds), int(expected_version), ok.ctypes.data,
                                                     roots.ctypes.data), "debug_shred_roots")
        return ok, roots

    def debug_shred_time(self, arena, shreds, expected_version, iters=5):
        arena = np.ascontiguousarray(arena, dtype=np.uint8)
        shreds = np.ascontiguousarray(shreds, dtype=SHRED_DTYPE)
        a, v = ctypes.c_double(), ctypes.c_double()
        self._chk(_lib.lib().fdgpu_debug_shred_time(self._h, arena.ctypes.data, arena.size, shreds.ctypes.data,
                                                    len(shreds), int(expected_version), int(iters), ctypes.byref(a),
                                                    ctypes.byref(v)), "debug_shred_time")
        return a.value, v.value

    def debug_shred_sets_time(self, arena, shreds, expected_version, iters=5):
        arena = np.ascontiguousarray(arena, dtype=np.uint8)
        shreds = np.ascontiguousarray(shreds, dtype=SET_SHRED_DTYPE)
        a, v = ctypes.c_double(), ctypes.c_double()
        self._chk(_lib.lib().fdgpu_debug_shred_sets_time(self._h, arena.ctypes.data, arena.size, shreds.ctypes.data,
                                                         len(shreds), int(expected_version), int(iters), ctypes.byref(a),
                                                         ctypes.byref(v)), "debug_shred_sets_time")
        return a.value, v.value

    def debug_precompile_walk(self, arena, txns):
        arena = np.ascontiguousarray(arena, dtype=np.uint8)
        txns = np.ascontiguousarray(txns, dtype=PRECOMPILE_DTYPE)
        cap = int(txns["sig_cap"].astype(np.uint64).sum())
        walk = np.zeros(len(txns), dtype=PRECOMPILE_WALK_DTYPE)
        descs = np.zeros(max(cap, 1), dtype=SIG_DESC_DTYPE)
        pos = np.zeros(max(cap, 1), dtype=np.uint32)
        k = ctypes.c_uint64()
        self._chk(_lib.lib().fdgpu_debug_precompile_walk(self._h, arena.ctypes.data, arena.size, txns.ctypes.data,
                                                         len(txns), walk.ctypes.data, descs.ctypes.data,
                                                         pos.ctypes.data, max(cap, 1), ctypes.byref(k)),
                  "debug_precompile_walk")
        return walk, descs[:k.value], pos[:k.value]

    def debug_precompile_time(self, arena, txns, iters=5):
        arena = np.ascontiguousarray(arena, dtype=np.uint8)
        txns = np.ascontiguousarray(txns, dtype=PRECOMPILE_DTYPE)
        a, v = ctypes.c_double(), ctypes.c_double()
        self._chk(_lib.lib().fdgpu_debug_precompile_time(self._h, arena.ctypes.data, arena.size, txns.ctypes.data,
                                                         len(txns), int(iters), ctypes.byref(a), ctypes.byref(v)),
                  "debug_precompile_time")
        return a.value, v.value

    def debug_secp256k1_walk(self, arena, txns, flags=0):
        arena = np.ascontiguousarray(arena, dtype=np.uint8)
        txns = np.ascontiguousarray(txns, dtype=PRECOMPILE_DTYPE)
        cap = int(txns["sig_cap"].astype(np.uint64).sum())
        walk = np.zeros(len(txns), dtype=PRECOMPILE_WALK_DTYPE)
        descs = np.zeros(max(cap, 1), dtype=SIG_DESC_DTYPE)
        pos = np.zeros(max(cap, 1), dtype=np.uint32)
        k = ctypes.c_uint64()
        self._chk(_lib.lib().fdgpu_debug_secp256k1_walk(self._h, arena.ctypes.data, arena.size, txns.ctypes.data,
                                                        len(txns), int(flags), walk.ctypes.data, descs.ctypes.data,
                                                        pos.ctypes.data, max(cap, 1), ctypes.byref(k)),
                  "debug_secp256k1_walk")
        return walk, descs[:k.value], pos[:k.value]

    def debug_keccak256(self, msgs):
        arena = np.frombuffer(b"".join(msgs) + b"\0", dtype=np.uint8)
        os_ = np.zeros((len(msgs), 2), dtype=np.uint32)
        at = 0
        for i, m in enumerate(msgs):
            os_[i] = (at, len(m))
            at += len(m)
        out = np.zeros((len(msgs), 32), dtype=np.uint8)
        self._chk(_lib.lib().fdgpu_debug_keccak256(self._h, arena.ctypes.data, arena.size - 1, os_.ctypes.data, len(msgs),
                                                   out.ctypes.data), "debug_keccak256")
        return out

    def debug_secp256k1_recover(self, items):
        buf = np.frombuffer(b"".join(bytes(h) + bytes(s) + bytes([r & 0xFF]) for h, s, r in items), dtype=np.uint8)
        if buf.size != 97 * len(items):
            raise ValueError("each item is 32 + 64 bytes and a recovery id")
        codes = np.zeros(len(items), dtype=np.int8)
        keys = np.zeros((len(items), 64), dtype=np.uint8)
        self._chk(_lib.lib().fdgpu_debug_secp256k1_recover(self._h, buf.ctypes.data, len(items), codes.ctypes.data,
                                                           keys.ctypes.data), "debug_secp256k1_recover")
        return codes, keys

    def debug_secp256k1_ops(self, items):
        buf = np.zeros((len(items), SECP256K1_OPS_IN), dtype=np.uint32)
        for i, it in enumerate(items):
            buf[i, 0] = it[0]
            for k, v in enumerate(it[1:]):
                buf[i, 1 + 8 * k:9 + 8 * k] = [(v >> (32 * j)) & 0xFFFFFFFF for j in range(8)]
        out = np.zeros((len(items), SECP256K1_OPS_OUT), dtype=np.uint32)
        self._chk(_lib.lib().fdgpu_debug_secp256k1_ops(self._h, buf.ctypes.data, len(items), out.ctypes.data),
                  "debug_secp256k1_ops")
        val = lambda w: sum(int(x) << (32 * j) for j, x in enumerate(w))
        return [(int(o[0]), val(o[1:9]), val(o[9:17])) for o in out]

    def debug_secp256k1_time(self, arena, txns, flags=0, iters=5):
        arena = np.ascontiguousarray(arena, dtype=np.uint8)
        txns = np.ascontiguousarray(txns, dtype=PRECOMPILE_DTYPE)
        a, v = ctypes.c_double(), ctypes.c_double()
        self._chk(_lib.lib().fdgpu_debug_secp256k1_time(self._h, arena.ctypes.data, arena.size, txns.ctypes.data,
                                                        len(txns), int(flags), int(iters), ctypes.byref(a),
                                                        ctypes.byref(v)), "debug_secp256k1_time")
        return a.value, v.value

    def debug_poh(self, arena, entries, sig_offs, hash_cnt_cap, grid_waves=0):
        arena, entries, sig_offs = _poh_arrays(arena, entries, sig_offs)
        codes = np.zeros(len(entries), dtype=np.int8)
        hashes = np.zeros((len(entries), 32), dtype=np.uint8)
        self._chk(_lib.lib().fdgpu_debug_poh(self._h, arena.ctypes.data, arena.size, entries.ctypes.data, len(entries),
                                             sig_offs.ctypes.data, len(sig_offs), int(hash_cnt_cap), int(grid_waves),
                                             codes.ctypes.data, hashes.ctypes.data), "debug_poh")
        return codes, hashes

    def debug_poh_time(self, arena, entries, sig_offs, hash_cnt_cap, iters=5):
        arena, entries, sig_offs = _poh_arrays(arena, entries, sig_offs)
        t, ch = ctypes.c_double(), ctypes.c_double()
        self._chk(_lib.lib().fdgpu_debug_poh_time(self._h, arena.ctypes.data, arena.size, entries.ctypes.data,
                                                  len(entries), sig_offs.ctypes.data, len(sig_offs), int(hash_cnt_cap),
                                                  int(iters), ctypes.byref(t), ctypes.byref(ch)), "debug_poh_time")
        return t.value, ch.value

    def debug_hram(self, arena, txns):
        arena = np.ascontiguousarray(arena, dtype=np.uint8)
        txns = np.ascontiguousarray(txns, dtype=TXN_DTYPE)
        out = np.zeros((len(txns), 32), dtype=np.uint8)
        self._chk(_lib.lib().fdgpu_debug_hram(self._h, arena.ctypes.data, arena.size, txns.ctypes.data, len(txns),
                                              out.ctypes.data), "debug_hram")
        return out

    def debug_sc_reduce(self, x):
        x = np.ascontiguousarray(x, dtype=np.uint8).reshape(-1, 64)
        out = np.zeros((len(x), 32), dtype=np.uint8)
        self._chk(_lib.lib().fdgpu_debug_sc_reduce(self._h, x.ctypes.data, len(x), out.ctypes.data), "debug_sc_reduce")
        return out

    def debug_hs_split(self, k):
        k = np.ascontiguousarray(k, dtype=np.uint8).reshape(-1, 32)
        out = np.zeros((len(k), 16), dtype=np.uint32)
        self._chk(_lib.lib().fdgpu_debug_hs_split(self._h, k.ctypes.data, len(k), out.ctypes.data), "debug_hs_split")
        return out

    def debug_fe_raw(self, fg):
        fg = np.ascontiguousarray(fg, dtype=np.uint32).reshape(-1, 20)
        out = np.zeros((len(fg), 10, 8), dtype=np.uint32)
        self._chk(_lib.lib().fdgpu_debug_fe_raw(self._h, fg.ctypes.data, len(fg), out.ctypes.data), "debug_fe_raw")
        return out

    def debug_ge_ops(self, rec):
        w_in, n_res = ge_ops_shape()
        rec = np.ascontiguousarray(rec, dtype=np.uint32).reshape(-1, w_in)
        out = np.zeros((len(rec), n_res, 4, 8), dtype=np.uint32)
        self._chk(_lib.lib().fdgpu_debug_ge_ops(self._h, rec.ctypes.data, len(rec), out.ctypes.data), "debug_ge_ops")
        return out

    def debug_sc_recode(self, s):
        s = np.ascontiguousarray(s, dtype=np.uint8).reshape(-1, 32)
        out = np.zeros((len(s), 16), dtype=np.uint32)
        self._chk(_lib.lib().fdgpu_debug_sc_recode(self._h, s.ctypes.data, len(s), out.ctypes.data), "debug_sc_recode")
        return out

    def debug_tabpack(self, ent):
        ent = np.ascontiguousarray(ent, dtype=np.uint32).reshape(-1, 40)
        out = np.zeros((len(ent), 160), dtype=np.uint32)
        self._chk(_lib.lib().fdgpu_debug_tabpack(self._h, ent.ctypes.data, len(ent), out.ctypes.data), "debug_tabpack")
        return out[:, :32].copy(), out[:, 32:152].reshape(-1, 3, 40).copy()

    def debug_verify_prehashed(self, arena, descs, full=False, pair=False, ref_mapping=False):
        arena = np.ascontiguousarray(arena, dtype=np.uint8)
        descs = np.ascontiguousarray(descs, dtype=SIG_DESC_DTYPE)
        codes = np.zeros(len(descs), dtype=np.int8)
        n_full = ctypes.c_uint32(0)
        flags = (KFLAG_REF_MAP if ref_mapping else 0) | (KFLAG_FULL if full else 0) | (KFLAG_PAIR if pair else 0)
        self._chk(_lib.lib().fdgpu_debug_verify_prehashed(self._h, arena.ctypes.data, arena.size, descs.ctypes.data,
                                                          len(descs), flags, codes.ctypes.data, ctypes.byref(n_full)),
                  "debug_verify_prehashed")
        return codes, int(n_full.value)

    def debug_btab(self):
        d = bcomb_dims()
        out = np.zeros((d["ndig"], d["entries"], d["stride"]), dtype=np.uint32)
        self._chk(_lib.lib().fdgpu_debug_btab(self._h, 0, d["ndig"] * d["entries"], out.ctypes.data), "debug_btab")
        return out

    def debug_sig_codes(self, arena, txns):
        arena = np.ascontiguousarray(arena, dtype=np.uint8)
        txns = np.ascontiguousarray(txns, dtype=TXN_DTYPE)
        cnt = txns["sig_cnt"].astype(np.int64)
        n = int(np.where((cnt >= 1) & (cnt <= 16), cnt, 0).sum())
        out = np.zeros(max(n, 1), dtype=np.int8)
        self._chk(_lib.lib().fdgpu_debug_sig_codes(self._h, arena.ctypes.data, arena.size, txns.ctypes.data,
                                                   len(txns), out.ctypes.data), "debug_sig_codes")
        return out[:n]


class DeviceBatch:

    def __init__(self, engine, arena, txns):
        arena = np.ascontiguousarray(arena, dtype=np.uint8)
        txns = np.ascontiguousarray(txns, dtype=TXN_DTYPE)
        self._e = engine
        self.n_txn = len(txns)
        self._b = _lib.lib().fdgpu_dev_batch_upload(engine._h, arena.ctypes.data, arena.size, txns.ctypes.data,
                                                    len(txns))
        if not self._b:
            raise RuntimeError(f"fdgpu_dev_batch_upload failed: {_lib.last_error()}")
        self.n_sig = int(_lib.lib().fdgpu_dev_batch_sig_cnt(self._b))

    def own_queue(self):
        rc = _lib.lib().fdgpu_dev_batch_own_queue(self._e._h, self._b)
        if rc != 0:
            raise RuntimeError(f"fdgpu_dev_batch_own_queue failed ({rc}): {_lib.last_error()}")
        return self

    def verify(self):
        rc = _lib.lib().fdgpu_dev_batch_verify(self._e._h, self._b)
        if rc != 0:
            raise RuntimeError(f"fdgpu_dev_batch_verify failed ({rc}): {_lib.last_error()}")

    def codes(self, sig_codes=False):
        t = np.zeros(max(self.n_txn, 1), dtype=np.int8)
        s = np.zeros(max(self.n_sig, 1), dtype=np.int8) if sig_codes else None
        rc = _lib.lib().fdgpu_dev_batch_codes(self._e._h, self._b, t.ctypes.data,
                                              s.ctypes.data if s is not None else None)
        if rc != 0:
            raise RuntimeError(f"fdgpu_dev_batch_codes failed ({rc}): {_lib.last_error()}")
        return (t[:self.n_txn], s[:self.n_sig]) if sig_codes else t[:self.n_txn]

    def time(self, iters):
        import ctypes as c
        w, v, k = c.c_double(), c.c_double(), c.c_double()
        rc = _lib.lib().fdgpu_dev_batch_time(self._e._h, self._b, int(iters), c.byref(w), c.byref(v), c.byref(k))
        if rc != 0:
            raise RuntimeError(f"fdgpu_dev_batch_time failed ({rc}): {_lib.last_error()}")
        return w.value, v.value, k.value

    def free(self):
        if self._b:
            _lib.lib().fdgpu_dev_batch_free(self._e._h, self._b)
            self._b = None

    def __del__(self):
        try:
            self.free()
        except Exception:
            pass


FRAG_DTYPE = np.dtype([("off", "<u4"), ("sz", "<u4")])
FRAG_EX_DTYPE = np.dtype([("off", "<u4"), ("sz", "<u4"), ("tr_off", "<u4"), ("tr_cap", "<u4")])
FRAG_IO_DTYPE = np.dtype([("src", "<u8"), ("sz", "<u4"), ("out_off", "<u4"), ("out_cap", "<u4"), ("link", "<u4"),
                          ("seq", "<u8")])
LINK_DTYPE = np.dtype([("mcache", "<u8"), ("depth", "<u8")])
CODE_LAPPED = -66
CODE_TRAILER_CAP = -65
CODE_PARSE_FAIL = -64
TXN_MAX_SZ = 852


class FragBatch(DeviceBatch):

    def __init__(self, engine, arena, frags):
        arena = np.ascontiguousarray(arena, dtype=np.uint8)
        frags = np.ascontiguousarray(frags, dtype=FRAG_DTYPE)
        self._e = engine
        self.n_txn = len(frags)
        self._b = _lib.lib().fdgpu_dev_batch_upload_frags(engine._h, arena.ctypes.data, arena.size,
                                                          frags.ctypes.data, len(frags))
        if not self._b:
            raise RuntimeError(f"fdgpu_dev_batch_upload_frags failed: {_lib.last_error()}")
        sz = frags["sz"].astype(np.int64)
        self.sig_bound = int(np.where(sz >= 134, np.minimum(16, (sz - 38) // 96), 0).sum())
        self.n_sig = self.sig_bound

    def codes(self, sig_codes=False):
        out = super().codes(sig_codes)
        self.n_sig = int(_lib.lib().fdgpu_dev_batch_sig_cnt(self._b))
        if sig_codes:
            return out[0], out[1][:self.n_sig]
        return out

    def txns(self, records=True):
        out = np.zeros((max(self.n_txn, 1), TXN_MAX_SZ), dtype=np.uint8) if records else None
        sz = np.zeros(max(self.n_txn, 1), dtype=np.uint16)
        rc = _lib.lib().fdgpu_dev_batch_txns(self._e._h, self._b, out.ctypes.data if records else None,
                                             sz.ctypes.data)
        if rc != 0:
            raise RuntimeError(f"fdgpu_dev_batch_txns failed ({rc}): {_lib.last_error()}")
        return (out[:self.n_txn] if records else None), sz[:self.n_txn]

    def time2(self, iters):
        import ctypes as c
        w, g, v, k = c.c_double(), c.c_double(), c.c_double(), c.c_double()
        rc = _lib.lib().fdgpu_dev_batch_time2(self._e._h, self._b, int(iters), c.byref(w), c.byref(g), c.byref(v),
                                              c.byref(k))
        if rc != 0:
            raise RuntimeError(f"fdgpu_dev_batch_time2 failed ({rc}): {_lib.last_error()}")
        return w.value, g.value, v.value, k.value
```

Baseline: 109.6 million sigs/s.

## Use affine-specialized table build, direct cached-to-p3 init, and pipelined SHA-512 loads

Builds the per-key point table with Z=1 specialized doubling and addition formulas, since the decoded point is affine. The first window's accumulator now comes straight from the cached entry instead of adding to the identity, which drops a full point addition. SHA-512 now prefetches the next message block's words before compressing the current block, uses alignbyte for unaligned extraction, and reads the block count as wave-uniform. The S load is hoisted before hashing, and a debug test kernel for the new formulas is added; the risk is correctness of the specialized formulas and higher register pressure from the prefetch.

```diff
diff --git a/firedancer_amd/_lib.py b/firedancer_amd/_lib.py
--- a/firedancer_amd/_lib.py
+++ b/firedancer_amd/_lib.py
@@ -197,6 +197,7 @@
     L.fdgpu_debug_sc_recode.argtypes = [vp, vp, c.c_uint64, vp]
     L.fdgpu_debug_btab.argtypes = [vp, c.c_uint64, c.c_uint64, vp]
     L.fdgpu_debug_tabpack.argtypes = [vp, vp, c.c_uint64, vp]
+    L.fdgpu_debug_affine_ops.argtypes = [vp, vp, c.c_uint64, vp]
     L.fdgpu_debug_verify_prehashed.argtypes = [vp, vp, c.c_uint64, vp, c.c_uint64, c.c_uint32, vp,
                                                c.POINTER(c.c_uint32)]
     L.fdgpu_bcomb_dim.argtypes = [c.c_int]
@@ -208,7 +209,7 @@
     for fn in ("fdgpu_debug_fe_ops", "fdgpu_debug_decode", "fdgpu_debug_sha512", "fdgpu_debug_hram",
                "fdgpu_debug_sc_reduce", "fdgpu_debug_hs_split", "fdgpu_debug_sig_codes",
                "fdgpu_debug_fe_raw", "fdgpu_debug_ge_ops", "fdgpu_debug_sc_recode", "fdgpu_debug_btab",
-               "fdgpu_debug_tabpack", "fdgpu_debug_verify_prehashed"):
+               "fdgpu_debug_tabpack", "fdgpu_debug_affine_ops", "fdgpu_debug_verify_prehashed"):
         getattr(L, fn).restype = c.c_int
     _LIB = L
     return L
diff --git a/firedancer_amd/csrc/fdgpu_atab.h b/firedancer_amd/csrc/fdgpu_atab.h
--- a/firedancer_amd/csrc/fdgpu_atab.h
+++ b/firedancer_amd/csrc/fdgpu_atab.h
@@ -106,6 +106,29 @@
   return s;
 }
 
+FDG_DEV void atab_build(uint32_t *wsl, const ge_p3 &An) {
+  ge_cached c;
+  ge_p3_to_cached(c, An); atab_store(wsl, 1, c);
+  ge_p1p1 t; ge_p2 a2; ge_p3 P;
+  ge_dbl_affine(t, An); ge_p1p1_to_p3(P, t);
+  ge_p3_to_cached(c, P); atab_store(wsl, 2, c);
+  const uint32_t *ent1 = wsl + 1u * FDGPU_PTAB_WORDS;
+  auto ld1 = [ent1](int cc, int w) { return atab_limb(ent1, cc, w); };
+#pragma unroll 1
+  for (uint32_t e = 3; e < FDGPU_ATAB_ENTRIES; e++) {
+    if (e & 1u) {
+      ge_add_cached_z1_ld(t, P, ld1, false);
+    } else {
+      uint32_t q[40];
+      atab_load(q, wsl, (int)(e >> 1));
+      ge_cached_regs_to_p2(a2, q, false);
+      ge_dbl(t, a2);
+    }
+    ge_p1p1_to_p3(P, t);
+    ge_p3_to_cached(c, P); atab_store(wsl, e, c);
+  }
+}
+
 typedef __attribute__((address_space(3))) void lds_void_t;
 
 FDG_DEV void stage_entry(uint32_t *lds_wave, const uint32_t *tab, int e) {
diff --git a/firedancer_amd/csrc/fdgpu_consts.h b/firedancer_amd/csrc/fdgpu_consts.h
--- a/firedancer_amd/csrc/fdgpu_consts.h
+++ b/firedancer_amd/csrc/fdgpu_consts.h
@@ -9,6 +9,7 @@
 #define FDGPU_FE_BT { 0x1b7dda3u, 0x1a2ace9u, 0x25eadbbu, 0x003ba8au, 0x083c27eu, 0x0abe37du, 0x1274732u, 0x0ccacddu, 0x0fd78b7u, 0x19e1d7cu }
 #define FDGPU_FE_Y0 { 0x395e826u, 0x1ecb0a3u, 0x068b604u, 0x1944fa6u, 0x3c263bfu, 0x1acdfd5u, 0x1e36982u, 0x1162726u, 0x2d88023u, 0x017f14du }
 #define FDGPU_FE_Y1 { 0x06a17c7u, 0x0134f5cu, 0x39749fbu, 0x06bb059u, 0x03d9c40u, 0x053202au, 0x21c967du, 0x0e9d8d9u, 0x1277fdcu, 0x1e80eb2u }
+#define FDGPU_FE_INV2D { 0x2e4fc18u, 0x01e4ed9u, 0x142e25eu, 0x06109e5u, 0x016bbadu, 0x0dce7b3u, 0x1884533u, 0x0e432b1u, 0x290a6aeu, 0x18120fdu }
 
 #define FDGPU_FE_2P { 0x07ffffdau, 0x03fffffeu, 0x07fffffeu, 0x03fffffeu, 0x07fffffeu, 0x03fffffeu, 0x07fffffeu, 0x03fffffeu, 0x07fffffeu, 0x03fffffeu }
 #define FDGPU_FE_4P { 0x0fffffb4u, 0x07fffffcu, 0x0ffffffcu, 0x07fffffcu, 0x0ffffffcu, 0x07fffffcu, 0x0ffffffcu, 0x07fffffcu, 0x0ffffffcu, 0x07fffffcu }
diff --git a/firedancer_amd/csrc/fdgpu_diag.cpp b/firedancer_amd/csrc/fdgpu_diag.cpp
--- a/firedancer_amd/csrc/fdgpu_diag.cpp
+++ b/firedancer_amd/csrc/fdgpu_diag.cpp
@@ -117,6 +117,10 @@
 
 int fdgpu_debug_tabpack(fdgpu_engine_t *e, uint8_t const *in, uint64_t n, uint8_t *out) {
   return debug_map(e, in, n, FDGPU_ATAB_WORDS, FDGPU_TABPACK_OUT_WORDS, out, fdgpu_launch_test_tabpack);
+}
+
+int fdgpu_debug_affine_ops(fdgpu_engine_t *e, uint8_t const *enc, uint64_t n, uint8_t *out) {
+  return debug_map(e, enc, n, 8, FDGPU_AFFINE_OUT_WORDS, out, fdgpu_launch_test_affine);
 }
 
 int fdgpu_debug_verify_prehashed(fdgpu_engine_t *e, uint8_t const *arena, uint64_t arena_sz,
diff --git a/firedancer_amd/csrc/fdgpu_ge.h b/firedancer_amd/csrc/fdgpu_ge.h
--- a/firedancer_amd/csrc/fdgpu_ge.h
+++ b/firedancer_amd/csrc/fdgpu_ge.h
@@ -40,6 +40,20 @@
   fe_carry_par(r.T);
 }
 
+FDG_DEV void ge_dbl_affine(ge_p1p1 &r, const ge_p3 &p) {
+  fe s;
+  fe_sq(r.X, p.X);
+  fe_sq(r.Z, p.Y);
+  fe_add(r.Y, r.Z, r.X);
+  fe_sub(r.Z, r.Z, r.X);
+  fe_add(s, p.X, p.Y);
+  fe_sq(r.X, s);
+  fe_sub4(r.X, r.X, r.Y);
+  fe_0(s); s.v[0] = 2;
+  fe_sub4(r.T, s, r.Z);
+  fe_carry_par(r.T);
+}
+
 FDG_DEV void fe_cswap(fe &a, fe &b, bool c) {
 #pragma unroll
   for (int i = 0; i < 10; i++) { const uint32_t x = a.v[i], y = b.v[i]; a.v[i] = c ? y : x; b.v[i] = c ? x : y; }
@@ -135,6 +149,12 @@
   r.Y = t;
 }
 
+template <class LD>
+FDG_DEV void ge_add_cached_z1_ld(ge_p1p1 &r, const ge_p3 &p, const LD &ld, bool neg) {
+  auto ldn = [&ld](int coord, int w) { return ld(coord == 2 ? 3 : coord, w); };
+  ge_add_niels_ld(r, p, ldn, neg);
+}
+
 FDG_DEV void ge_add_cached_regs(ge_p1p1 &r, const ge_p3 &p, const uint32_t (&q)[40], bool neg) {
   fe t, c;
 #pragma unroll
@@ -193,6 +213,21 @@
   fe_add(r.Y, a, b); fe_carry(r.Y);
 #pragma unroll
   for (int i = 0; i < 10; i++) r.Z.v[i] = q[20 + i];
+}
+
+FDG_DEV void ge_cached_regs_to_p3(ge_p3 &r, const uint32_t (&q)[40], bool neg) {
+  constexpr uint32_t I2D[10] = FDGPU_FE_INV2D;
+  fe a, b, c, i2d;
+  fe_set(i2d, I2D);
+#pragma unroll
+  for (int i = 0; i < 10; i++) { a.v[i] = neg ? q[10 + i] : q[i]; b.v[i] = neg ? q[i] : q[10 + i]; }
+  fe_sub(r.X, a, b); fe_carry(r.X);
+  fe_add(r.Y, a, b); fe_carry(r.Y);
+#pragma unroll
+  for (int i = 0; i < 10; i++) { r.Z.v[i] = q[20 + i]; c.v[i] = q[30 + i]; }
+  fe_cneg(c, neg);
+  fe_add(c, c, c);
+  fe_mul(r.T, c, i2d);
 }
 
 FDG_DEV void ge_niels_regs_to_p3(ge_p3 &r, const uint32_t (&q)[32], bool neg) {
diff --git a/firedancer_amd/csrc/fdgpu_internal.h b/firedancer_amd/csrc/fdgpu_internal.h
--- a/firedancer_amd/csrc/fdgpu_internal.h
+++ b/firedancer_amd/csrc/fdgpu_internal.h
@@ -179,11 +179,14 @@
 hipError_t fdgpu_launch_test_sc_recode(const uint32_t *d_in, uint32_t *d_out, uint32_t n, hipStream_t stream);
 #define FDGPU_TABPACK_OUT_WORDS 160u
 hipError_t fdgpu_launch_test_tabpack(const uint32_t *d_in, uint32_t *d_out, uint32_t n, hipStream_t stream);
+#define FDGPU_AFFINE_OUT_WORDS 1024u
+hipError_t fdgpu_launch_test_affine(const uint32_t *d_enc, uint32_t *d_out, uint32_t n, hipStream_t stream);
 
 int      fdgpu_debug_fe_raw(fdgpu_engine_t *e, uint8_t const *fg, uint64_t n, uint8_t *out);
 int      fdgpu_debug_ge_ops(fdgpu_engine_t *e, uint8_t const *in, uint64_t n, uint8_t *out);
 int      fdgpu_debug_sc_recode(fdgpu_engine_t *e, uint8_t const *s, uint64_t n, uint8_t *out);
 int      fdgpu_debug_tabpack(fdgpu_engine_t *e, uint8_t const *in, uint64_t n, uint8_t *out);
+int      fdgpu_debug_affine_ops(fdgpu_engine_t *e, uint8_t const *enc, uint64_t n, uint8_t *out);
 int      fdgpu_debug_verify_prehashed(fdgpu_engine_t *e, uint8_t const *arena, uint64_t arena_sz,
                                       fdgpu_sig_desc_t const *descs, uint64_t n, uint32_t flags, int8_t *codes_out,
                                       uint32_t *n_full_out);
diff --git a/firedancer_amd/csrc/fdgpu_sha512.h b/firedancer_amd/csrc/fdgpu_sha512.h
--- a/firedancer_amd/csrc/fdgpu_sha512.h
+++ b/firedancer_amd/csrc/fdgpu_sha512.h
@@ -77,20 +77,25 @@
   return (uint32_t)((((uint64_t)hi << 32) | lo) >> (8u * mis));
 }
 
-template <int T0>
-FDG_DEV void msg_block(uint64_t (&w)[16], const uint8_t *msg, uint32_t msg_sz, uint32_t base) {
-  constexpr int NW = 16 - T0;
+template <int NW>
+FDG_DEV void msg_load(uint32_t (&d)[2 * NW + 1], const uint8_t *msg, uint32_t msg_sz, uint32_t base) {
   const uint32_t lb = base < msg_sz ? base : 0u;
   const uint8_t *p = msg + lb;
   const uint32_t mis = (uint32_t)((uintptr_t)p & 3u);
   const uint32_t *q = (const uint32_t *)(p - mis);
-  uint32_t d[2 * NW + 1];
 #pragma unroll
   for (int i = 0; i < 2 * NW + 1; i++) d[i] = q[i];
+}
+template <int T0>
+FDG_DEV void msg_words(uint64_t (&w)[16], const uint32_t (&d)[2 * (16 - T0) + 1], const uint8_t *msg, uint32_t msg_sz,
+                       uint32_t base) {
+  constexpr int NW = 16 - T0;
+  const uint32_t lb = base < msg_sz ? base : 0u;
+  const uint32_t mis = (uint32_t)((uintptr_t)(msg + lb) & 3u);
 #pragma unroll
   for (int u = 0; u < NW; u++) {
-    const uint32_t lo = (uint32_t)((((uint64_t)d[2 * u + 1] << 32) | d[2 * u]) >> (8u * mis));
-    const uint32_t hi = (uint32_t)((((uint64_t)d[2 * u + 2] << 32) | d[2 * u + 1]) >> (8u * mis));
+    const uint32_t lo = __builtin_amdgcn_alignbyte(d[2 * u + 1], d[2 * u], mis);
+    const uint32_t hi = __builtin_amdgcn_alignbyte(d[2 * u + 2], d[2 * u + 1], mis);
     uint64_t v = ((uint64_t)hi << 32) | lo;
     const int64_t rem = (int64_t)msg_sz - (int64_t)base - 8 * u;
     if (rem < 8) {
@@ -101,29 +106,24 @@
     w[T0 + u] = ((uint64_t)bswap32((uint32_t)v) << 32) | bswap32((uint32_t)(v >> 32));
   }
 }
+template <int T0>
+FDG_DEV void msg_block(uint64_t (&w)[16], const uint8_t *msg, uint32_t msg_sz, uint32_t base) {
+  uint32_t d[2 * (16 - T0) + 1];
+  msg_load<16 - T0>(d, msg, msg_sz, base);
+  msg_words<T0>(w, d, msg, msg_sz, base);
+}
 
 FDG_DEV uint32_t sha512_hram_blocks(uint32_t msg_sz) { return (64u + msg_sz + 16u) / 128u + 1u; }
 
-FDG_DEV void sha512_hram(uint64_t (&h)[8], const uint32_t (&R)[8], const uint32_t (&A)[8],
-                         const uint8_t *msg, uint32_t msg_sz, uint32_t nblk_wave) {
+FDG_DEV void sha512_blocks(uint64_t (&h)[8], uint64_t (&w)[16], const uint8_t *msg, uint32_t msg_sz, uint32_t lead,
+                           uint32_t nblk, uint32_t nblk_wave, uint64_t bitlen) {
   const uint64_t H0[8] = {0x6a09e667f3bcc908ULL, 0xbb67ae8584caa73bULL, 0x3c6ef372fe94f82bULL,
                           0xa54ff53a5f1d36f1ULL, 0x510e527fade682d1ULL, 0x9b05688c2b3e6c1fULL,
                           0x1f83d9abfb41bd6bULL, 0x5be0cd19137e2179ULL};
 #pragma unroll
   for (int i = 0; i < 8; i++) h[i] = H0[i];
-  const uint32_t nblk = sha512_hram_blocks(msg_sz);
-  const uint64_t bitlen = (uint64_t)(64u + msg_sz) * 8u;
-  for (uint32_t blk = 0; blk < nblk_wave; blk++) {
-    uint64_t w[16];
-    if (blk == 0) {
-      msg_block<8>(w, msg, msg_sz, 0u);
-#pragma unroll
-      for (int t = 0; t < 4; t++) w[t] = ((uint64_t)bswap32(R[2 * t]) << 32) | bswap32(R[2 * t + 1]);
-#pragma unroll
-      for (int t = 0; t < 4; t++) w[4 + t] = ((uint64_t)bswap32(A[2 * t]) << 32) | bswap32(A[2 * t + 1]);
-    } else {
-      msg_block<0>(w, msg, msg_sz, 128u * blk - 64u);
-    }
+  nblk_wave = (uint32_t)__builtin_amdgcn_readfirstlane((int)nblk_wave);
+  auto step = [&](uint32_t blk) {
     if (blk + 1 == nblk) { w[14] = 0; w[15] = bitlen; }
     uint64_t hs[8];
 #pragma unroll
@@ -133,30 +133,33 @@
 #pragma unroll
       for (int i = 0; i < 8; i++) h[i] = hs[i];
     }
+  };
+  uint32_t blk = 0;
+  for (; blk + 1 < nblk_wave; blk++) {
+    const uint32_t next = 128u * (blk + 1u) - lead;
+    uint32_t d[33];
+    msg_load<16>(d, msg, msg_sz, next);
+    step(blk);
+    msg_words<0>(w, d, msg, msg_sz, next);
   }
+  step(blk);
+}
+
+FDG_DEV void sha512_hram(uint64_t (&h)[8], const uint32_t (&R)[8], const uint32_t (&A)[8],
+                         const uint8_t *msg, uint32_t msg_sz, uint32_t nblk_wave) {
+  uint64_t w[16];
+  msg_block<8>(w, msg, msg_sz, 0u);
+#pragma unroll
+  for (int t = 0; t < 4; t++) w[t] = ((uint64_t)bswap32(R[2 * t]) << 32) | bswap32(R[2 * t + 1]);
+#pragma unroll
+  for (int t = 0; t < 4; t++) w[4 + t] = ((uint64_t)bswap32(A[2 * t]) << 32) | bswap32(A[2 * t + 1]);
+  sha512_blocks(h, w, msg, msg_sz, 64u, sha512_hram_blocks(msg_sz), nblk_wave, (uint64_t)(64u + msg_sz) * 8u);
 }
 
 FDG_DEV void sha512_plain(uint64_t (&h)[8], const uint8_t *msg, uint32_t msg_sz, uint32_t nblk_wave) {
-  const uint64_t H0[8] = {0x6a09e667f3bcc908ULL, 0xbb67ae8584caa73bULL, 0x3c6ef372fe94f82bULL,
-                          0xa54ff53a5f1d36f1ULL, 0x510e527fade682d1ULL, 0x9b05688c2b3e6c1fULL,
-                          0x1f83d9abfb41bd6bULL, 0x5be0cd19137e2179ULL};
-#pragma unroll
-  for (int i = 0; i < 8; i++) h[i] = H0[i];
-  const uint32_t nblk = (msg_sz + 16u) / 128u + 1u;
-  const uint64_t bitlen = (uint64_t)msg_sz * 8u;
-  for (uint32_t blk = 0; blk < nblk_wave; blk++) {
-    uint64_t w[16];
-    msg_block<0>(w, msg, msg_sz, 128u * blk);
-    if (blk + 1 == nblk) { w[14] = 0; w[15] = bitlen; }
-    uint64_t hs[8];
-#pragma unroll
-    for (int i = 0; i < 8; i++) hs[i] = h[i];
-    sha512_compress(hs, w);
-    if (blk < nblk) {
-#pragma unroll
-      for (int i = 0; i < 8; i++) h[i] = hs[i];
-    }
-  }
+  uint64_t w[16];
+  msg_block<0>(w, msg, msg_sz, 0u);
+  sha512_blocks(h, w, msg, msg_sz, 0u, (msg_sz + 16u) / 128u + 1u, nblk_wave, (uint64_t)msg_sz * 8u);
 }
 
 }
diff --git a/firedancer_amd/csrc/fdgpu_test_kernels.hip b/firedancer_amd/csrc/fdgpu_test_kernels.hip
--- a/firedancer_amd/csrc/fdgpu_test_kernels.hip
+++ b/firedancer_amd/csrc/fdgpu_test_kernels.hip
@@ -256,10 +256,56 @@
   for (int w = 0; w < 40; w++) dst[112 + w] = q[w];
 }
 
+__global__ void __launch_bounds__(64) fdgpu_test_affine_kernel(const uint32_t *enc, uint32_t *out, uint32_t n) {
+  const uint32_t i = blockIdx.x * blockDim.x + threadIdx.x;
+  if (i >= n) return;
+  uint32_t e[8];
+#pragma unroll
+  for (int j = 0; j < 8; j++) e[j] = enc[8 * (size_t)i + j];
+  uint32_t *dst = out + FDGPU_AFFINE_OUT_WORDS * (size_t)i;
+  uint32_t *res = dst + 8u * FDGPU_PTAB_WORDS;
+  uint32_t *tab = dst - FDGPU_PTAB_WORDS;
+  ge_p3 P, Pn, Q;
+  const bool ok = ge_decode(P, e, false);
+  for (int j = 2; j < 32; j++) res[32 * 23 + j] = 0u;
+  res[32 * 23] = ok ? 1u : 0u;
+  res[32 * 23 + 1] = ge_is_small_order_affine(P) ? 1u : 0u;
+  ge_p3_neg(Pn, P);
+
+  ge_p1p1 t;
+  ge_p2 a2;
+  ge_dbl_affine(t, Pn);
+  put_p1p1(res, t);
+  ge_p3_to_p2(a2, Pn);
+  ge_dbl(t, a2);
+  ge_p1p1_to_p3(Q, t);
+  put_p3(res + 32, Q);
+
+  atab_build(tab, Pn);
+  const uint32_t *ent1 = tab + 1u * FDGPU_PTAB_WORDS;
+  auto ld1 = [ent1](int cc, int w) { return atab_limb(ent1, cc, w); };
+#pragma unroll 1
+  for (int s = 0; s < 2; s++) {
+    ge_add_cached_z1_ld(t, Q, ld1, s != 0); put_p1p1(res + 32 * (2 + s), t);
+    ge_add_cached_ld(t, Q, ld1, s != 0);    put_p1p1(res + 32 * (4 + s), t);
+  }
+#pragma unroll 1
+  for (int k = 0; k <= 16; k++) {
+    uint32_t q[40];
+    atab_load(q, tab, k == 16 ? 0 : 1 + (k & 7));
+    ge_cached_regs_to_p3(Q, q, k >= 8 && k < 16);
+    put_p3(res + 32 * (6 + k), Q);
+  }
+}
+
 }
 
 extern "C" {
 
+hipError_t fdgpu_launch_test_affine(const uint32_t *d_enc, uint32_t *d_out, uint32_t n, hipStream_t stream) {
+  hipLaunchKernelGGL(fdgpu_test_affine_kernel, dim3((n + 63) / 64), dim3(64), 0, stream, d_enc, d_out, n);
+  return hipGetLastError();
+}
 hipError_t fdgpu_launch_test_fe(const uint32_t *d_in, uint32_t *d_out, uint32_t n, hipStream_t stream) {
   hipLaunchKernelGGL(fdgpu_test_fe_kernel, dim3((n + 63) / 64), dim3(64), 0, stream, d_in, d_out, n);
   return hipGetLastError();
diff --git a/firedancer_amd/csrc/fdgpu_verify.hip b/firedancer_amd/csrc/fdgpu_verify.hip
--- a/firedancer_amd/csrc/fdgpu_verify.hip
+++ b/firedancer_amd/csrc/fdgpu_verify.hip
@@ -120,29 +120,6 @@
 #pragma unroll
     for (int w = 0; w < 32; w++) qa[w] = qb[w];
     d = dn;
-  }
-}
-
-FDG_DEV void atab_build(uint32_t *wsl, const ge_p3 &An) {
-  ge_cached c;
-  ge_p3_to_cached(c, An); atab_store(wsl, 1, c);
-  ge_p1p1 t; ge_p2 a2; ge_p3 P;
-  ge_p3_to_p2(a2, An); ge_dbl(t, a2); ge_p1p1_to_p3(P, t);
-  ge_p3_to_cached(c, P); atab_store(wsl, 2, c);
-  const uint32_t *ent1 = wsl + 1u * FDGPU_PTAB_WORDS;
-  auto ld1 = [ent1](int cc, int w) { return atab_limb(ent1, cc, w); };
-#pragma unroll 1
-  for (uint32_t e = 3; e < FDGPU_ATAB_ENTRIES; e++) {
-    if (e & 1u) {
-      ge_add_cached_ld(t, P, ld1, false);
-    } else {
-      uint32_t q[40];
-      atab_load(q, wsl, (int)(e >> 1));
-      ge_cached_regs_to_p2(a2, q, false);
-      ge_dbl(t, a2);
-    }
-    ge_p1p1_to_p3(P, t);
-    ge_p3_to_cached(c, P); atab_store(wsl, e, c);
   }
 }
 
@@ -235,9 +212,7 @@
     const int du = sext4(ud[4] >> 28), dv = sext4(vd[4] >> 28);
     shl4_5(ud); shl4_5(vd);
     atab_load(q, ta, du);
-    ge_p3_0(acc3);
-    ge_add_cached_regs(t, acc3, q, (du < 0) != u_neg);
-    ge_p1p1_to_p3(acc3, t);
+    ge_cached_regs_to_p3(acc3, q, (du < 0) != u_neg);
     atab_load(q, tr, dv);
     ge_add_cached_regs(t, acc3, q, (dv < 0) != v_neg);
   }
@@ -332,9 +307,10 @@
   uint32_t *aux = lane_aux(queue, i);
   const uint32_t *ta = tab_a(wsl);
   FDGPU_STAMP(0);
-  uint32_t Renc[8], Aenc[8];
+  uint32_t Renc[8], Aenc[8], S[8];
   load32(Renc, arena + d.sig_off);
   load32(Aenc, arena + d.pub_off);
+  load32(S, arena + d.sig_off + 32);
   uint32_t k[8];
   {
     uint64_t h[8];
@@ -350,8 +326,6 @@
     for (int j = 0; j < 8; j++) { kx[2 * j] = bswap32((uint32_t)(h[j] >> 32)); kx[2 * j + 1] = bswap32((uint32_t)h[j]); }
     sc_reduce512(k, kx);
   }
-  uint32_t S[8];
-  load32(S, arena + d.sig_off + 32);
   int code = sc_lt_L(S) ? 0 : -1;
 #pragma unroll
   for (int j = 0; j < 8; j++) S[j] = code ? 0u : S[j];
@@ -493,8 +467,8 @@
     const int d = sext4(dd[4] >> 28);
     shl4_5(dd);
     atab_load(q, tab, d);
-    ge_p3_0(acc3);
-    ge_add_cached_regs(t, acc3, q, (d < 0) != neg);
+    ge_cached_regs_to_p2(acc2, q, (d < 0) != neg);
+    t.X = acc2.X; t.Y = acc2.Y; t.Z = acc2.Z; t.T = acc2.Z;
   }
 #pragma unroll 1
   for (uint32_t j = 1; j < nwin; j++) {
@@ -536,9 +510,10 @@
   uint32_t *wsl = lane_ws(ws, i);
   uint32_t *aux = lane_aux(queue, i);
   uint32_t *tab = rl ? tab_r(wsl) : tab_a(wsl);
-  uint32_t Renc[8], Aenc[8];
+  uint32_t Renc[8], Aenc[8], S[8];
   load32(Renc, arena + d.sig_off);
   load32(Aenc, arena + d.pub_off);
+  load32(S, arena + d.sig_off + 32);
   uint32_t k[8];
   if (PH) {
     uint32_t kx[16];
@@ -551,8 +526,6 @@
   } else {
     hram_k(k, Renc, Aenc, arena, d, nb);
   }
-  uint32_t S[8];
-  load32(S, arena + d.sig_off + 32);
   int code = sc_lt_L(S) ? 0 : -1;
 #pragma unroll
   for (int j = 0; j < 8; j++) S[j] = code ? 0u : S[j];
diff --git a/firedancer_amd/ed25519.py b/firedancer_amd/ed25519.py
--- a/firedancer_amd/ed25519.py
+++ b/firedancer_amd/ed25519.py
@@ -613,6 +613,13 @@
         self._chk(_lib.lib().fdgpu_debug_tabpack(self._h, ent.ctypes.data, len(ent), out.ctypes.data), "debug_tabpack")
         return out[:, :32].copy(), out[:, 32:152].reshape(-1, 3, 40).copy()
 
+    def debug_affine_ops(self, enc):
+        enc = np.ascontiguousarray(enc, dtype=np.uint8).reshape(-1, 32)
+        out = np.zeros((len(enc), 1024), dtype=np.uint32)
+        self._chk(_lib.lib().fdgpu_debug_affine_ops(self._h, enc.ctypes.data, len(enc), out.ctypes.data),
+                  "debug_affine_ops")
+        return out[:, :256].reshape(-1, 8, 32).copy(), out[:, 256:].reshape(-1, 24, 4, 8).copy()
+
     def debug_verify_prehashed(self, arena, descs, full=False, pair=False, ref_mapping=False):
         arena = np.ascontiguousarray(arena, dtype=np.uint8)
         descs = np.ascontiguousarray(descs, dtype=SIG_DESC_DTYPE)
```

Measured after the change: 110.6 million sigs/s (median of 6 runs). Within noise of the previous version (+0.9%).
